# harrywaugh/UOB_Raytracer

Measured on AMD Instinct MI355X. Metric: Mrays/sec (nominal = W*H*AA*(1+S)/t), Cornell Box 4096^2, 8xAA, 64 shadow rays, higher is better.
Workload: dtype f32; 1 GPU; headline: Cornell Box 4096x4096, 4x2 AA, 64 shadow rays, 2 spheres, <=10 bounces, 26 triangles; parallelism=1 GPU

## Files before the change

include/uob_rt.h:

```cpp
#ifndef UOB_RT_H
#define UOB_RT_H

#include <stddef.h>
#include <stdint.h>

#ifdef __cplusplus
extern "C" {
#endif

#define RT_ABI_VERSION 2
#define RT_MAX_SPHERES 4
#define RT_MAX_DEVICES 8

enum {
  RT_OK = 0,
  RT_E_INVALID = -1,
  RT_E_DEVICE = -2,
  RT_E_NOMEM = -3,
  RT_E_IO = -4,
  RT_E_UNSUPPORTED = -5
};

typedef struct rt_sphere {
  float center[3];
// ... 39 lines not shown
            int32_t n_triangles, rt_ctx** out_ctx);

#define RT_UPDATE_REORDER 1u
int rt_update_scene(rt_ctx* ctx, const float* vertices4, const float* normals4, const float* colors4, int32_t n,
                    uint32_t flags);

int rt_update_scene_device(rt_ctx* ctx, const void* d_vertices4, const void* d_normals4, const void* d_colors4, int32_t n,
                           uint32_t flags, void* hip_stream);

#define RT_UPDATE_DEVICE_TILES 2u

int rt_replace_scene(rt_ctx* ctx, const float* vertices4, const float* normals4, const float* colors4, int32_t n_new,
                     uint32_t flags);

int rt_replace_scene_device(rt_ctx* ctx, const void* d_vertices4, const void* d_normals4, const void* d_colors4,
                            int32_t n_new, uint32_t flags, void* hip_stream);

int rt_update_spheres(rt_ctx* ctx, const rt_sphere* spheres, int32_t num_spheres);

int rt_debug_scene_capacity(rt_ctx* ctx, int64_t* out_triangles);

int rt_set_objects(rt_ctx* ctx, const int32_t* first, const int32_t* count, int32_t nobj);

int rt_pose_objects(rt_ctx* ctx, const float* xforms12, uint32_t flags);

int rt_pose_objects_device(rt_ctx* ctx, const void* d_xforms12, uint32_t flags, void* hip_stream);

int rt_debug_object_count(rt_ctx* ctx, int32_t* out);

int rt_set_skin(rt_ctx* ctx, int32_t first, int32_t count, const uint16_t* bone_index, const float* weights, int32_t nbones);

int rt_pose_skin(rt_ctx* ctx, const float* bones12, uint32_t flags);

int rt_pose_skin_device(rt_ctx* ctx, const void* d_bones12, uint32_t flags, void* hip_stream);

int rt_debug_skin_info(rt_ctx* ctx, int32_t* first, int32_t* count, int32_t* nbones);

int rt_render(rt_ctx* ctx, const float rot[12], const float cam[3], const float light[3], float focal,
              uint32_t* out_argb, float* out_rgb_f32);

int rt_render_device(rt_ctx* ctx, const float rot[12], const float cam[3], const float light[3],
                     float focal, void* d_out_argb, void* d_out_rgb_f32, void* hip_stream);

int rt_count_work(rt_ctx* ctx, const float rot[12], const float cam[3], const float light[3],
                  float focal, rt_work* out);

int rt_count_executed(rt_ctx* ctx, const float rot[12], const float cam[3], const float light[3],
                      float focal, uint64_t out[8]);

int rt_last_kernel_ms(rt_ctx* ctx, float* out_ms);

enum { RT_TRACE_IN_SHADOW = 0, RT_TRACE_CLOSEST_HIT = 1 };
int rt_debug_trace_rays(rt_ctx* ctx, int32_t what, const float* rays6, const float* radius_sq, int64_t nray,
                        int32_t* out_tri, float* out10);

int rt_trace_rays(rt_ctx* ctx, int32_t what, const float* rays6, const float* radius_sq, int64_t nray,
                  int32_t* out_tri, float* out10);
int rt_trace_rays_device(rt_ctx* ctx, int32_t what, const void* d_rays6, const void* d_radius_sq, int64_t nray,
                         void* d_out_tri, void* d_out10, void* hip_stream);
int rt_debug_trace_stats(rt_ctx* ctx, uint64_t out[8]);

int rt_shade_points(rt_ctx* ctx, const float* points6, const int32_t* seeds, int64_t npoints, const float light[3],
                    float* out_light, int32_t* out_unshadowed);
int rt_shade_points_device(rt_ctx* ctx, const void* d_points6, const void* d_seeds, int64_t npoints, const float light[3],
                           void* d_out_light, void* d_out_unshadowed, void* hip_stream);
int rt_debug_shade_stats(rt_ctx* ctx, uint64_t out[8]);

int rt_radiance_rays(rt_ctx* ctx, const float* rays6, const int32_t* seeds, int64_t nray, const float light[3],
                     float* out_rgba4, int32_t* out_prim);
int rt_radiance_rays_device(rt_ctx* ctx, const void* d_rays6, const void* d_seeds, int64_t nray, const float light[3],
                            void* d_out_rgba4, void* d_out_prim, void* hip_stream);
int rt_debug_radiance_stats(rt_ctx* ctx, uint64_t out[8]);

typedef struct rt_aov_buffers {
  int32_t* prim;
  float*   depth;
  float*   position4;
  float*   normal4;
  float*   albedo4;
  float*   direction4;
} rt_aov_buffers;

#define RT_AOV_ALL_SAMPLES (-1)
int rt_render_aov(rt_ctx* ctx, const float rot[12], const float cam[3], float focal, int32_t sample,
                  const rt_aov_buffers* host_out);
int rt_render_aov_device(rt_ctx* ctx, const float rot[12], const float cam[3], float focal, int32_t sample,
                         const rt_aov_buffers* device_out, void* hip_stream);
int rt_debug_aov_stats(rt_ctx* ctx, uint64_t out[8]);

typedef struct rt_filter_params {
  int32_t width, height;
  int32_t passes;
  float   normal_min_dot;
  float   plane_eps;
  float   value_max_diff;
} rt_filter_params;
void rt_filter_params_default(rt_filter_params* params, int32_t width, int32_t height);
int rt_filter_plane(rt_ctx* ctx, const rt_filter_params* params, const float* value, const float* position4,
                    const float* normal4, float* out);
int rt_filter_plane_device(rt_ctx* ctx, const rt_filter_params* params, const void* d_value, const void* d_position4,
                           const void* d_normal4, void* d_out, void* hip_stream);
int rt_debug_filter_stats(rt_ctx* ctx, uint64_t out[8]);
int rt_filter_plane_host(const rt_filter_params* params, const float* value, const float* position4, const float* normal4,
                         float* out);

typedef struct rt_history_texel {
  float position[3]; float mean;
  float normal[3];   float m2;
  float count;
  int32_t prim;
  float pad[2];
} rt_history_texel;

typedef struct rt_accumulate_params {
  int32_t width, height;
  float   prev_rot[12];
  float   prev_cam[3];
  float   prev_focal_px;
  float   normal_min_dot;
  float   plane_eps;
  int32_t max_history;
} rt_accumulate_params;
void rt_accumulate_params_default(rt_accumulate_params* params, int32_t width, int32_t height);
int rt_accumulate_plane(rt_ctx* ctx, const rt_accumulate_params* params, const float* value, const float* position4,
                        const float* normal4, const int32_t* prim, const rt_history_texel* prev, rt_history_texel* next,
                        float* out_mean, float* out_variance);
int rt_accumulate_plane_device(rt_ctx* ctx, const rt_accumulate_params* params, const void* d_value, const void* d_position4,
                               const void* d_normal4, const void* d_prim, const void* d_prev, void* d_next, void* d_out_mean,
                               void* d_out_variance, void* hip_stream);
int rt_debug_accumulate_stats(rt_ctx* ctx, uint64_t out[8]);
int rt_accumulate_plane_host(const rt_accumulate_params* params, const float* value, const float* position4,
                             const float* normal4, const int32_t* prim, const rt_history_texel* prev, rt_history_texel* next,
                             float* out_mean, float* out_variance);

int rt_debug_block_costs(rt_ctx* ctx, uint32_t* out, int32_t cap);

int rt_debug_world_masks(rt_ctx* ctx, uint64_t* out, int64_t cap, int32_t* grid, int32_t* words);

int rt_debug_tile_data(rt_ctx* ctx, int32_t* orig, float* tiles, int32_t cap_tiles);

int rt_debug_scene_data(rt_ctx* ctx, float* vertices4, float* normals4, float* colors4, float* vertices4_m,
                        float* normals4_m, float* colors4_m, int32_t* n_shadow, float vbox_lo[3], float vbox_hi[3],
                        int32_t cap_triangles);

int rt_register_output(rt_ctx* ctx, void* host, size_t bytes);
int rt_unregister_output(rt_ctx* ctx);

int rt_debug_wave_timeline(rt_ctx* ctx, uint64_t out[8]);

int rt_debug_wave_seeds(rt_ctx* ctx, void* records, int64_t cap, int32_t dims[3], uint64_t counters[4]);

int rt_debug_wave_seeds_wide(rt_ctx* ctx, void* records, int64_t cap, int32_t dims[3], uint64_t counters[10]);

enum { RT_COPY_2D = 0,
       RT_COPY_PEER = 1,
       RT_COPY_LINEAR = 2    };
typedef struct rt_band_copy {
  int32_t op, reserved;
  uint64_t dst_offset, dst_pitch, src_offset, src_pitch, width_bytes, rows;
} rt_band_copy;
int rt_debug_band_copy_plan(int32_t num_devices, int32_t k, int32_t device_band_rows, int32_t width, int32_t height,
                            int32_t elem_bytes, int32_t dev_to_dev, int32_t peer_ok, int32_t same_device,
                            rt_band_copy* out, int32_t cap);

int rt_selftest_rcp(uint64_t out[64]);

int rt_selftest_normalize(uint64_t out[8], uint32_t b_stride);

int rt_selftest_shade(int32_t nwaves, const int32_t* ns, const int32_t* lit, const int32_t* secondary, const int32_t* unshadowed,
                      const float* term, const float* col, int32_t straight_line, float* out);

int rt_selftest_all_within(int32_t nwaves, const int32_t* in, const float* v, const float* bound, int32_t* out);

void rt_destroy(rt_ctx* ctx);

int rt_debug_live_device_objects(int64_t out[4]);
const char* rt_last_error(void);
int rt_abi_version(void);

typedef struct rt_triangle {
  float v0[4], v1[4], v2[4], normal[4], color[4];
} rt_triangle;

int rt_scene_cornell_box(rt_triangle* out, int32_t cap);
int rt_scene_load_obj(const char* path, rt_triangle* out, int32_t cap);
int rt_scene_load_obj_ex(const char* path, const float color[4], float scale, const float translate[3],
                         rt_triangle* out, int32_t cap);
void rt_triangle_compute_normal(rt_triangle* t);
void rt_scene_transform(rt_triangle* tris, int32_t n, int32_t first, int32_t count, const float xform12[12]);
void rt_scene_skin(rt_triangle* tris, int32_t n, int32_t first, int32_t count, const uint16_t* bone_index,
                   const float* weights, const float* bones12, int32_t nbones);
void rt_scene_pack(const rt_triangle* tris, int32_t n, float* vertices4, float* normals4, float* colors4);
void rt_rotation_matrix(float yaw, float pitch, float rot[12]);

#ifdef __cplusplus
}
#endif
#endif
```

uob_raytracer_amd/csrc/rt_api.hip:

```cpp
#include <cmath>
#include <cstdarg>
#include <cstdio>
#include <cstdlib>
#include <cstring>
#include <memory>
#include <new>
#include <string>
#include <vector>

#include "rt_host.h"

namespace uobrt {

static thread_local std::string g_last_error;

void set_error(const char* fmt, ...) {
  char buf[1024];
  va_list ap;
  va_start(ap, fmt);
  vsnprintf(buf, sizeof buf, fmt, ap);
  va_end(ap);
  g_last_error = buf;
}

KeepError::KeepError() : text(g_last_error) {}
KeepError::~KeepError() { g_last_error = text; }

}

using namespace uobrt;

static int validate_config(const rt_config* c) {
  if (!c) { set_error("rt_config is NULL"); return RT_E_INVALID; }
  if (c->width < 1 || c->height < 1 || c->width > 32767 || c->height > 32767) {
    set_error("width/height must be in [1, 32767] (got %dx%d)", c->width, c->height); return RT_E_INVALID;
  }
  if (c->aa_x < 1 || c->aa_y < 1 || c->aa_x > 16 || c->aa_y > 16) { set_error("aa_x/aa_y must be in [1,16]"); return RT_E_INVALID; }
  if (c->shadow_samples < 1 || c->shadow_samples > 4096) { set_error("shadow_samples must be in [1,4096]"); return RT_E_INVALID; }
  if (c->max_bounces < 0 || c->max_bounces > 64) { set_error("max_bounces must be in [0,64]"); return RT_E_INVALID; }
  if (c->num_spheres < 0 || c->num_spheres > RT_MAX_SPHERES) { set_error("num_spheres must be in [0,%d]", RT_MAX_SPHERES); return RT_E_INVALID; }
  if (c->band_count < 1 || c->band_index < 0 || c->band_index >= c->band_count || c->band_rows < 1) {
    set_error("band partition invalid (rows=%d index=%d count=%d)", c->band_rows, c->band_index, c->band_count); return RT_E_INVALID;
  }
  if (!(c->light_spread >= 0.0f) || !(c->light_spread <= kMaxCoordinate)) { set_error("light_spread must be in [0, 2^16]"); return RT_E_INVALID; }
  if (validate_spheres(c->spheres, c->num_spheres) != RT_OK) return RT_E_INVALID;
  if ((double)c->width * c->height > 16777216.0) {
    set_error("width*height must not exceed 2^24 (the reference's FP32 pixel id)"); return RT_E_INVALID;
  }
  if (c->flags & 1) { set_error("flag bit 0 (the former RT_FLAG_FAST_MATH) is not defined in ABI %d", RT_ABI_VERSION); return RT_E_UNSUPPORTED; }
  if (c->num_devices < 0 || c->num_devices > RT_MAX_DEVICES || c->device_band_rows < 0) {
    set_error("num_devices must be in [0,%d] and device_band_rows >= 0", RT_MAX_DEVICES); return RT_E_INVALID;
  }
  if (c->num_devices > 1 && c->band_count != 1) {
    set_error("several devices in one context need the whole frame (band_count == 1)"); return RT_E_UNSUPPORTED;
  }
  return RT_OK;
}

static Tuning read_tuning(const rt_config& cfg) {
  Tuning t;
  if (const char* e = getenv("UOB_RT_JOB_TASKS")) t.job_tasks = atoi(e);
  if (const char* e = getenv("UOB_RT_HEAVY_FACTOR4")) { const int v = atoi(e); if (v >= 1 && v <= 4096) t.heavy_factor4 = v; }
  t.plain_order = (cfg.flags & RT_FLAG_PLAIN_ORDER) != 0 || getenv("UOB_RT_PLAIN_ORDER") != nullptr;
  t.full_grid = getenv("UOB_RT_FULL_GRID") != nullptr;
  t.no_specialise = getenv("UOB_RT_NO_SPECIALISE") != nullptr;
  if (const char* e = getenv("UOB_RT_HEAVY_DILATE")) t.heavy_dilate = atoi(e) != 0;
  if (const char* e = getenv("UOB_RT_L1_INFLATE")) { const float v = (float)atof(e); if (v >= 1.0f && v <= 64.0f) t.l1_inflate = v; }
  if (const char* e = getenv("UOB_RT_GRID_PER_CU")) { const int v = atoi(e); if (v >= 1 && v <= 8) t.grid_per_cu = v; }
  t.phase_profile = getenv("UOB_RT_PHASE_PROFILE") != nullptr;
  t.timeline = getenv("UOB_RT_TIMELINE") != nullptr;
  if (const char* e = getenv("UOB_RT_MASK_DEBUG")) t.mask_debug = atoi(e);
  if (const char* e = getenv("UOB_RT_TILE_ORDER")) t.tile_morton = !strcmp(e, "morton");
  if (const char* e = getenv("UOB_RT_NO_SEED")) t.no_seed = atoi(e) != 0;
  if (const char* e = getenv("UOB_RT_SEED_ROWS")) { const int v = atoi(e); if (v >= 1 && v <= 64) t.seed_rows = v; }
  if (const char* e = getenv("UOB_RT_SEED_KP")) { const int v = atoi(e); if (v >= 1 && v <= 64) t.seed_kp = v; }
  if (const char* e = getenv("UOB_RT_SEED_CASTERS")) { const int v = atoi(e); if (v >= 0 && v <= 64) t.seed_casters = v; }
  if (const char* e = getenv("UOB_RT_SEED_SPH")) t.seed_sph = atoi(e) != 0;
  if (const char* e = getenv("UOB_RT_FILTER_FORM")) t.filter_form = !strcmp(e, "direct") ? kFilterFormDirect : kFilterFormBuiltIn;
  return t;
}

extern "C" {

int rt_abi_version(void) { return RT_ABI_VERSION; }
const char* rt_last_error(void) { return g_last_error.c_str(); }

void rt_config_default(rt_config* cfg) {
  if (!cfg) return;
  memset(cfg, 0, sizeof *cfg);
  cfg->width = 1024; cfg->height = 1024;
  cfg->aa_x = 2; cfg->aa_y = 2;
  cfg->shadow_samples = 10; cfg->light_spread = 0.05f;
  cfg->max_bounces = 10;
  cfg->num_spheres = 2;
  const rt_sphere glass = {{0.3f, 0.1f, -0.5f}, 0.075f, {0.0f, 0.f, 0.f, -1.0f}};
  const rt_sphere mirror = {{-0.4f, 0.8f, -0.5f}, 0.05f, {0.0f, 0.f, 0.f, 0.0f}};
  cfg->spheres[0] = glass; cfg->spheres[1] = mirror;
  cfg->band_rows = cfg->height; cfg->band_index = 0; cfg->band_count = 1;
  cfg->device = -1; cfg->flags = 0;
  cfg->num_devices = 0; cfg->device_band_rows = 0;
}

int32_t rt_config_owned_rows(const rt_config* c) {
  if (!c || c->band_rows < 1 || c->band_count < 1) return 0;
  int rows = 0;
  for (int y = 0; y < c->height; ++y) rows += ((y / c->band_rows) % c->band_count) == c->band_index;
  return rows;
}

static int init_parent(const rt_config* cfg, const float* vertices4, const float* normals4, const float* colors4,
                       int32_t n, rt_ctx** out_ctx) {
  int ndev = 0;
  HIP_TRY(hipGetDeviceCount(&ndev));
  if (ndev < 1) { set_error("no HIP device present"); return RT_E_DEVICE; }
  for (int d = 0; d < cfg->num_devices; ++d)
    if (cfg->devices[d] < 0 || cfg->devices[d] >= ndev) {
      set_error("devices[%d] = %d, but %d HIP device(s) are present", d, cfg->devices[d], ndev); return RT_E_INVALID;
    }
  std::unique_ptr<rt_ctx> p(new (std::nothrow) rt_ctx());
  if (!p) { set_error("out of host memory"); return RT_E_NOMEM; }
  std::string downgrade;
  p->cfg = *cfg;
  p->device = cfg->devices[0];
  p->n = n; p->cap = n > 0 ? n : 1;
  p->owned_rows = rt_config_owned_rows(cfg);
  const int dbr = cfg->device_band_rows > 0 ? cfg->device_band_rows : 32;
  p->cfg.device_band_rows = dbr;
  for (int d = 0; d < cfg->num_devices; ++d) {
    rt_config kc = *cfg;
    kc.num_devices = 0; kc.device = cfg->devices[d];
    kc.band_rows = dbr; kc.band_index = d; kc.band_count = cfg->num_devices;
    rt_ctx* k = nullptr;
    const int rc = rt_init(&kc, vertices4, normals4, colors4, n, &k);
    if (rc != RT_OK) return rc;
    p->kids.push_back(k);
    if (hipSetDevice(k->device) != hipSuccess || k->ev_done.create(hipEventDisableTiming) != hipSuccess) {
      set_error("event creation failed on device %d", k->device); return RT_E_DEVICE;
    }
    if (k->device != p->device) {
      int can = 0;
      hipError_t e = hipDeviceCanAccessPeer(&can, k->device, p->device);
      if (e == hipSuccess && can) {
        e = hipDeviceEnablePeerAccess(p->device, 0);
        k->peer_ok = (e == hipSuccess || e == hipErrorPeerAccessAlreadyEnabled);
      } else {
        k->peer_ok = false;
      }
      (void)hipGetLastError();
      if (!k->peer_ok) {
        char line[160];
        snprintf(line, sizeof line, "%sdevice %d has no peer access to device %d (%s)", downgrade.empty() ? "warning: " : "; ",
                 k->device, p->device, e == hipSuccess ? "hipDeviceCanAccessPeer: no" : hipGetErrorString(e));
        downgrade += line;
      }
    }
  }
  if (hipSetDevice(p->device) != hipSuccess || p->ev_go.create(hipEventDisableTiming) != hipSuccess ||
      p->stream.create() != hipSuccess || p->ev0.create() != hipSuccess || p->ev1.create() != hipSuccess) {
    set_error("stream/event creation failed on device %d", p->device); return RT_E_DEVICE;
  }
  if (!downgrade.empty()) set_error("%s: their bands are copied band by band (hipMemcpyPeerAsync)", downgrade.c_str());
  *out_ctx = p.release();
  return RT_OK;
}

int rt_init(const rt_config* cfg, const float* vertices4, const float* normals4, const float* colors4,
            int32_t n, rt_ctx** out_ctx) {
  if (!out_ctx) { set_error("out_ctx is NULL"); return RT_E_INVALID; }
  *out_ctx = nullptr;
  int rc = validate_config(cfg);
  if (rc != RT_OK) return rc;
  if (n < 0 || (n > 0 && (!vertices4 || !normals4 || !colors4))) { set_error("scene arrays missing"); return RT_E_INVALID; }
  rc = validate_vertices(vertices4, n);
  if (rc != RT_OK) return rc;
  if (n > kMaxTriangles) { set_error("triangle list of %d exceeds the supported maximum of %d", n, kMaxTriangles); return RT_E_UNSUPPORTED; }
  DeviceGuard guard;
  if (cfg->num_devices > 1) return init_parent(cfg, vertices4, normals4, colors4, n, out_ctx);
  int ndev = 0;
  HIP_TRY(hipGetDeviceCount(&ndev));
  if (ndev < 1) { set_error("no HIP device present"); return RT_E_DEVICE; }
  std::unique_ptr<rt_ctx> c(new (std::nothrow) rt_ctx());
  if (!c) { set_error("out of host memory"); return RT_E_NOMEM; }
  c->cfg = *cfg;
  c->tune = read_tuning(*cfg);
  if (cfg->num_devices == 1) c->device = cfg->devices[0];
  else if (cfg->device >= 0) c->device = cfg->device;
  else hipGetDevice(&c->device);
  if (hipSetDevice(c->device) != hipSuccess) { set_error("hipSetDevice(%d) failed", c->device); return RT_E_DEVICE; }
  c->owned_rows = rt_config_owned_rows(cfg);
  if (hipDeviceGetAttribute(&c->cus, hipDeviceAttributeMultiprocessorCount, c->device) != hipSuccess || c->cus < 1) c->cus = 256;
  const size_t px = (size_t)(c->owned_rows > 0 ? c->owned_rows : 1) * cfg->width;
  if (c->d_argb.alloc(px) != hipSuccess || c->d_counters.alloc(sizeof(rt_work) / sizeof(unsigned long long)) != hipSuccess ||
      c->d_jobctr.alloc((2 * kJobHeads + 2) * kJobHeadStride) != hipSuccess || c->d_spheres.alloc(RT_MAX_SPHERES) != hipSuccess)
    return alloc_failed();
  {
    const int aa = cfg->aa_x * cfg->aa_y;
    const int pt = (aa >= 1 && aa <= 64) ? 64 / aa : 16;
    const size_t jobs_max = (size_t)((cfg->width + pt - 1) / pt) * (size_t)(c->owned_rows > 0 ? c->owned_rows : 1);
    c->heavy_cap = (int)(jobs_max / 3 > 64 ? jobs_max / 3 : 64);
    c->heavy_jobs_max = jobs_max;
  }
  if (c->stream.create() != hipSuccess || c->ev0.create() != hipSuccess || c->ev1.create() != hipSuccess) {
    set_error("stream/event creation failed"); return RT_E_DEVICE;
  }
  rc = upload_spheres(c.get());
  if (rc != RT_OK) return rc;
  rc = scene_first(c.get(), vertices4, normals4, colors4, n);
  if (rc != RT_OK) return rc;
  *out_ctx = c.release();
  return RT_OK;
}

}

void uobrt::fill_params(const rt_ctx* c, const float rot[12], const float cam[3], const float light[3], float focal,
                        FrameParams* P) {
  memset(P, 0, sizeof *P);
  memcpy(P->rot, rot, 12 * sizeof(float));
  memcpy(P->cam, cam, 3 * sizeof(float));
  memcpy(P->light, light, 3 * sizeof(float));
  P->focal = focal;
  const rt_config& g = c->cfg;
  P->spread = g.light_spread;
  P->W = g.width; P->H = g.height; P->aa_x = g.aa_x; P->aa_y = g.aa_y;
  P->S = g.shadow_samples; P->bounces = g.max_bounces; P->nsph = g.num_spheres; P->n = c->n;
  P->band_rows = g.band_rows; P->band_index = g.band_index; P->band_count = g.band_count;
  P->owned_rows = c->owned_rows;
  P->sy = (float)g.aa_x / (float)g.aa_y;
  {
    P->half_wx = ((float)g.width * (float)g.aa_x) / 2.0f;
    P->half_hy = ((float)g.height * (float)g.aa_y) / 2.0f;
    P->w_f = (float)g.width;
    P->focal0 = focal + 0.0f;
    P->rzf[0] = rot[2] * P->focal0; P->rzf[1] = rot[6] * P->focal0; P->rzf[2] = rot[10] * P->focal0;
    P->hbox = g.light_spread / 2.f;
    P->light_inf = fmaxf(fmaxf(fabsf(light[0]), fabsf(light[1])), fabsf(light[2]));
    P->band_rows_magic = div_magic_for(g.band_rows);
  }
  {
    const int aa = g.aa_x * g.aa_y;
    P->inv_S = (g.shadow_samples & (g.shadow_samples - 1)) == 0 ? 1.0f / (float)g.shadow_samples : 0.0f;
    P->inv_aa = (aa & (aa - 1)) == 0 ? 1.0f / (float)aa : 0.0f;
  }
  P->n_shadow = c->n_shadow;
  for (int i = 0; i < g.num_spheres; ++i) {
    P->sph[i].cx = g.spheres[i].center[0]; P->sph[i].cy = g.spheres[i].center[1]; P->sph[i].cz = g.spheres[i].center[2];
    P->sph[i].r2 = g.spheres[i].radius_sq;
    memcpy(P->sph[i].col, g.spheres[i].color, 16);
  }
  P->verts = c->d_verts; P->normals = c->d_normals; P->colors = c->d_colors;
  P->sph_dev = c->d_spheres;
  P->records = c->d_records;
  P->mask_debug = c->tune.mask_debug;
  P->job_counter = c->d_jobctr + kJobHeadStride;
  {
    const int aa = g.aa_x * g.aa_y;
    const bool wave_aa = aa >= 1 && aa <= 64;
    const int big_chunks = aa > 64 ? (aa + 63) / 64 : 0;
    const int pt = wave_aa ? 64 / aa : 64;
    P->aa_magic = wave_aa ? (65536 + aa - 1) / aa : 65536;
    P->aax_magic = (65536 + g.aa_x - 1) / g.aa_x;
    const int per_cu = c->tune.grid_per_cu ? c->tune.grid_per_cu : wave_blocks_per_cu(g.band_count > 1 && !c->tune.full_grid);
    P->wave_blocks = c->cus * per_cu;
    const long waves = (long)P->wave_blocks * 4;
    int jt = wave_aa ? 64 / pt : 1;
    while (jt > 1 && ((jt + 1) / 2) * pt >= 16 && (long)((g.width + jt * pt - 1) / (jt * pt)) * c->owned_rows < 16 * waves) jt = (jt + 1) / 2;
    if (wave_aa && c->tune.job_tasks >= 1 && c->tune.job_tasks * pt <= 64 && (c->tune.job_tasks * pt >= 16 || c->tune.job_tasks >= jt))
      jt = c->tune.job_tasks;
    if (big_chunks) jt = 16 * big_chunks;
    int job_pixels = 0;
    for (;;) {
      job_pixels = big_chunks ? jt / big_chunks : jt * pt;
      P->nseg = (g.width + job_pixels - 1) / job_pixels;
      P->njobs = P->nseg * c->owned_rows;
      P->nseg_magic = div_magic_for(P->nseg);
      if (big_chunks) break;
      const uint64_t err = P->nseg_magic ? (uint64_t)P->nseg_magic * (uint64_t)P->nseg - 0x100000000ull : 0ull;
      if ((uint64_t)(P->njobs > 0 ? P->njobs - 1 : 0) * err < 0x100000000ull || 2 * jt * pt > 64) break;
      jt *= 2;
    }
    P->job_tasks = jt;
    P->no_specialise = c->tune.no_specialise ? 1 : 0;
    P->l1_inflate = c->tune.l1_inflate;
    P->job_hx = 0.5f * (float)(job_pixels * g.aa_x - 1);
    P->job_hy = 0.5f * (float)(g.aa_y - 1) * P->sy;
    for (int k = 0; k < 3; ++k)
      P->job_eu[k] = 1.0001f * (fabsf(rot[4 * k]) * P->job_hx + fabsf(rot[4 * k + 1]) * P->job_hy);
  }
  if (c->d_screen_masks) {
    P->screen_masks = c->d_screen_masks; P->world_masks = c->d_world_masks; P->world_occ = c->d_world_occ;
    P->nwords = c->nwords; P->scx = c->scx; P->scy = c->scy; P->grid_g = kWorldGrid;
    float ext = 0.0f, dmax = 0.0f, amax = 0.0f, cmax = 0.0f;
    for (int k = 0; k < 3; ++k) {
      ext = fmaxf(ext, c->box_hi[k] - c->box_lo[k]);
      dmax = fmaxf(dmax, fmaxf(fabsf(light[k] - c->box_lo[k]), fabsf(light[k] - c->box_hi[k])));
      amax = fmaxf(amax, fmaxf(fabsf(c->box_lo[k]), fabsf(c->box_hi[k])));
      cmax = fmaxf(cmax, fabsf(cam[k]));
    }
    float grow = 2e-4f * dmax + 1e-4f * (amax + cmax) + 1e-3f * ext + 1e-30f;
    for (int i = 0; i < g.num_spheres; ++i) {
      float l2 = 0.0f;
      for (int k = 0; k < 3; ++k) l2 += (cam[k] - g.spheres[i].center[k]) * (cam[k] - g.spheres[i].center[k]);
      const float far = fmaxf(sqrtf(l2), 1.7321f * (ext + 2.0f * grow));
      grow = fmaxf(grow, 2.5e-3f * (far + sqrtf(fmaxf(g.spheres[i].radius_sq, 0.0f))));
    }
    for (int k = 0; k < 3; ++k) P->grid_lo[k] = c->box_lo[k] - grow;
    P->grid_cell = (ext + 2.0f * grow) / (float)kWorldGrid;
    P->grid_inv = 1.0f / P->grid_cell;
  }
}

void uobrt::use_tiled_scene(const rt_ctx* c, FrameParams* P) {
  P->verts = c->d_verts_m; P->normals = c->d_normals_m; P->colors = c->d_colors_m;
  P->orig = c->d_orig; P->tile_box = c->d_tile_box;
  P->mesh_blocks = c->cus * mesh_blocks_per_cu();
}

void uobrt::scene_params(const rt_ctx* c, const float light[3], bool tiled, FrameParams* P) {
  const float zero3[3] = {0.f, 0.f, 0.f}, ident[12] = {1, 0, 0, 0, 0, 1, 0, 0, 0, 0, 1, 0};
  fill_params(c, ident, zero3, light, 1.0f, P);
  if (tiled) use_tiled_scene(c, P);
}

static int launch_frame(rt_ctx* c, const float rot[12], const float cam[3], const float light[3], float focal,
                        uint32_t* d_argb, float4* d_rgb, hipStream_t stream, bool out_global = false) {
  if (!c || !rot || !cam || !light) { set_error("NULL argument"); return RT_E_INVALID; }
  for (int k = 0; k < 3; ++k)
    if (!(fabsf(cam[k]) <= kMaxCoordinate) || !(fabsf(light[k]) <= kMaxCoordinate)) {
      set_error("camera / light coordinates must be finite and <= 2^16"); return RT_E_INVALID;
    }
  if (!(fabsf(focal) <= 1.0e9f)) { set_error("focal length must be finite and <= 1e9"); return RT_E_INVALID; }
  for (int k = 0; k < 12; ++k)
    if (!(fabsf(rot[k]) <= 4.0f)) { set_error("rotation matrix entries must be finite and <= 4"); return RT_E_INVALID; }
  if (c->owned_rows == 0) return RT_OK;
  FrameParams P;
  fill_params(c, rot, cam, light, focal, &P);
  P.out_argb = d_argb; P.out_rgb = d_rgb; P.counters = nullptr;
  P.out_global = out_global ? 1 : 0;
  HIP_TRY(hipSetDevice(c->device));
  if (c->timed && stream != c->last_stream) HIP_TRY(hipStreamWaitEvent(stream, c->ev1, 0));
  HIP_TRY(wait_aov(c, stream));
  HIP_TRY(wait_scene(c, stream));
  HIP_TRY(hipEventRecord(c->ev0, stream));
  const bool wave_paths = !(c->cfg.flags & RT_FLAG_GENERIC_KERNEL);
  c->seed_tile_rows = 0;
  if (wave_paths && wave_kernel_supports(P) && (P.aa_x * P.aa_y <= 64 || !(c->cfg.flags & RT_FLAG_NO_CULL))) {
    if (c->d_heavy_flags && P.job_tasks >= 4) {
      const int prev = c->heavy_phase, cur = prev ^ 1;
      unsigned int* const st[2] = {c->d_jobctr, c->d_jobctr + (2 * kJobHeads + 1) * kJobHeadStride};
      P.heavy_prev = c->d_heavy[prev]; P.heavy_prev_state = st[prev];
      P.heavy_new = c->d_heavy[cur]; P.heavy_new_state = st[cur];
      P.heavy_flags = c->d_heavy_flags + (size_t)prev * c->heavy_jobs_max; P.heavy_flags_new = c->d_heavy_flags + (size_t)cur * c->heavy_jobs_max;
      P.heavy_gen = ++c->heavy_gen;
      P.heavy_factor4 = c->tune.heavy_factor4;
      P.heavy_cap = P.njobs / 3 < c->heavy_cap ? P.njobs / 3 : c->heavy_cap;
      P.heavy_dilate = c->tune.heavy_dilate ? 1 : 0;
      c->heavy_phase = cur;
    }
    c->timeline_valid = false;
    if (c->tune.timeline) {
      const size_t waves = (size_t)P.wave_blocks * 4;
      if (!c->d_timeline) {
        if (c->d_timeline.alloc(waves * 3) != hipSuccess) { set_error("hipMalloc failed (timeline)"); return RT_E_NOMEM; }
        c->timeline_waves = waves;
      }
      if (c->timeline_waves >= waves) {
        HIP_TRY(hipMemsetAsync(c->d_timeline, 0, c->timeline_waves * 3 * sizeof(uint64_t), stream));
        P.counters = reinterpret_cast<unsigned long long*>(c->d_timeline.p);
        c->timeline_valid = true;
      }
    }
    if (!c->tune.no_seed && wave_takes_seed(P, !(c->cfg.flags & RT_FLAG_NO_CULL))) {
      const int R = c->tune.seed_rows;
      const int tile_rows = (P.H + R - 1) / R;
      const size_t tiles = (size_t)tile_rows * (size_t)P.nseg;
      if (c->seed_cap < tiles) {
        if (c->d_seed.alloc(tiles) != hipSuccess) return alloc_failed();
        c->seed_cap = tiles;
      }
      P.seed = c->d_seed; P.seed_rows = R; P.seed_tile_rows = tile_rows; P.seed_rows_magic = div_magic_for(R);
      P.seed_hy = 0.5f * (float)(R * P.aa_y - 1) * P.sy;
      for (int k = 0; k < 3; ++k) P.seed_eu[k] = 1.0001f * (fabsf(rot[4 * k]) * P.job_hx + fabsf(rot[4 * k + 1]) * P.seed_hy);
      P.seed_kp_cap = c->tune.seed_kp; P.seed_caster_cap = c->tune.seed_casters; P.seed_keep_sph = c->tune.seed_sph ? 1 : 0;
      c->seed_tile_rows = tile_rows; c->seed_nseg = P.nseg; c->seed_rows = R;
    }
    launch_wave(P, !(c->cfg.flags & RT_FLAG_NO_CULL), false, stream);
  } else if (wave_paths && !(c->cfg.flags & RT_FLAG_NO_CULL) && mesh_kernel_supports(P)) {
    use_tiled_scene(c, &P);
    if (c->d_mesh_cost) {
      P.mesh_order = c->mesh_order_valid ? c->d_mesh_order : nullptr;
      P.mesh_cost = c->d_mesh_cost; P.mesh_order_out = c->d_mesh_order;
      P.mesh_queue_len = c->d_mesh_order + 4 * (size_t)((c->cfg.width + 15) / 16) * (size_t)((c->owned_rows + 15) / 16);
      c->mesh_order_valid = true;
    }
    launch_stage_records(P, stream);
    launch_mesh(P, false, false, stream, c->aux_stream, c->ev_fork, c->ev_join);
  } else {
    launch_generic(P, false, stream);
  }
  HIP_TRY(hipGetLastError());
  HIP_TRY(hipEventRecord(c->ev1, stream));
  c->timed = true;
  c->last_stream = stream;
  return RT_OK;
}

static int band_copy_plan(int N, int k, int dbr, int W, int owned_rows, size_t elem, bool dev_to_dev, bool peer_ok,
                          bool same_device, rt_band_copy* out, int cap) {
  const size_t band_bytes = (size_t)dbr * W * elem;
  const int full = owned_rows / dbr, rem = owned_rows % dbr;
  const size_t d0 = (size_t)k * band_bytes;
  int cnt = 0;
  auto emit = [&](int op, size_t doff, size_t dpitch, size_t soff, size_t spitch, size_t width, size_t rows) {
    if (cnt < cap && out) {
      rt_band_copy& c = out[cnt];
      c.op = op; c.reserved = 0; c.dst_offset = doff; c.dst_pitch = dpitch; c.src_offset = soff; c.src_pitch = spitch;
      c.width_bytes = width; c.rows = rows;
    }
    ++cnt;
  };
  if (full > 0) {
    if (!dev_to_dev || peer_ok) {
      emit(RT_COPY_2D, d0, (size_t)N * band_bytes, 0, band_bytes, band_bytes, (size_t)full);
    } else {
      for (int b = 0; b < full; ++b)
        emit(RT_COPY_PEER, d0 + (size_t)b * N * band_bytes, 0, (size_t)b * band_bytes, 0, band_bytes, 1);
    }
  }
  if (rem > 0) {
    const size_t bytes = (size_t)rem * W * elem;
    emit(dev_to_dev && !same_device ? RT_COPY_PEER : RT_COPY_LINEAR, d0 + (size_t)full * N * band_bytes, 0,
         (size_t)full * band_bytes, 0, bytes, 1);
  }
  return cnt;
}

static int deliver_bands(rt_ctx* p, int k, const void* stripe, void* dst, size_t elem, hipMemcpyKind kind, hipStream_t stream) {
  rt_ctx* c = p->kids[k];
  const int N = (int)p->kids.size(), dbr = p->cfg.device_band_rows, W = p->cfg.width;
  const bool d2d = kind == hipMemcpyDeviceToDevice;
  const int full = c->owned_rows / dbr;
  std::vector<rt_band_copy> plan((size_t)full + 2);
  int cnt = band_copy_plan(N, k, dbr, W, c->owned_rows, elem, d2d, c->peer_ok, c->device == p->device, plan.data(), (int)plan.size());
  for (int i = 0; i < cnt; ++i) {
    const rt_band_copy& q = plan[(size_t)i];
    char* const d = (char*)dst + q.dst_offset;
    const char* const sp = (const char*)stripe + q.src_offset;
    if (q.op == RT_COPY_2D) {
      const hipError_t e = hipMemcpy2DAsync(d, q.dst_pitch, sp, q.src_pitch, q.width_bytes, q.rows, kind, stream);
      if (e != hipSuccess && d2d && c->device != p->device) {
        (void)hipGetLastError();
        c->peer_ok = false;
        set_error("warning: device %d cannot copy 2-D into device %d (%s): its bands go band by band through hipMemcpyPeerAsync",
                  c->device, p->device, hipGetErrorString(e));
        cnt = band_copy_plan(N, k, dbr, W, c->owned_rows, elem, d2d, false, false, plan.data(), (int)plan.size());
        i = -1;
        continue;
      }
      if (e != hipSuccess) { set_error("hipMemcpy2DAsync failed: %s", hipGetErrorString(e)); return RT_E_DEVICE; }
    } else if (q.op == RT_COPY_PEER) {
      HIP_TRY(hipMemcpyPeerAsync(d, p->device, sp, c->device, q.width_bytes, stream));
    } else {
      HIP_TRY(hipMemcpyAsync(d, sp, q.width_bytes, kind, stream));
    }
  }
  return RT_OK;
}

static int parent_render(rt_ctx* p, const float rot[12], const float cam[3], const float light[3], float focal,
                         uint32_t* host_argb, float* host_rgb, uint32_t* d_argb, float4* d_rgb, hipStream_t caller) {
  const bool to_host = host_argb != nullptr;
  const size_t W = (size_t)p->cfg.width;
  const size_t nk = p->kids.size();
  if (!to_host) {
    HIP_TRY(hipSetDevice(p->device));
    HIP_TRY(hipEventRecord(p->ev0, caller));
    HIP_TRY(hipEventRecord(p->ev_go, caller));
  }
  const bool want_rgb = to_host ? host_rgb != nullptr : d_rgb != nullptr;
  std::vector<char> launched(nk, 0), direct(nk, 0);
  auto fail = [&](int rc) {
    KeepError keep;
    for (size_t k = 0; k < nk; ++k)
      if (launched[k]) { hipSetDevice(p->kids[k]->device); hipStreamSynchronize(p->kids[k]->stream); }
    (void)hipGetLastError();
    return rc;
  };
  for (size_t k = 0; k < nk; ++k) {
    rt_ctx* c = p->kids[k];
    if (c->owned_rows == 0) continue;
    if (hipSetDevice(c->device) != hipSuccess) { set_error("hipSetDevice(%d) failed", c->device); return fail(RT_E_DEVICE); }
    if (want_rgb && !c->d_rgb && c->d_rgb.alloc((size_t)c->owned_rows * W) != hipSuccess) {
      set_error("hipMalloc failed (float tap, device %d)", c->device); return fail(RT_E_NOMEM);
    }
    if (!to_host && hipStreamWaitEvent(c->stream, p->ev_go, 0) != hipSuccess) { set_error("hipStreamWaitEvent failed"); return fail(RT_E_DEVICE); }
    const bool mapped = to_host && !host_rgb && c->reg_host && (char*)host_argb >= c->reg_host &&
                        (char*)host_argb + (size_t)p->cfg.height * W * 4 <= c->reg_host + c->reg_bytes &&
                        !(p->cfg.flags & RT_FLAG_STAGED_GATHER);
    direct[k] = mapped || (!to_host && c->device == p->device && !(p->cfg.flags & RT_FLAG_STAGED_GATHER));
    uint32_t* const dst = mapped ? reinterpret_cast<uint32_t*>(c->reg_dev + ((char*)host_argb - c->reg_host)) : d_argb;
    const int rc = direct[k] ? launch_frame(c, rot, cam, light, focal, dst, mapped ? nullptr : d_rgb, c->stream, true)
                             : launch_frame(c, rot, cam, light, focal, c->d_argb, want_rgb ? c->d_rgb : nullptr, c->stream);
    if (rc != RT_OK) return fail(rc);
    launched[k] = 1;
  }
  for (size_t k = 0; k < nk; ++k) {
    rt_ctx* c = p->kids[k];
    if (!launched[k]) continue;
    if (hipSetDevice(c->device) != hipSuccess) { set_error("hipSetDevice(%d) failed", c->device); return fail(RT_E_DEVICE); }
    if (!direct[k]) {
      const hipMemcpyKind kind = to_host ? hipMemcpyDeviceToHost : hipMemcpyDeviceToDevice;
      int rc = deliver_bands(p, (int)k, c->d_argb, to_host ? (void*)host_argb : (void*)d_argb, 4, kind, c->stream);
      if (rc == RT_OK && want_rgb)
        rc = deliver_bands(p, (int)k, c->d_rgb, to_host ? (void*)host_rgb : (void*)d_rgb, sizeof(float4), kind, c->stream);
      if (rc != RT_OK) return fail(rc);
    }
    if (!to_host && hipEventRecord(c->ev_done, c->stream) != hipSuccess) { set_error("hipEventRecord failed"); return fail(RT_E_DEVICE); }
  }
  if (to_host) {
    for (rt_ctx* c : p->kids) if (c->owned_rows) { HIP_TRY(hipSetDevice(c->device)); HIP_TRY(hipStreamSynchronize(c->stream)); }
    p->timed = false;
  } else {
    HIP_TRY(hipSetDevice(p->device));
    for (rt_ctx* c : p->kids) if (c->owned_rows) HIP_TRY(hipStreamWaitEvent(caller, c->ev_done, 0));
    HIP_TRY(hipEventRecord(p->ev1, caller));
    p->timed = true;
  }
  return RT_OK;
}

extern "C" {

int rt_render_device(rt_ctx* c, const float rot[12], const float cam[3], const float light[3], float focal,
                     void* d_out_argb, void* d_out_rgb_f32, void* hip_stream) {
  if (!c || !d_out_argb) { set_error("NULL argument"); return RT_E_INVALID; }
  DeviceGuard guard;
  if (!c->kids.empty()) {
// ... 49 lines not shown
  return RT_OK;
}

int rt_register_output(rt_ctx* c, void* host, size_t bytes) {
  if (!c || !host || bytes == 0) { set_error("NULL argument"); return RT_E_INVALID; }
  const int rc = rt_unregister_output(c);
  if (rc != RT_OK) return rc;
  DeviceGuard guard;
  HIP_TRY(hipSetDevice(c->device));
  HIP_TRY(hipHostRegister(host, bytes, hipHostRegisterMapped | hipHostRegisterPortable));
  auto alias = [&](rt_ctx* x) -> bool {
    void* dev = nullptr;
    if (hipSetDevice(x->device) != hipSuccess || hipHostGetDevicePointer(&dev, host, 0) != hipSuccess || !dev) return false;
    x->reg_host = static_cast<char*>(host); x->reg_dev = static_cast<char*>(dev); x->reg_bytes = bytes;
    return true;
  };
  bool ok = alias(c);
  for (rt_ctx* k : c->kids) ok = ok && alias(k);
  if (!ok) {
    for (rt_ctx* k : c->kids) { k->reg_host = k->reg_dev = nullptr; k->reg_bytes = 0; }
    c->reg_host = c->reg_dev = nullptr; c->reg_bytes = 0;
    hipHostUnregister(host);
    set_error("hipHostGetDevicePointer failed: %s", hipGetErrorString(hipGetLastError()));
    return RT_E_DEVICE;
  }
  c->reg_owner = true;
  return RT_OK;
}

int rt_count_work(rt_ctx* c, const float rot[12], const float cam[3], const float light[3], float focal, rt_work* out) {
  if (!c || !out || !rot || !cam || !light) { set_error("NULL argument"); return RT_E_INVALID; }
  memset(out, 0, sizeof *out);
  DeviceGuard guard;
  if (!c->kids.empty()) {
    for (rt_ctx* k : c->kids) {
      rt_work w;
      const int rc = rt_count_work(k, rot, cam, light, focal, &w);
      if (rc != RT_OK) return rc;
      for (size_t q = 0; q < sizeof(rt_work) / 8; ++q) ((uint64_t*)out)[q] += ((const uint64_t*)&w)[q];
    }
    return RT_OK;
  }
  if (c->owned_rows == 0) return RT_OK;
  FrameParams P;
  fill_params(c, rot, cam, light, focal, &P);
  P.counters = c->d_counters;
  HIP_TRY(hipSetDevice(c->device));
  HIP_TRY(wait_aov(c, c->stream));
  HIP_TRY(wait_scene(c, c->stream));
  HIP_TRY(hipMemsetAsync(c->d_counters, 0, sizeof(rt_work), c->stream));
  launch_generic(P, true, c->stream);
  HIP_TRY(hipGetLastError());
  HIP_TRY(hipMemcpyAsync(out, c->d_counters, sizeof(rt_work), hipMemcpyDeviceToHost, c->stream));
  HIP_TRY(hipStreamSynchronize(c->stream));
  return RT_OK;
}

int rt_count_executed(rt_ctx* c, const float rot[12], const float cam[3], const float light[3], float focal, uint64_t out[8]) {
  if (!c || !out || !rot || !cam || !light) { set_error("NULL argument"); return RT_E_INVALID; }
  memset(out, 0, 8 * sizeof(uint64_t));
  DeviceGuard guard;
  if (!c->kids.empty()) {
    for (rt_ctx* k : c->kids) {
      uint64_t w[8];
      const int rc = rt_count_executed(k, rot, cam, light, focal, w);
      if (rc != RT_OK) return rc;
      for (int q = 0; q < 8; ++q) out[q] += w[q];
    }
    return RT_OK;
  }
  if (c->owned_rows == 0) return RT_OK;
  FrameParams P;
  fill_params(c, rot, cam, light, focal, &P);
  const bool generic = (c->cfg.flags & RT_FLAG_GENERIC_KERNEL) != 0;
  const bool mesh = !generic && !wave_kernel_supports(P) && !(c->cfg.flags & RT_FLAG_NO_CULL) && mesh_kernel_supports(P);
  if (generic || (!wave_kernel_supports(P) && !mesh) || (!mesh && P.S > 64)) {
    set_error("rt_count_executed: this configuration runs on the generic kernel, whose executed work is rt_count_work");
    return RT_E_UNSUPPORTED;
  }
  if (!mesh && P.aa_x * P.aa_y > 64) {
    set_error("rt_count_executed: more than 64 AA samples per pixel run on the wave kernel's chunked build, which has no counting build");
    return RT_E_UNSUPPORTED;
  }
  P.counters = c->d_counters;
  HIP_TRY(hipSetDevice(c->device));
  if (c->timed) HIP_TRY(hipStreamWaitEvent(c->stream, c->ev1, 0));
  HIP_TRY(wait_aov(c, c->stream));
  HIP_TRY(wait_scene(c, c->stream));
  HIP_TRY(hipMemsetAsync(c->d_counters, 0, sizeof(rt_work), c->stream));
  if (mesh) { use_tiled_scene(c, &P); launch_stage_records(P, c->stream); launch_mesh(P, true, c->tune.phase_profile, c->stream, nullptr, nullptr, nullptr); }
  else if (c->tune.phase_profile) launch_wave_prof(P, c->stream);
  else launch_wave(P, !(c->cfg.flags & RT_FLAG_NO_CULL), true, c->stream);
  HIP_TRY(hipGetLastError());
  HIP_TRY(hipMemcpyAsync(out, c->d_counters, sizeof(rt_work), hipMemcpyDeviceToHost, c->stream));
  HIP_TRY(hipStreamSynchronize(c->stream));
  return RT_OK;
}

int rt_debug_wave_timeline(rt_ctx* c, uint64_t out[8]) {
  if (!c || !out) { set_error("NULL argument"); return RT_E_INVALID; }
  c = lead_ctx(c);
  if (!c->tune.timeline || !c->timeline_valid) {
    set_error("rt_debug_wave_timeline: needs UOB_RT_TIMELINE=1 at rt_init and a frame rendered by the wave kernel");
    return RT_E_UNSUPPORTED;
  }
  DeviceGuard guard;
  HIP_TRY(hipSetDevice(c->device));
  if (c->timed) HIP_TRY(hipEventSynchronize(c->ev1));
  std::vector<uint64_t> rec(c->timeline_waves * 3);
  HIP_TRY(hipMemcpy(rec.data(), c->d_timeline, rec.size() * sizeof(uint64_t), hipMemcpyDeviceToHost));
  for (int q = 0; q < 8; ++q) out[q] = 0;
  out[1] = ~0ull;
  for (size_t w = 0; w < c->timeline_waves; ++w) {
    const uint64_t t0 = rec[3 * w], t1 = rec[3 * w + 1], jobs = rec[3 * w + 2] & 0xffffffffull;
    if (t1 == 0) continue;
    out[7] = rec[3 * w + 2] >> 32;
    out[0] += 1; out[3] += t0; out[4] += t1; out[5] += jobs;
    if (t0 < out[1]) out[1] = t0;
    if (t1 > out[2]) out[2] = t1;
    if (jobs > out[6]) out[6] = jobs;
  }
  return RT_OK;
}

static int read_seed_table(rt_ctx* c, std::vector<SeedRec>* rec, std::vector<uint64_t>* rows) {
  rec->clear(); rows->clear();
  if (c->seed_tile_rows == 0) return RT_OK;
  DeviceGuard guard;
  HIP_TRY(hipSetDevice(c->device));
  if (c->timed) HIP_TRY(hipEventSynchronize(c->ev1));
  rec->resize((size_t)c->seed_tile_rows * (size_t)c->seed_nseg);
  HIP_TRY(hipMemcpy(rec->data(), c->d_seed, rec->size() * sizeof(SeedRec), hipMemcpyDeviceToHost));
  const rt_config& g = c->cfg;
  rows->assign((size_t)c->seed_tile_rows, 0);
  for (int tr = 0; tr < c->seed_tile_rows; ++tr)
    for (int y = tr * c->seed_rows; y < (tr + 1) * c->seed_rows && y < g.height; ++y)
      (*rows)[tr] += ((y / g.band_rows) % g.band_count) == g.band_index;
  return RT_OK;
}

int rt_debug_wave_seeds(rt_ctx* c, void* records, int64_t cap, int32_t dims[3], uint64_t counters[4]) {
  if (!c || !dims || !counters || cap < 0 || (cap > 0 && !records)) { set_error("NULL argument"); return RT_E_INVALID; }
  c = lead_ctx(c);
  dims[0] = c->seed_tile_rows; dims[1] = c->seed_nseg; dims[2] = c->seed_rows;
  for (int q = 0; q < 4; ++q) counters[q] = 0;
  if (c->seed_tile_rows == 0) { dims[1] = 0; return RT_OK; }
  std::vector<SeedRec> rec;
  std::vector<uint64_t> rows;
  const int rc = read_seed_table(c, &rec, &rows);
  if (rc != RT_OK) return rc;
  for (size_t t = 0; t < rec.size(); ++t) {
    SeedRec& r = rec[t];
    r.flags &= kSeedPrimary | kSeedShadow;
    if (!(r.flags & kSeedPrimary)) r.Kp = 0ull;
    if (!(r.flags & kSeedShadow)) { r.D0[0] = r.D0[1] = r.D0[2] = 0.0f; r.ed = 0.0f; r.K = 0ull; r.Kh = 0ull; r.h = -1; }
    const uint64_t n = rows[t / (size_t)c->seed_nseg];
    if (r.flags & kSeedPrimary) { counters[0] += 1; counters[2] += n; }
    if (r.flags & kSeedShadow) { counters[1] += 1; counters[3] += n; }
  }
  if (records) memcpy(records, rec.data(), (size_t)((int64_t)rec.size() < cap ? (int64_t)rec.size() : cap) * sizeof(SeedRec));
  return RT_OK;
}

int rt_debug_wave_seeds_wide(rt_ctx* c, void* records, int64_t cap, int32_t dims[3], uint64_t counters[10]) {
  if (!c || !dims || !counters || cap < 0 || (cap > 0 && !records)) { set_error("NULL argument"); return RT_E_INVALID; }
  c = lead_ctx(c);
  dims[0] = c->seed_tile_rows; dims[1] = c->seed_nseg; dims[2] = c->seed_rows;
  for (int q = 0; q < 10; ++q) counters[q] = 0;
  if (c->seed_tile_rows == 0) { dims[1] = 0; return RT_OK; }
  std::vector<SeedRec> rec;
  std::vector<uint64_t> rows;
  const int rc = read_seed_table(c, &rec, &rows);
  if (rc != RT_OK) return rc;
  for (size_t t = 0; t < rec.size(); ++t) {
    const SeedRec& r = rec[t];
    const uint64_t n = rows[t / (size_t)c->seed_nseg];
    const bool shadow = (r.flags & kSeedShadowWide) != 0u;
    const bool is[5] = {(r.flags & kSeedPrimaryWide) != 0u, shadow, shadow && r.Kh != 0ull, shadow && (r.flags & kSeedShadowSph) != 0u,
                        shadow && (r.flags & kSeedShadowBlocked) != 0u};
    for (int q = 0; q < 5; ++q)
      if (is[q]) { counters[2 * q] += 1; counters[2 * q + 1] += n; }
  }
  if (records) memcpy(records, rec.data(), (size_t)((int64_t)rec.size() < cap ? (int64_t)rec.size() : cap) * sizeof(SeedRec));
  return RT_OK;
}

int rt_debug_trace_rays(rt_ctx* c, int32_t what, const float* rays6, const float* radius_sq, int64_t nray,
                        int32_t* out_tri, float* out10) {
  if (!c || !rays6 || !out_tri || nray < 0) { set_error("NULL argument"); return RT_E_INVALID; }
  if (what != RT_TRACE_IN_SHADOW && what != RT_TRACE_CLOSEST_HIT) { set_error("rt_debug_trace_rays: unknown mode %d", what); return RT_E_INVALID; }
  if (what == RT_TRACE_IN_SHADOW && !radius_sq) { set_error("rt_debug_trace_rays: radius_sq missing"); return RT_E_INVALID; }
  if (what == RT_TRACE_CLOSEST_HIT && !out10) { set_error("rt_debug_trace_rays: out10 missing"); return RT_E_INVALID; }
  c = lead_ctx(c);
  if (nray == 0) return RT_OK;
  DeviceGuard guard;
  HIP_TRY(hipSetDevice(c->device));
  const float zero3[3] = {0.f, 0.f, 0.f};
  FrameParams P;
  scene_params(c, zero3, false, &P);
  DevMem<float> d_rays, d_r2, d_out;
  DevMem<int> d_tri;
  const size_t n = (size_t)nray;
  if (d_rays.alloc(n * 6) != hipSuccess || d_tri.alloc(n) != hipSuccess || (radius_sq && d_r2.alloc(n) != hipSuccess) ||
      (out10 && d_out.alloc(n * 10) != hipSuccess))
    return alloc_failed();
  if (c->timed) HIP_TRY(hipStreamWaitEvent(c->stream, c->ev1, 0));
  HIP_TRY(wait_aov(c, c->stream));
  HIP_TRY(wait_scene(c, c->stream));
  HIP_TRY(hipMemcpyAsync(d_rays, rays6, n * 24, hipMemcpyHostToDevice, c->stream));
  if (radius_sq) HIP_TRY(hipMemcpyAsync(d_r2, radius_sq, n * 4, hipMemcpyHostToDevice, c->stream));
  if (d_out) HIP_TRY(hipMemsetAsync(d_out, 0, n * 40, c->stream));
  if (generic_needs_records(c->n)) launch_stage_records(P, c->stream);
  launch_trace_rays(P, what, d_rays, d_r2, (long)nray, d_tri, d_out, c->stream);
  HIP_TRY(hipGetLastError());
  HIP_TRY(hipMemcpyAsync(out_tri, d_tri, n * 4, hipMemcpyDeviceToHost, c->stream));
  if (out10 && what == RT_TRACE_CLOSEST_HIT) HIP_TRY(hipMemcpyAsync(out10, d_out, n * 40, hipMemcpyDeviceToHost, c->stream));
  HIP_TRY(hipStreamSynchronize(c->stream));
  return RT_OK;
}

int rt_debug_band_copy_plan(int32_t num_devices, int32_t k, int32_t device_band_rows, int32_t width, int32_t height,
                            int32_t elem_bytes, int32_t dev_to_dev, int32_t peer_ok, int32_t same_device,
                            rt_band_copy* out, int32_t cap) {
  if (num_devices < 1 || num_devices > RT_MAX_DEVICES || k < 0 || k >= num_devices || device_band_rows < 0 || width < 1 ||
      height < 1 || elem_bytes < 1 || cap < 0 || (!out && cap > 0)) {
    set_error("rt_debug_band_copy_plan: invalid argument"); return RT_E_INVALID;
  }
  const int dbr = device_band_rows > 0 ? device_band_rows : 32;
  rt_config kc;
  memset(&kc, 0, sizeof kc);
  kc.height = height; kc.band_rows = dbr; kc.band_index = k; kc.band_count = num_devices;
  return band_copy_plan(num_devices, k, dbr, width, rt_config_owned_rows(&kc), (size_t)elem_bytes, dev_to_dev != 0, peer_ok != 0,
                        same_device != 0, out, cap);
}

int rt_debug_block_costs(rt_ctx* c, uint32_t* out, int32_t cap) {
  if (!c || (!out && cap > 0) || cap < 0) { set_error("NULL argument"); return RT_E_INVALID; }
  c = lead_ctx(c);
  if (!c->d_mesh_cost || !c->mesh_order_valid) { set_error("rt_debug_block_costs: this context records no block costs"); return RT_E_UNSUPPORTED; }
  DeviceGuard guard;
  HIP_TRY(hipSetDevice(c->device));
  const int jobs = ((c->cfg.width + 15) / 16) * ((c->owned_rows + 15) / 16);
  if (c->timed) HIP_TRY(hipEventSynchronize(c->ev1));
  std::vector<uint32_t> raw((size_t)jobs);
  HIP_TRY(hipMemcpy(raw.data(), c->d_mesh_cost, (size_t)jobs * 4, hipMemcpyDeviceToHost));
  const int wx = (c->cfg.width + 15) / 16, wy = (c->owned_rows + 15) / 16, mid = (wy + 1) >> 1;
  for (int j = 0; j < jobs; ++j) {
    const int jy = j / wx, jx = j - jy * wx;
    const int row = (jy & 1) ? mid + (jy >> 1) : mid - 1 - (jy >> 1);
    const int at = row * wx + jx;
    if (at >= 0 && at < cap) out[at] = raw[(size_t)j];
  }
  return jobs;
}

int rt_debug_world_masks(rt_ctx* c, uint64_t* out, int64_t cap, int32_t* grid, int32_t* words) {
  if (!c || (!out && cap > 0) || cap < 0 || !grid || !words) { set_error("NULL argument"); return RT_E_INVALID; }
  c = lead_ctx(c);
  if (!c->d_world_masks || c->nwords <= 0) { set_error("rt_debug_world_masks: this context builds no tile masks"); return RT_E_UNSUPPORTED; }
  DeviceGuard guard;
  HIP_TRY(hipSetDevice(c->device));
  if (c->timed) HIP_TRY(hipEventSynchronize(c->ev1));
  const size_t total = (size_t)kWorldGrid * kWorldGrid * kWorldGrid * (size_t)c->nwords;
  *grid = kWorldGrid; *words = c->nwords;
  const size_t take = total < (size_t)cap ? total : (size_t)cap;
  if (take > 0) HIP_TRY(hipMemcpy(out, c->d_world_masks, take * 8, hipMemcpyDeviceToHost));
  return (int)total;
}

int rt_last_kernel_ms(rt_ctx* c, float* out_ms) {
  if (!c || !out_ms) { set_error("NULL argument"); return RT_E_INVALID; }
  DeviceGuard guard;
  if (!c->kids.empty() && !c->timed) {
    float mx = -1.0f;
    for (rt_ctx* k : c->kids) {
      float ms = 0.0f;
      if (k->timed && rt_last_kernel_ms(k, &ms) == RT_OK && ms > mx) mx = ms;
    }
    if (mx < 0.0f) { set_error("no frame has been rendered on this context"); return RT_E_INVALID; }
    *out_ms = mx;
    return RT_OK;
  }
  if (!c->timed) { set_error("no frame has been rendered on this context"); return RT_E_INVALID; }
  HIP_TRY(hipSetDevice(c->device));
  HIP_TRY(hipEventSynchronize(c->ev1));
  HIP_TRY(hipEventElapsedTime(out_ms, c->ev0, c->ev1));
  return RT_OK;
}

int rt_debug_live_device_objects(int64_t out[4]) {
  if (!out) { set_error("rt_debug_live_device_objects: NULL argument"); return RT_E_INVALID; }
  for (int k = 0; k < 4; ++k) out[k] = g_live[k].load(std::memory_order_relaxed);
  return RT_OK;
}

void rt_destroy(rt_ctx* c) {
  if (!c) return;
  DeviceGuard guard;
  delete c;
}

}

rt_ctx::~rt_ctx() {
  for (rt_ctx* k : kids) delete k;
  hipSetDevice(device);
  if (stream) hipStreamSynchronize(stream);
  if (aux_stream) hipStreamSynchronize(aux_stream);
  for (SideCall* k : {&query, &shade, &rad, &aov, &filter, &accum})
    if (k->ev) hipEventSynchronize(k->ev);
  if (reg_host && reg_owner) hipHostUnregister(reg_host);
}
```

uob_raytracer_amd/csrc/rt_device.h:

```cpp
#pragma once
#include <hip/hip_runtime.h>
#include <stdint.h>

#include "../../include/uob_rt.h"

namespace uobrt {

constexpr int kJobHeads = 31;
constexpr int kJobHeadStride = 32;
constexpr int kHeavyStateWords = 8;
constexpr float kMaxCoordinate = 65536.0f;
constexpr int kRecordsPerTriangle = 8;

struct DevSphere {
  float cx, cy, cz, r2;
  float col[4];
};

struct alignas(16) SeedRec {
  float D0[3], ed;
  unsigned long long K, Kh, Kp;
  int32_t h;
  uint32_t flags;
  uint32_t pad[4];
};
constexpr uint32_t kSeedPrimary = 1u, kSeedShadow = 2u;
constexpr uint32_t kSeedPrimaryWide = 4u, kSeedPrimarySph = 8u;
constexpr int kSeedShadowShift = 4;
constexpr uint32_t kSeedShadowWide = 1u << kSeedShadowShift, kSeedShadowSph = 2u << kSeedShadowShift, kSeedShadowBlocked = 4u << kSeedShadowShift;
static_assert(sizeof(SeedRec) == 64, "one record per 64-byte line");

struct FrameParams {
  float rot[12];
  float cam[3];
  float focal;
  float light[3];
  float spread;
  int32_t W, H, aa_x, aa_y;
  int32_t S;
  int32_t bounces;
  int32_t nsph;
  int32_t n;
  int32_t band_rows, band_index, band_count, owned_rows;
  float sy;
  float half_wx, half_hy;
  float w_f;
  float focal0;
  float rzf[3];
  float hbox;
  float light_inf;
  float job_hx, job_hy;
  float job_eu[3];
  uint32_t nseg_magic, band_rows_magic;
  float inv_S, inv_aa;
  int32_t n_shadow;
  DevSphere sph[RT_MAX_SPHERES];
  const DevSphere* sph_dev;
  const float4* verts;
  const float4* normals;
  const float4* colors;
  uint32_t* out_argb;
  float4* out_rgb;
  int32_t out_global;
  int32_t wave_blocks;
  unsigned long long* counters;
  unsigned int* job_counter;
  int32_t njobs, nseg;
  int32_t aa_magic;
  int32_t aax_magic;
  int32_t job_tasks;
  int32_t no_specialise;
  const unsigned int* heavy_prev;
  const unsigned int* heavy_prev_state;
  unsigned int* heavy_new;
  unsigned int* heavy_new_state;
  const unsigned int* heavy_flags;
  unsigned int* heavy_flags_new;
  uint32_t heavy_gen;
  int32_t heavy_factor4;
  int32_t heavy_cap;
  float l1_inflate;
  int32_t heavy_dilate;
  float4* records;
  const unsigned int* mesh_order;
  unsigned int* mesh_cost;
  unsigned int* mesh_order_out;
  unsigned int* mesh_queue_len;
  int32_t mesh_blocks;
  const int* orig;
  const float4* tile_box;
  unsigned long long* screen_masks;
  unsigned long long* world_masks;
  unsigned int* world_occ;
  int32_t mask_debug;
  int32_t nwords, scx, scy, grid_g;
  float grid_lo[3], grid_cell, grid_inv;
  SeedRec* seed;
  int32_t seed_rows;
  int32_t seed_tile_rows;
  uint32_t seed_rows_magic;
  float seed_hy;
  float seed_eu[3];
  int32_t seed_kp_cap, seed_caster_cap, seed_keep_sph;
};


struct AovPlanes {
  int* prim;
  float* depth;
  float4 *position, *normal, *albedo, *direction;
};

__device__ inline uint32_t div_magic(uint32_t n, uint32_t magic) { return magic ? __umulhi(n, magic) : n; }

__host__ __device__ inline int band_global_row(int lr, int band_rows, int band_index, int band_count) {
  return ((lr / band_rows) * band_count + band_index) * band_rows + (lr % band_rows);
}
__device__ inline int band_global_row(const struct FrameParams& P, int lr);

__device__ inline int band_global_row(const FrameParams& P, int lr) {
  const int q = (int)div_magic((uint32_t)lr, P.band_rows_magic);
  return (q * P.band_count + P.band_index) * P.band_rows + (lr - q * P.band_rows);
}

}
```

uob_raytracer_amd/csrc/rt_host.h:

```cpp
#pragma once
#include <hip/hip_runtime.h>

#include <atomic>
#include <string>
#include <utility>
#include <vector>

#include "rt_device.h"

#define HIP_TRY(expr)                                                                   \
  do {                                                                                  \
    hipError_t e_ = (expr);                                                             \
    if (e_ != hipSuccess) {                                                             \
      uobrt::set_error("%s failed: %s (%s:%d)", #expr, hipGetErrorString(e_), __FILE__, __LINE__); \
      return RT_E_DEVICE;                                                               \
    }                                                                                   \
  } while (0)

namespace uobrt {

void set_error(const char* fmt, ...);

struct KeepError {
  std::string text;
  KeepError();
  ~KeepError();
};

constexpr int kMaxTriangles = 4000000;
constexpr int kWorldGrid = 32;

void launch_generic(const FrameParams& P, bool count, hipStream_t stream);
bool generic_needs_records(int n);
void launch_stage_records(const FrameParams& P, hipStream_t stream);
void launch_trace_rays(const FrameParams& P, int what, const float* d_rays, const float* d_r2, long nray, int* d_tri,
                       float* d_out10, hipStream_t stream);
void launch_wave(const FrameParams& P, bool cull, bool count, hipStream_t stream);
void launch_wave_prof(const FrameParams& P, hipStream_t stream);
bool wave_kernel_supports(const FrameParams& P);
bool wave_takes_seed(const FrameParams& P, bool cull);
int wave_blocks_per_cu(bool leave_room);
void launch_mesh(const FrameParams& P, bool count, bool prof, hipStream_t stream, hipStream_t aux, hipEvent_t ev_fork, hipEvent_t ev_join);
void launch_bin_primary(const FrameParams& P, hipStream_t stream);
bool mesh_kernel_supports(const FrameParams& P);
int mesh_tiles(int n);
int mesh_occ_words(int grid);
int mesh_screen_cells(int pixels);
int mesh_blocks_per_cu();
int launch_scene_check(const float4* v, const float4* col, int n, unsigned int* out, hipStream_t stream);
void launch_scene_refit(const float4* v, const float4* nrm, const float4* col, const int* orig, int n, float4* vm, float4* nm,
                        float4* cm, float4* tile_box, hipStream_t stream);
constexpr unsigned int kPoseStatic = 0xffffu;
void launch_pose(const float4* rest_v, const float4* rest_n, const unsigned short* object_of, const float* d_xforms12, int n,
                 float4* out_v, float4* out_n, hipStream_t stream);
void launch_skin(const float4* rest_v, const float4* rest_n, const ushort4* index, const float4* weights, const float* d_bones12,
                 int n, int first, int count, float4* out_v, float4* out_n, hipStream_t stream);
size_t tile_build_scratch_bytes(int n);
int launch_tile_build(const float4* v, int n, const float lo[3], const float hi[3], int* orig, void* scratch, hipStream_t stream);
int query_stats_words();
void launch_query(const FrameParams& P, bool tiled, int what, const float* d_rays, const float* d_r2, long nray, int* d_tri,
                  float* d_out10, unsigned long long* stats, int cus, hipStream_t stream);
int shade_stats_words();
void launch_shade(const FrameParams& P, bool tiled, const float* d_points6, const int* d_seeds, long npoints, float* d_light,
                  int* d_cnt, unsigned long long* stats, int cus, hipStream_t stream);
int radiance_stats_words();
size_t radiance_record_bytes(long nray);
void launch_radiance(const FrameParams& P, bool tiled, const float* d_rays6, const int* d_seeds, long nray, float4* d_rgba,
                     int* d_prim, float4* d_records, unsigned long long* stats, int cus, hipStream_t stream);
int aov_stats_words();
void launch_aov(const FrameParams& P, bool tiled, const AovPlanes& A, int sample, unsigned long long* stats, int cus, hipStream_t stream);
constexpr int kFilterTX = 64, kFilterTY = 4, kFilterMaxTiledSpacing = 32;
constexpr int kFilterFormBuiltIn = 0, kFilterFormDirect = 1;
int filter_stats_words();
void launch_filter_pack(const float4* d_pos, const float4* d_nrm, long count, int passes, float4* d_rec, unsigned long long* stats,
                        hipStream_t stream);
void launch_filter_pass(const rt_filter_params& p, int pass, int form, const float4* d_rec, const float* d_src, float* d_dst,
                        unsigned long long* stats, hipStream_t stream);
void launch_filter_counters(unsigned long long* stats, hipStream_t stream);
int filter_check(const rt_filter_params* p, const void* value, const void* position4, const void* normal4, const void* out,
                 const char* fn);
int accumulate_stats_words();
void launch_accumulate(const rt_accumulate_params& p, const float* d_value, const float4* d_pos, const float4* d_nrm, const int* d_prim,
                       const float4* d_prev, float4* d_next, float* d_out_mean, float* d_out_variance, unsigned long long* stats,
                       hipStream_t stream);
int accumulate_check(const rt_accumulate_params* p, const void* value, const void* position4, const void* normal4, const void* prev,
                     const void* next, const char* fn);
void vertex_box(const float* vertices4, int n, float lo[3], float hi[3]);
std::vector<int> tiled_order(const float* v4, int n, bool morton);
std::vector<float> tile_data_host(const float* v4, const int* orig, int n);

inline uint32_t div_magic_for(int d) { return d > 1 ? (uint32_t)((0x100000000ull + (uint64_t)d - 1) / (uint64_t)d) : 0u; }

inline int blocks_per_cu(const void* kernel, int threads) {
  int per_cu = 0;
  if (hipOccupancyMaxActiveBlocksPerMultiprocessor(&per_cu, kernel, threads, 0) != hipSuccess || per_cu < 1) per_cu = 2;
  return per_cu;
}
inline unsigned grid_blocks(long want, long cap) { return (unsigned)(want < cap ? (want > 0 ? want : 1) : cap); }

struct Tuning {
  int job_tasks = 0;
  int heavy_factor4 = 8;
  bool plain_order = false;
  bool full_grid = false;
  float l1_inflate = 3.5f;
  bool heavy_dilate = true;
  bool no_specialise = false;
  int grid_per_cu = 0;
  bool phase_profile = false;
  bool timeline = false;
  int mask_debug = 0;
  bool tile_morton = false;
  int filter_form = 0;
  bool no_seed = false;
  int seed_rows = 16;
  int seed_kp = 64;
  int seed_casters = 32;
  bool seed_sph = true;
};

inline std::atomic<int64_t> g_live[4];
inline void live_add(int slot, int64_t d) { g_live[slot].fetch_add(d, std::memory_order_relaxed); }

template <class T>
struct DevMem {
  T* p = nullptr;
  size_t bytes = 0;
  DevMem() = default;
  DevMem(DevMem&& o) noexcept : p(std::exchange(o.p, nullptr)), bytes(std::exchange(o.bytes, 0)) {}
  DevMem& operator=(DevMem&& o) noexcept {
    if (this != &o) { reset(); p = std::exchange(o.p, nullptr); bytes = std::exchange(o.bytes, 0); }
    return *this;
  }
  ~DevMem() { reset(); }
  hipError_t alloc(size_t count) {
    reset();
    const size_t want = count ? count * sizeof(T) : 1;
    const hipError_t e = hipMalloc(&p, want);
    if (e != hipSuccess) { p = nullptr; return e; }
    bytes = want; live_add(0, 1); live_add(1, (int64_t)want);
    return hipSuccess;
  }
  void reset() {
    if (p) { hipFree(p); live_add(0, -1); live_add(1, -(int64_t)bytes); }
    p = nullptr; bytes = 0;
  }
  operator T*() const { return p; }
};
inline int alloc_failed() { set_error("hipMalloc failed: %s", hipGetErrorString(hipGetLastError())); return RT_E_NOMEM; }
using DevBuffer = DevMem<char>;
int ensure_bytes(DevBuffer* b, size_t bytes);

template <class H, hipError_t (*Create)(H*, unsigned), hipError_t (*Destroy)(H), int Slot>
struct Handle {
  H h = nullptr;
  Handle() = default;
  Handle(Handle&& o) noexcept : h(std::exchange(o.h, nullptr)) {}
  Handle& operator=(Handle&& o) noexcept { if (this != &o) { reset(); h = std::exchange(o.h, nullptr); } return *this; }
  ~Handle() { reset(); }
  hipError_t create(unsigned flags = 0) {
    reset();
    const hipError_t e = Create(&h, flags);
    if (e != hipSuccess) h = nullptr; else live_add(Slot, 1);
    return e;
  }
  void reset() { if (h) { Destroy(h); live_add(Slot, -1); h = nullptr; } }
  operator H() const { return h; }
};
using Event = Handle<hipEvent_t, hipEventCreateWithFlags, hipEventDestroy, 2>;
using Stream = Handle<hipStream_t, hipStreamCreateWithFlags, hipStreamDestroy, 3>;

struct SceneStore {
  DevMem<float4> verts_m, normals_m, colors_m, tile_box, records;
  DevMem<int> orig;
  DevMem<unsigned long long> screen_masks, world_masks;
  DevMem<unsigned int> world_occ;
  DevMem<unsigned int> heavy[2], heavy_flags, mesh_cost, mesh_order;
};

struct SideCall {
  Event ev;
  bool pending = false;
  DevMem<unsigned long long> d_stats;
  int tiles = 0;
  DevBuffer io;
};

}

struct rt_ctx {
  ~rt_ctx();
  rt_config cfg;
  uobrt::Tuning tune;
  int device = 0;
  int n = 0, n_shadow = 0;
  int cap = 0;
  uobrt::SceneStore own;
  uobrt::DevBuffer tile_scratch;
  int owned_rows = 0;
  uobrt::DevMem<float4> d_verts, d_normals, d_colors;
  uobrt::DevMem<uint32_t> d_argb;
  uobrt::DevMem<float4> d_rgb;
  uobrt::DevMem<unsigned long long> d_counters;
  uobrt::DevMem<unsigned int> d_jobctr;
  uobrt::DevMem<uobrt::SeedRec> d_seed;
  size_t seed_cap = 0;
  int seed_tile_rows = 0, seed_nseg = 0, seed_rows = 0;
  int cus = 256;
  unsigned int *d_heavy[2] = {nullptr, nullptr}, *d_heavy_flags = nullptr;
  int heavy_cap = 0, heavy_phase = 0;
  size_t heavy_jobs_max = 0;
  char* reg_host = nullptr; char* reg_dev = nullptr; size_t reg_bytes = 0;
  bool reg_owner = false;
  bool timeline_valid = false;
  uobrt::DevMem<uint64_t> d_timeline;
  size_t timeline_waves = 0;
  uint32_t heavy_gen = 0;
  float4* d_records = nullptr;
  float4 *d_verts_m = nullptr, *d_normals_m = nullptr, *d_colors_m = nullptr, *d_tile_box = nullptr;
  int* d_orig = nullptr;
  uobrt::DevMem<uobrt::DevSphere> d_spheres;
  unsigned int *d_mesh_cost = nullptr, *d_mesh_order = nullptr;
  bool mesh_order_valid = false;
  unsigned long long *d_screen_masks = nullptr, *d_world_masks = nullptr;
  unsigned int* d_world_occ = nullptr;
  int nwords = 0, scx = 0, scy = 0;
  float box_lo[3] = {0, 0, 0}, box_hi[3] = {0, 0, 0};
  float vbox_lo[3] = {0, 0, 0}, vbox_hi[3] = {0, 0, 0};
  uobrt::Stream stream;
  uobrt::Stream aux_stream;
  uobrt::Event ev_fork, ev_join;
  uobrt::Event ev0, ev1;
  bool timed = false;
  hipStream_t last_stream = nullptr;
  std::vector<rt_ctx*> kids;
  uobrt::Event ev_go;
  uobrt::Event ev_done;
  bool peer_ok = true;
  uobrt::Event ev_upd;
  bool upd_pending = false;
  uobrt::DevMem<unsigned int> d_check;
  int nobj = 0;
  uobrt::DevMem<float4> d_rest_verts, d_rest_normals;
  uobrt::DevMem<unsigned short> d_object_of;
  uobrt::DevBuffer pose_verts, pose_normals, pose_xforms;
  int skin_first = 0, skin_count = 0, skin_nbones = 0;
  uobrt::DevMem<ushort4> d_skin_index;
  uobrt::DevMem<float4> d_skin_weights;
  uobrt::SideCall query, shade, rad;
  uobrt::DevMem<float4> d_qrecords;
  uobrt::DevBuffer rrec;
  uobrt::SideCall aov;
  hipStream_t aov_stream = nullptr;
  uobrt::SideCall filter;
  uobrt::DevBuffer filter_guides, filter_planes;
  uobrt::SideCall accum;
};

namespace uobrt {

struct DeviceGuard {
  int prev = -1;
  DeviceGuard() { if (hipGetDevice(&prev) != hipSuccess) prev = -1; }
  ~DeviceGuard() { if (prev >= 0) hipSetDevice(prev); }
};

inline rt_ctx* lead_ctx(rt_ctx* c) { return c->kids.empty() ? c : c->kids[0]; }

inline hipError_t wait_scene(const rt_ctx* c, hipStream_t s) {
  return c->upd_pending ? hipStreamWaitEvent(s, c->ev_upd, 0) : hipSuccess;
}
// ... 21 lines not shown
```

uob_raytracer_amd/csrc/rt_kernel_wave.hip:

```cpp
#define RT_SPHERES_IN_LDS
#define RT_RNG_JUMP_IN_LDS
#include "rt_host.h"
#include "rt_wave_common.h"

#include <type_traits>

namespace uobrt {

namespace {

constexpr int kChunk = 4;

struct WaveLds {
  float4* r0;
  float4* r1;
  float2* r2;
  float4* h0;
  float4* h1;
  uint32_t* rng;
};
__host__ __device__ constexpr int wave_lds_bytes(bool cull) {
  return (cull ? 0 : 64 * (16 + 16 + 8)) + 64 * 32 + kRngPixels * kRngStride * 4;
}

// ... 132 lines not shown

template <int SP>
__device__ __forceinline__ void wave_unshadowed_packed(const FrameParams& P, const ShadowCasters& SC, const WaveLds& L, int lane,
                                                       unsigned long long pmA, int baseA, const uint32_t* rngA,
                                                       unsigned long long pmB, int baseB, const uint32_t* rngB,
                                                       unsigned long long K, unsigned long long need_l, unsigned long long sphmask,
                                                       int NS, int& unshadowed) {
  constexpr int PK = 64 / SP;
  const int q = lane / SP, sidx = lane - q * SP;
  int ja[PK], jb[PK];
  {
    unsigned long long m = pmA;
#pragma unroll
    for (int i = 0; i < PK; ++i) { ja[i] = m != 0ull ? baseA + __builtin_ctzll(m) : -1; m &= m - 1ull; }
    m = pmB;
#pragma unroll
    for (int i = 0; i < PK; ++i) { jb[i] = m != 0ull ? baseB + __builtin_ctzll(m) : -1; m &= m - 1ull; }
  }
  int myA = ja[0], myB = jb[0];
#pragma unroll
  for (int i = 1; i < PK; ++i) { myA = q == i ? ja[i] : myA; myB = q == i ? jb[i] : myB; }
  const bool actA = myA >= 0 && sidx < NS, actB = myB >= 0 && sidx < NS;
  unsigned long long need = 0ull;
#pragma unroll
  for (int i = 0; i < PK; ++i) {
    if (ja[i] >= 0) need |= ((unsigned long long)(unsigned)__builtin_amdgcn_readlane((int)(need_l >> 32), ja[i]) << 32) | (unsigned)__builtin_amdgcn_readlane((int)need_l, ja[i]);
    if (jb[i] >= 0) need |= ((unsigned long long)(unsigned)__builtin_amdgcn_readlane((int)(need_l >> 32), jb[i]) << 32) | (unsigned)__builtin_amdgcn_readlane((int)need_l, jb[i]);
  }
  const float4 ha0 = L.h0[actA ? myA : 0], ha1 = L.h1[actA ? myA : 0], hb0 = L.h0[actB ? myB : 0], hb1 = L.h1[actB ? myB : 0];
  const f3 sa = mk(ha0.x, ha0.y, ha0.z), sb = mk(hb0.x, hb0.y, hb0.z);
  const float ra = ha0.w, rb = hb0.w;
  const int sw = (sidx < NS ? sidx : 0) * 4;
  const f3 jitA = mk(crush1(rngA[sw], P.spread), crush1(rngA[sw + 1], P.spread), crush1(rngA[sw + 2], P.spread));
  const f3 jitB = mk(crush1(rngB[sw], P.spread), crush1(rngB[sw + 1], P.spread), crush1(rngB[sw + 2], P.spread));
  const f3 da = mk(ha1.x, ha1.y, ha1.z) + jitA, db = mk(hb1.x, hb1.y, hb1.z) + jitB;
  const f3 nda = -da, ndb = -db;
  bool blkA = false, blkB = false;
  int pos = 0;
  for (unsigned long long kk = K; kk != 0ull; kk &= kk - 1ull, ++pos) {
    if (((need >> pos) & 1ull) == 0ull) continue;
    const int k = __builtin_ctzll(kk);
    const f3 v0 = xyz(SC.v0[k]), e1 = xyz(SC.e1[k]), e2 = xyz(SC.e2[k]), c = xyz(SC.c[k]);
    const f3 ba = sa - v0, bb = sb - v0;
    const float nA0a = detc(ba, c), nA0b = detc(bb, c);
    const float detAa = detc(nda, c), detAb = detc(ndb, c);
    float rra = rcp_newton(detAa, 1), rrb = rcp_newton(detAb, 1);
    float ta = nA0a * rra, tb = nA0b * rrb;
    f3 dva = ta * da, dvb = tb * db;
    float dista = dva.x * dva.x + dva.y * dva.y + dva.z * dva.z;
    float distb = dvb.x * dvb.x + dvb.y * dvb.y + dvb.z * dvb.z;
    bool passa = !(ta < 0.0f) && !(dista >= ra), passb = !(tb < 0.0f) && !(distb >= rb);
    if (ballot((actA && !blkA && passa) || (actB && !blkB && passb)) == 0ull) continue;
    if (ballot((actA && rra != rra) || (actB && rrb != rrb)) != 0ull) {
      rra = 1.0f / detAa; rrb = 1.0f / detAb;
      ta = nA0a * rra; tb = nA0b * rrb;
      dva = ta * da; dvb = tb * db;
      dista = dva.x * dva.x + dva.y * dva.y + dva.z * dva.z;
      distb = dvb.x * dvb.x + dvb.y * dvb.y + dvb.z * dvb.z;
      passa = ta >= 0 && dista < ra; passb = tb >= 0 && distb < rb;
    }
    const float ua = detc(nda, cof(ba, e2)) * rra, va = detc(nda, cof(e1, ba)) * rra;
    const float ub = detc(ndb, cof(bb, e2)) * rrb, vb = detc(ndb, cof(e1, bb)) * rrb;
    blkA = blkA || (passa && ua >= 0 && va >= 0 && (ua + va) <= 1);
    blkB = blkB || (passb && ub >= 0 && vb >= 0 && (ub + vb) <= 1);
    if (ballot((actA && !blkA) || (actB && !blkB)) == 0ull) break;
  }
  const bool sphA = actA && ((sphmask >> (myA >= 0 ? myA : 0)) & 1ull) != 0ull, sphB = actB && ((sphmask >> (myB >= 0 ? myB : 0)) & 1ull) != 0ull;
  if (ballot((sphA && !blkA) || (sphB && !blkB)) != 0ull) {
    Work unused;
    if (sphA && !blkA) blkA = shadow_spheres<false>(P, sa, da, ra, unused);
    if (sphB && !blkB) blkB = shadow_spheres<false>(P, sb, db, rb, unused);
  }
  const unsigned long long mA = ballot(actA && !blkA), mB = ballot(actB && !blkB);
#pragma unroll
  for (int i = 0; i < PK; ++i) {
    if (jb[i] >= 0 && lane == jb[i]) unshadowed = __popcll((mB >> (i * SP)) & ((1ull << SP) - 1ull));
    if (ja[i] >= 0 && lane == ja[i]) unshadowed = __popcll((mA >> (i * SP)) & ((1ull << SP) - 1ull));
  }
}


}

constexpr int kWavesPerBlock = 4;
constexpr int kMinWaves = 5;
template <int STRIDE, bool CULL>
__host__ __device__ constexpr int wave_fixed_lds_float4() {
  return kLdsRecords * STRIDE + STRIDE / 4 + 4 * STRIDE + kWavesPerBlock * wave_lds_bytes(CULL) / 16;
}

template <bool CULL, bool COUNT, bool PROF = false, int STRIDE = 0, bool MULTI = false, int AA_X = 0, int AA_Y = 0, int SS = 0, bool BIGAA = false>
__global__ __launch_bounds__(64 * kWavesPerBlock, kMinWaves) void rt_draw_wave(const FrameParams P) {
  unsigned long long prof[8] = {0, 0, 0, 0, 0, 0, 0, 0};
  unsigned long long tlast = PROF ? __builtin_amdgcn_s_memtime() : 0ull;
  extern __shared__ float4 lds_dyn[];
  __shared__ float4 lds_fix[STRIDE ? wave_fixed_lds_float4<STRIDE ? STRIDE : 4, CULL>() : 1];
  float4* const lds = STRIDE ? lds_fix : lds_dyn;
  const int tid = threadIdx.x;
  const int wave = tid >> 6, lane = tid & 63;
  const int n = P.n, ns = P.n_shadow;
  const int st = STRIDE ? STRIDE : n, sst = STRIDE ? STRIDE : ns;

  stage_triangles(P, lds, tid, 64 * kWavesPerBlock, st);
  stage_spheres(P, tid);
  stage_rng_jump(tid);
  int* sidx = reinterpret_cast<int*>(lds + kLdsRecords * st);
  if (wave == 0) {
    const bool casts = (lane < n) && (P.colors[lane < n ? lane : 0].w != -1.0f);
    const unsigned long long m = ballot(casts);
    if (casts) sidx[__popcll(m & ((1ull << lane) - 1ull))] = lane;
  }
  RT_STAMP(prof, 7)
  __syncthreads();
  float4* scbase = reinterpret_cast<float4*>(sidx + ((st + 3) & ~3));
  for (int kq = tid; kq < ns; kq += 64 * kWavesPerBlock) {
    const int ti = sidx[kq];
    scbase[kq] = lds[ti]; scbase[sst + kq] = lds[st + ti]; scbase[2 * sst + kq] = lds[2 * st + ti];
    const float4 c4 = lds[3 * st + ti];
    scbase[3 * sst + kq] = make_float4(c4.x, c4.y, c4.z, norm1(xyz(c4)));
  }
  __syncthreads();
  const ShadowCasters SC{scbase, scbase + sst, scbase + 2 * sst, scbase + 3 * sst};
  const WaveLds L = wave_lds(reinterpret_cast<char*>(scbase + 4 * sst) + wave * wave_lds_bytes(CULL), CULL);

  const LdsScene S = lds_scene(lds, n, st);
  const int aa_x = AA_X ? AA_X : P.aa_x, aa_y = AA_Y ? AA_Y : P.aa_y;
  const float sy = (AA_X && AA_Y) ? (float)AA_X / (float)AA_Y : P.sy;
  const int aa_full = aa_x * aa_y;
  const int chunks = BIGAA ? (aa_full + 63) >> 6 : 1;
  const int aa = BIGAA ? 64 : aa_full;
  const int PT = BIGAA ? 1 : 64 / aa;
  f3 aa_run = mk(0.f, 0.f, 0.f);
  const int GP = PT < kRngPixels ? PT : kRngPixels;
  const int gp_magic = (65536 + GP - 1) / GP;
  const f3 light = mk(P.light[0], P.light[1], P.light[2]);
  const float hbox = P.hbox;
  const unsigned long long tri_lanes = ns == 64 ? ~0ull : ((1ull << ns) - 1ull);
  const int NS = SS ? SS : P.S;
  const float inv_S = SS ? ((SS & (SS - 1)) == 0 ? 1.0f / (float)(SS ? SS : 1) : 0.0f) : P.inv_S;
  const float inv_aa = (AA_X && AA_Y) ? (((AA_X * AA_Y) & (AA_X * AA_Y - 1)) == 0 ? 1.0f / (float)(AA_X * AA_Y ? AA_X * AA_Y : 1) : 0.0f) : P.inv_aa;
  const int n_pass = MULTI ? (NS + 63) >> 6 : 1;
  const unsigned long long active = NS >= 64 ? ~0ull : ((1ull << NS) - 1ull);

  const int tl = lane < ns ? lane : 0;
  TriLane T;
  if (!CULL) {
    T = tri_lane(SC.v0, SC.e1, SC.e2, SC.c, tl);
    L.r0[lane] = make_float4(T.c.x, T.c.y, T.c.z, 0.f);
  }

  RT_STAMP(prof, 0)
  Work wk, xw;
  if (COUNT) for (int q = 0; q < 8; ++q) xw.v[q] = 0;
  int head = (int)((blockIdx.x * kWavesPerBlock + wave) % kJobHeads);
  const bool lpt = !COUNT && !PROF && PC(heavy_new) != nullptr;
  unsigned int n_heavy = 0u;
  unsigned long long heavy_thr = ~0ull;
  unsigned long long* const cost_acc = reinterpret_cast<unsigned long long*>(L.rng + 256);
  if (lpt && lane == 0) { cost_acc[0] = 0ull; cost_acc[1] = 0ull; }
  if (lpt) {
    n_heavy = PC(heavy_prev_state)[0] < (unsigned int)PC(heavy_cap) ? PC(heavy_prev_state)[0] : (unsigned int)PC(heavy_cap);
    const unsigned long long psum = ((unsigned long long)PC(heavy_prev_state)[3] << 32) | PC(heavy_prev_state)[2];
    const unsigned int pjobs = PC(heavy_prev_state)[4];
    if (pjobs != 0u) heavy_thr = (unsigned long long)PC(heavy_factor4) * (psum / pjobs) / 4ull;
  }
  const bool timeline = !COUNT && !PROF && PC(counters) != nullptr;
  unsigned long long* const tls = reinterpret_cast<unsigned long long*>(L.rng + kRngStride + 256);
  if (timeline && lane == 0) { tls[0] = __builtin_amdgcn_s_memrealtime(); tls[1] = 0ull; }
  bool phase_a = n_heavy != 0u;
  const int grid_waves = (int)gridDim.x * kWavesPerBlock;
  const int per_wave = PC(job_tasks) * PT > 32 ? 8 * grid_waves : grid_waves;
  int next_job = -1, chunk_left = 0;
  unsigned int listed = 0u;
  int chunk = PC(njobs) > 2 * per_wave ? kChunk : (PC(njobs) > per_wave ? 2 : 1);
  for (;;) {
  int job = 0;
  const int jt = PC(job_tasks);
  if (phase_a) {
    if (lane == 0) job = (int)atomicAdd(PC(job_counter) + (kJobHeads + head) * kJobHeadStride, 1u);
    const unsigned int unit = (unsigned int)__builtin_amdgcn_readfirstlane(job) * kJobHeads + (unsigned int)head;
    if (unit >= n_heavy) { phase_a = false; continue; }
    job = (int)PC(heavy_prev)[unit];
    if (job < 0 || job >= PC(njobs)) continue;
  } else {
    if (chunk_left > 0) {
      job = next_job; next_job += kJobHeads; --chunk_left; listed >>= 1;
    } else {
      if (lane == 0) job = (int)atomicAdd(PC(job_counter) + head * kJobHeadStride, (unsigned int)chunk);
      job = __builtin_amdgcn_readfirstlane(job) * kJobHeads + head;
      next_job = job + kJobHeads; chunk_left = chunk - 1;
      listed = 0u;
      if (n_heavy != 0u) {
        const int jl = job + lane * kJobHeads;
        listed = (unsigned int)ballot(lane <= chunk_left && jl < PC(njobs) && PC(heavy_flags)[jl] == PC(heavy_gen));
      }
      const int left = PC(njobs) - next_job;
      chunk = left > 2 * per_wave ? kChunk : (left > per_wave ? 2 : 1);
    }
    if (job >= PC(njobs)) {
      chunk_left = 0;
      const unsigned int at = lane < kJobHeads ? __hip_atomic_load(PC(job_counter) + lane * kJobHeadStride, __ATOMIC_RELAXED, __HIP_MEMORY_SCOPE_AGENT) : 0u;
      const unsigned long long avail = ballot(lane < kJobHeads && (long long)at * kJobHeads + lane < (long long)PC(njobs));
      if (avail == 0ull) break;
      const unsigned long long above = avail & ~((2ull << head) - 1ull);
      head = __builtin_ctzll(above != 0ull ? above : avail);
      continue;
    }
    if ((listed & 1u) != 0u) continue;
  }
  RT_STAMP(prof, 7)
  if (timeline && lane == 0) tls[1] += 1ull;
  const unsigned long long job_t0 = lpt ? __builtin_amdgcn_s_memtime() : 0ull;
  const int jrow = (int)div_magic((uint32_t)job, PC(nseg_magic));
  const int mid = (PC(owned_rows) + 1) >> 1;
  const int lr = (jrow & 1) ? mid + (jrow >> 1) : mid - 1 - (jrow >> 1);
  const int JP = BIGAA ? jt / chunks : jt * PT;
  const int x0 = (job - jrow * PC(nseg)) * JP;
  const int y = band_global_row_cold(P, lr);
  f3 outc = mk(0.f, 0.f, 0.f);
  constexpr bool MASKS = !(SS > 0 && SS < 32) && (STRIDE != 0 || BIGAA || COUNT);
  constexpr int kJkValid = 1, kJkSph = 2, kJkBlocked = 4;
  int jk_flags = 0;
  bool jk_valid = false, jk_sph = false, jk_blocked = false;
  f3 jk_D0 = mk(0.f, 0.f, 0.f);
  float jk_ed = 0.0f;
  unsigned long long jk_K = 0ull;
  using kh_t = typename std::conditional<STRIDE == 32, uint32_t, unsigned long long>::type;
  kh_t jk_Kh = (kh_t)0;
  int jk_h = -1;
  unsigned long long Kp_job = n == 64 ? ~0ull : ((1ull << n) - 1ull);
  bool sph_job = P.nsph > 0;
  constexpr bool SEED = CULL && !COUNT && !PROF && MASKS && STRIDE == 32 && AA_X == 4 && AA_Y == 2 && SS == 64 && !MULTI && !BIGAA;
  bool seeded = false;
  if (SEED && PC(seed) != nullptr) {
    const int trow = (int)div_magic((uint32_t)y, PC(seed_rows_magic));
    const int ti = __builtin_amdgcn_readfirstlane(trow * PC(nseg) + (job - jrow * PC(nseg)));
    typedef const __attribute__((address_space(4))) SeedRec* SeedPtr;
    const SeedPtr rec = (SeedPtr)(unsigned long long)(PC(seed) + ti);
    const uint32_t sf = rec->flags;
    if ((sf & kSeedPrimaryWide) != 0u) { Kp_job = rec->Kp; sph_job = (sf & kSeedPrimarySph) != 0u; seeded = true; }
    if ((sf & kSeedShadowWide) != 0u) {
      jk_D0 = mk(rec->D0[0], rec->D0[1], rec->D0[2]); jk_ed = rec->ed;
      jk_K = rec->K; jk_Kh = (kh_t)rec->Kh; jk_h = rec->h;
    }
    static_assert((kSeedShadowWide >> kSeedShadowShift) == kJkValid && (kSeedShadowSph >> kSeedShadowShift) == kJkSph &&
                  (kSeedShadowBlocked >> kSeedShadowShift) == kJkBlocked, "jk_flags is a shift and a mask of the record's flags");
    jk_flags = (int)((sf >> kSeedShadowShift) & 7u);
  }
  if (CULL && !(SEED && seeded)) {
    const int lnJ = opaque(lane);
    const float Xlo = (float)(x0 * aa_x) - P.half_wx;
    const float Ylo = ((float)(y * aa_y) - P.half_hy) * sy;
    const f3 wc = mk(Xlo + PC(job_hx), Ylo + PC(job_hy), P.focal);
    const f3 duc = mk(P.rot[0] * wc.x + P.rot[1] * wc.y + P.rzf[0], P.rot[4] * wc.x + P.rot[5] * wc.y + P.rzf[1],
                      P.rot[8] * wc.x + P.rot[9] * wc.y + P.rzf[2]);
    const f3 eu = mk(PC(job_eu[0]), PC(job_eu[1]), PC(job_eu[2]));
    const float dumax = fmaxf(fmaxf(fabsf(duc.x) + eu.x, fabsf(duc.y) + eu.y), fabsf(duc.z) + eu.z);
    const int ti = lnJ < n ? lnJ : 0;
    const float4 c4 = S.c[ti];
    const bool clear = primary_clear(duc, eu, dumax, xyz(c4), c4.w, xyz(S.pc[ti]), xyz(S.qc[ti]));
    if (dumax < 1e30f) Kp_job &= ~ballot(clear);
    if (P.nsph > 0 && dumax < 1e30f)
      sph_job = ballot(sphere_bundle_maybe(P, lane, mk(P.cam[0], P.cam[1], P.cam[2]), 0.0f, duc, bsqrt(dot3(duc, duc)),
                                           1.0001f * bsqrt(dot3(eu, eu)), false)) != 0ull;
  }
  RT_STAMP(prof, 0)
  for (int k = 0; k < jt; ++k) {
    const int lnA = opaque(lane);
    const int kp = BIGAA ? k / chunks : k;
    const int chunk = BIGAA ? k - kp * chunks : 0;
    const int pA = BIGAA ? 0 : ((AA_X && AA_Y) ? lnA / (AA_X * AA_Y ? AA_X * AA_Y : 1) : (lnA * P.aa_magic) >> 16);
    const int pj = kp * PT + pA;
    const int a = (lnA - pA * aa) + 64 * chunk;
    const int x = x0 + pj;
    const bool valid = x < P.W && pA < PT && (!BIGAA || a < aa_full);
    const int ay = AA_X ? a / (AA_X ? AA_X : 1) : (a * P.aax_magic) >> 16;
    Ray ray = primary_ray(P, x, y, a - ay * aa_x, ay, aa_x, aa_y, sy);
    bool lit = false, secondary = false;
    const unsigned long long Kp = uniform64(Kp_job);
    if (valid) {
      if (CULL) closest_hit_primary_masked(S, P, ray, Kp, sph_job);
      else closest_hit_primary<false>(S, P, ray, wk);
      if (ray.tri != -1) {
        if (ray.col.w <= 0.0f) { secondary = true; if (!CULL) lit = bounce_to_diffuse<false>(S, P, ray, wk); }
        else lit = true;
      }
    }
    if (CULL) {
      bool bouncing = secondary;
      for (int b = 0; b < P.bounces; ++b) {
        const bool act = bouncing && ray.col.w <= 0.0f;
        const unsigned long long actm = ballot(act);
        if (actm == 0ull) break;
        if (act) ray = (ray.col.w == 0.0f) ? reflect_ray(ray) : refract_ray(ray);
        unsigned long long Kb = n == 64 ? ~0ull : ((1ull << n) - 1ull);
        {
          const int lnK = opaque(lane);
          const BounceBundle bnd = bounce_bundle(act, ray.start, ray.dir);
          if (bnd.mode == 1) {
            const TriLane Tb = tri_lane(S.v0, S.e1, S.e2, S.c, lnK < n ? lnK : 0);
            Kb &= ~ballot(task_bound(Tb, bnd.s0, bnd.D0, bnd.es, bnd.ed, 2e-6f * bnd.dl, 0.0f, bnd.dl).clear);
          } else if (!bnd.finite) {
            Kb = 0ull;
          }
        }
        if (act) {
          closest_hit_masked(S, P, ray, Kb);
          if (ray.tri != -1 && ray.col.w > 0.0f) { lit = true; bouncing = false; }
        }
      }
    }
    RT_STAMP(prof, 1)
    const int lnB = opaque(lane);
    const LightSetup ls = light_setup(light, ray);
    const f3 dir = ls.dir, start = ls.start;
    const float radius_sq = ls.radius_sq, term = ls.term;

    const bool slit = lit && !(term == 0.0f);
    int unshadowed = NS;
    unsigned long long work = ballot(slit);
    const bool sum_needed = work != 0ull;
    using need_t = typename std::conditional<STRIDE == 32, uint32_t, unsigned long long>::type;
    unsigned long long K = tri_lanes, sphmask = P.nsph > 0 ? ~0ull : 0ull;
    need_t need = (need_t)~(need_t)0;
    if (CULL && work != 0ull) {
      const CullConsts cc = cull_consts(radius_sq, hbox, slit);
      const float dlen = cc.dlen, hh = cc.hh;
      const bool sane = cc.sane;
      bool task_blocked = false;
      SphereBound sb;
      sb.maybe = false; sb.all_blocked = false;
      bool task_sph = P.nsph > 0;
      {
        const bool all_sane = ballot(slit && !sane) == 0ull;
        bool reuse = false;
        if ((MASKS ? (jk_flags & kJkValid) != 0 : jk_valid) && all_sane) {
          const f3 dj = dir - jk_D0;
          reuse = MASKS ? all_within(work, norm_inf(dj), jk_ed) : wave_max_pos(slit ? norm_inf(dj) : 0.0f) <= jk_ed;
        }
        int h = -1;
        unsigned long long Kh = 0ull;
        if (reuse) {
          K = jk_K; Kh = (unsigned long long)jk_Kh; h = jk_h;
          task_sph = MASKS ? (jk_flags & kJkSph) != 0 : jk_sph; task_blocked = MASKS ? (jk_flags & kJkBlocked) != 0 : jk_blocked;
        } else {
        const int jr = 63 - __builtin_clzll(work);
        const f3 s0 = mk(rl(start.x, jr), rl(start.y, jr), rl(start.z, jr));
        const f3 D0 = mk(rl(dir.x, jr), rl(dir.y, jr), rl(dir.z, jr));
        const f3 dd = dir - D0;
        const float ed_task = wave_max_pos(slit ? norm_inf(dd) : 0.0f);
        const float left = (float)(jt - 1 - k);
        const float ed = ed_task * (left > 0.0f ? fminf(PC(l1_inflate), left + 0.5f) : 1.0f);
        const float dlen0 = rl(dlen, jr);
        const float dlen_max = (dlen0 + 1.7321f * ed) * 1.000001f;
        const float dlen_min = fmaxf(dlen0 - 1.7321f * ed, 0.0f) * 0.999999f;
        const float es = 1.0002f * ed + 2e-6f * (P.light_inf + dlen_max);
        jk_flags = 0; jk_valid = false;
        if (all_sane && es < 1e30f && ed < 1e30f) {
          const float hh_task = 1.002f * hbox + 2e-6f * (dlen_max + hbox);
          if (P.nsph > 0)
            task_sph = ballot(sphere_bundle_maybe(P, lane, s0, es, D0, dlen0, 1.7321f * (1.001f * ed + hh_task), true)) != 0ull;
          const TriLane T1 = tri_lane(SC.v0, SC.e1, SC.e2, SC.c, lnB < ns ? lnB : 0);
          const Bound tb = light_bundle_bound(T1, light, s0, es, D0, ed, hh_task, dlen_min, dlen_max, P.light_inf + dlen_max + norm1(T1.v0));
          K = tri_lanes & ~ballot(tb.clear);
          task_blocked = (tri_lanes & ballot(tb.all_blocked)) != 0ull;
          h = __builtin_amdgcn_readlane(ray.tri, jr);
          Kh = K;
          if (left < 2.0f || aa < 8) h = -1;
          if (h >= 0) {
            __builtin_amdgcn_sched_barrier(0);
            const int lnH = opaque(lane);
            const float4 kc = SC.c[lnH < ns ? lnH : 0];
            TriLane Tk;
            Tk.v0 = xyz(SC.v0[lnH < ns ? lnH : 0]); Tk.c = xyz(kc); Tk.c1 = kc.w;
            const f3 hv0 = xyz(S.v0[h]), he1 = xyz(S.e1[h]), he2 = xyz(S.e2[h]);
            const float Mh = norm_inf(hv0) + norm_inf(he1) + norm_inf(he2);
            Kh = K & ~ballot(plane_slab_tneg(Tk, hv0, he1, he2, D0, ed, hh_task, Mh + P.light_inf + dlen_max + norm1(Tk.v0)));
          }
          jk_Kh = (kh_t)Kh; jk_h = h;
          jk_D0 = D0; jk_ed = uniform(ed * 0.9999f); jk_K = K;
          if (MASKS) jk_flags = kJkValid | (task_sph ? kJkSph : 0) | (task_blocked ? kJkBlocked : 0);
          else { jk_valid = true; jk_sph = task_sph; jk_blocked = task_blocked; }
        }
        }
        if (h >= 0 && ballot(slit && ray.tri != h) == 0ull) K = Kh;
      }
      if (task_sph && !task_blocked && sane) sb = spheres_point(P, start, dir, dlen, hh);
      sphmask = ballot(slit && P.nsph > 0 && (sb.maybe || !sane));
      const bool sph_blocked = sane && sb.all_blocked;
      RT_STAMP(prof, 2)
      if (task_blocked) {
        unshadowed = 0; work = 0ull;
        if (COUNT) xw.v[5] += 1;
      } else {

        bool blocked = sph_blocked;
        need = (need_t)0;
        int pos = 0;
        for (unsigned long long kk = K; kk != 0ull; kk &= kk - 1ull, ++pos) {
          const int kq = __builtin_ctzll(kk);
          const float4 c4_ = SC.c[kq];
          const f3 c_ = xyz(c4_);
          const float nA0_ = detc(start - xyz(SC.v0[kq]), c_), D0_ = detc(-dir, c_), Dl_ = hh * c4_.w;
          const bool tneg = sane && ((D0_ - Dl_ > 0.0f && nA0_ < -1e-18f) || (D0_ + Dl_ < 0.0f && nA0_ > 1e-18f));
          if (ballot(slit && !tneg) == 0ull) continue;
          const Bound pb = point_bound_c1<true>(start, dir, hh, dlen, cc.dminlen, cc.dk, xyz(SC.v0[kq]), xyz(SC.e1[kq]), xyz(SC.e2[kq]),
                                       c_, c4_.w, slit && !tneg && !blocked);
          if (!pb.clear || !sane) need |= (need_t)((need_t)1 << pos);
          blocked = blocked || (sane && pb.all_blocked);
        }
        if (blocked) unshadowed = 0;
        work = ballot(slit && !blocked && (need != (need_t)0 || ((sphmask >> lnB) & 1ull) != 0ull));
        if (COUNT) { xw.v[4] += (unsigned)__popcll(ballot(slit && !blocked && need == (need_t)0)); if (work == 0ull) xw.v[5] += 1; }
      }
    }

    RT_STAMP(prof, 3)
    const int lnC = opaque(lane);
    if (work != 0ull) {
      __builtin_amdgcn_wave_barrier();
      L.h0[lnC] = make_float4(start.x, start.y, start.z, radius_sq);
      L.h1[lnC] = make_float4(dir.x, dir.y, dir.z, 0.f);
      __builtin_amdgcn_wave_barrier();
    }
    const int GL = GP * aa;
    for (int g = 0; g * GP < PT && work != 0ull; ++g) {
      const unsigned long long gm = (work >> (g * GL)) & (GL == 64 ? ~0ull : ((1ull << GL) - 1ull));
      if (gm == 0ull) continue;
      for (int pass = 0; pass < n_pass; ++pass) {
      const int first_s = pass << 6;
      const int cnt_s = NS - first_s < 64 ? NS - first_s : 64;
      const unsigned long long act = (!MULTI || cnt_s == 64) ? active : ((1ull << cnt_s) - 1ull);
      const int q3 = lnC / 3, comp = lnC - 3 * q3;
      const int seg = (q3 * gp_magic) >> 16, pp = q3 - seg * GP;
      if (seg < kRngSegs) {
        uint32_t* dst = L.rng + pp * kRngStride + comp;
        const uint32_t s = (!MULTI || pass == 0) ? rng_seed(pixel_global_id(P, x0 + kp * PT + g * GP + pp, y), comp)
                                                 : dst[63 * 4];
        rng_fill_segment(dst, s, seg, cnt_s);
      }
      wave_lds_sync();
      RT_STAMP(prof, 4)
      if (CULL && !COUNT && !MULTI && ((SS > 0 && SS <= 32) || (SS == 0 && STRIDE == 32 && !BIGAA && NS <= 16))) {
        constexpr int SP = (SS > 16) ? 32 : 16, PK = 64 / SP;
        const unsigned long long aam = aa == 64 ? ~0ull : ((1ull << aa) - 1ull);
        unsigned long long rest = gm;
        while (rest != 0ull) {
          unsigned long long pmv[2] = {0ull, 0ull};
          int basev[2] = {0, 0}, ppv[2] = {0, 0};
#pragma unroll
          for (int inst = 0; inst < 2; ++inst) {
            if (rest == 0ull) break;
            const int b0 = __builtin_ctzll(rest);
            const int pp = (b0 * (aa == 1 ? 65536 : P.aa_magic)) >> 16;
            unsigned long long pm = (rest >> (pp * aa)) & aam, take = 0ull;
            for (int i = 0; i < PK && pm != 0ull; ++i) { take |= pm & (0ull - pm); pm &= pm - 1ull; }
            pmv[inst] = take; basev[inst] = g * GL + pp * aa; ppv[inst] = pp;
            rest &= ~(take << (pp * aa));
          }
          wave_unshadowed_packed<SP>(P, SC, L, lnC, pmv[0], basev[0], L.rng + ppv[0] * kRngStride, pmv[1], basev[1],
                                     L.rng + ppv[1] * kRngStride, K, (unsigned long long)need, sphmask, NS, unshadowed);
        }
      } else
      for (int pp = 0; pp < GP; ++pp) {
        unsigned long long pm = (gm >> (pp * aa)) & (aa == 64 ? ~0ull : ((1ull << aa) - 1ull));
        if (pm == 0ull) continue;
        const uint32_t* src = L.rng + pp * kRngStride + lnC * 4;
        const f3 jit = mk(crush1(src[0], P.spread), crush1(src[1], P.spread), crush1(src[2], P.spread));
        const int base = g * GL + pp * aa;
        while (pm != 0ull) {
          const int j = base + __builtin_ctzll(pm);
          pm &= pm - 1ull;
          if (CULL) {
            const int j2 = pm != 0ull ? base + __builtin_ctzll(pm) : j;
            pm &= pm - 1ull;
            unsigned long long n1, n2;
            if (STRIDE == 32) {
              n1 = (unsigned)__builtin_amdgcn_readlane((int)(uint32_t)need, j);
              n2 = (unsigned)__builtin_amdgcn_readlane((int)(uint32_t)need, j2);
            } else {
              const unsigned long long nd64 = (unsigned long long)need;
              n1 = ((unsigned long long)(unsigned)__builtin_amdgcn_readlane((int)(nd64 >> 32), j) << 32) | (unsigned)__builtin_amdgcn_readlane((int)nd64, j);
              n2 = ((unsigned long long)(unsigned)__builtin_amdgcn_readlane((int)(nd64 >> 32), j2) << 32) | (unsigned)__builtin_amdgcn_readlane((int)nd64, j2);
            }
            const Count2 c2 = wave_unshadowed_pair<COUNT>(P, SC, L, lnC, j, j2, K, n1 | n2, (sphmask >> j) & 1ull,
                                                          (sphmask >> j2) & 1ull, jit, act, xw);
            const int before = (MULTI && pass > 0) ? unshadowed : 0;
            if (lnC == j2) unshadowed = before + c2.b;
            if (lnC == j) unshadowed = before + c2.a;
          } else {
            const int cnt = wave_unshadowed_all<COUNT>(P, T, L, lnC, ns, j, jit, act, xw);
            if (lnC == j) unshadowed = (MULTI && pass > 0 ? unshadowed : 0) + cnt;
          }
        }
      }
      if (MULTI) __builtin_amdgcn_wave_barrier();
      }
      __builtin_amdgcn_wave_barrier();
      RT_STAMP(prof, 5)
    }
    RT_STAMP(prof, 5)

    const int lnD = opaque(lane);
    if (COUNT) {
      xw.v[6] += (unsigned)__popcll(work & ballot(lit && unshadowed == NS));
      xw.v[7] += (unsigned)__popcll(work & ballot(lit && unshadowed == 0));
    }
    const f3 contrib = shade<(SS <= 64 ? SS : 0)>(lit, secondary, unshadowed, NS, term, inv_S, ray.col, sum_needed);
    if (BIGAA) {
      if (chunk == 0) aa_run = mk(0.f, 0.f, 0.f);
#pragma unroll 8
      for (int r = 0; r < 64; ++r) aa_run = aa_run + mk(rl(contrib.x, r), rl(contrib.y, r), rl(contrib.z, r));
      if (chunk == chunks - 1 && lnD == kp) outc = aa_run;
    } else {
    const f3 acc = aa_sum(contrib, aa, ((AA_X && AA_Y) ? lnD / (AA_X * AA_Y ? AA_X * AA_Y : 1) : (lnD * P.aa_magic) >> 16) * aa);
      {
        const int rel = lnD - k * PT;
        const int srcl = (rel >= 0 && rel < PT) ? rel * aa : 0;
        const f3 v = mk(shfl(acc.x, srcl), shfl(acc.y, srcl), shfl(acc.z, srcl));
        if (rel >= 0 && rel < PT) outc = v;
      }
    }
    RT_STAMP(prof, 6)
  }
  const int x = x0 + lane;
  if (!COUNT && !PROF && (BIGAA ? lane < JP : lane < jt * PT) && x < P.W) {
    const f3 c = pixel_colour(outc, aa_full, inv_aa);
    const size_t o = (size_t)(PC(out_global) ? y : lr) * P.W + x;
    PC(out_argb)[o] = pack_argb(c);
    if (PC(out_rgb)) PC(out_rgb)[o] = make_float4(c.x, c.y, c.z, 1.0f);
  }
  if (lpt) {
    const unsigned long long cost = __builtin_amdgcn_s_memtime() - job_t0;
    if (lane == 0) { cost_acc[0] += cost; cost_acc[1] += (unsigned long long)jt; }
    if (cost > heavy_thr * (unsigned long long)jt && lane < (PC(heavy_dilate) ? 3 : 1)) {
      const int jn = job + (lane == 1 ? -1 : (lane == 2 ? 1 : 0));
      const int col = jn - jrow * PC(nseg);
      if (col >= 0 && col < PC(nseg)) {
        const unsigned int was = atomicMax(PC(heavy_flags_new) + jn, PC(heavy_gen) + 1u);
        if (was < PC(heavy_gen) + 1u) {
          const unsigned int at = atomicAdd(PC(heavy_new_state), 1u);
          if (at < (unsigned int)PC(heavy_cap)) PC(heavy_new)[at] = (unsigned int)jn;
          else atomicExch(PC(heavy_flags_new) + jn, was);
        }
      }
    }
  }
  }
  if (lpt && lane == 0) {
    atomicAdd(reinterpret_cast<unsigned long long*>(PC(heavy_new_state) + 2), cost_acc[0]);
    atomicAdd(PC(heavy_new_state) + 4, (unsigned int)cost_acc[1]);
  }
  if (timeline && lane == 0) {
    const unsigned long long t1 = __builtin_amdgcn_s_memrealtime(), t0 = tls[0];
    unsigned long long* const rec = PC(counters) + 3 * (size_t)(blockIdx.x * kWavesPerBlock + wave);
    rec[0] = t0; rec[1] = t1; rec[2] = tls[1] | ((unsigned long long)n_heavy << 32);
  }
  if (PROF) {
    if (lane == 0) for (int q = 0; q < 8; ++q) atomicAdd(&PC(counters)[q], prof[q]);
    return;
  }
  if (COUNT) {
    if (lane == 0) for (int q = 0; q < 8; ++q) if (xw.v[q]) atomicAdd(&PC(counters)[q], xw.v[q]);
  }
}

template __global__ void rt_draw_wave<false, false>(const FrameParams);
template __global__ void rt_draw_wave<true, false>(const FrameParams);
template __global__ void rt_draw_wave<false, true>(const FrameParams);
template __global__ void rt_draw_wave<true, true>(const FrameParams);
template __global__ void rt_draw_wave<true, false, true>(const FrameParams);
template __global__ void rt_draw_wave<true, false, false, 32>(const FrameParams);
template __global__ void rt_draw_wave<true, false, false, 0, true>(const FrameParams);
template __global__ void rt_draw_wave<true, false, false, 32, false, 4, 2, 64>(const FrameParams);
template __global__ void rt_draw_wave<true, false, false, 32, false, 2, 2, 64>(const FrameParams);
template __global__ void rt_draw_wave<true, false, false, 32, false, 2, 2, 16>(const FrameParams);
template __global__ void rt_draw_wave<true, false, false, 32, false, 2, 2, 10>(const FrameParams);
template __global__ void rt_draw_wave<false, false, false, 0, true>(const FrameParams);
template __global__ void rt_draw_wave<true, false, false, 0, false, 0, 0, 0, true>(const FrameParams);

__global__ __launch_bounds__(64 * kWavesPerBlock) void rt_wave_seed(const FrameParams P) {
  extern __shared__ float4 lds_dyn[];
  float4* const lds = lds_dyn;
  const int tid = threadIdx.x;
  const int wave = __builtin_amdgcn_readfirstlane(tid >> 6), lane = tid & 63;
  const int n = P.n, ns = P.n_shadow;
  stage_triangles(P, lds, tid, 64 * kWavesPerBlock, n);
  stage_spheres(P, tid);
  int* sidx = reinterpret_cast<int*>(lds + kLdsRecords * n);
  if (wave == 0) {
    const bool casts = (lane < n) && (P.colors[lane < n ? lane : 0].w != -1.0f);
    const unsigned long long m = ballot(casts);
    if (casts) sidx[__popcll(m & ((1ull << lane) - 1ull))] = lane;
  }
  __syncthreads();
  float4* scbase = reinterpret_cast<float4*>(sidx + ((n + 3) & ~3));
  for (int kq = tid; kq < ns; kq += 64 * kWavesPerBlock) {
    const int ti = sidx[kq];
    scbase[kq] = lds[ti]; scbase[ns + kq] = lds[n + ti]; scbase[2 * ns + kq] = lds[2 * n + ti];
    const float4 c4 = lds[3 * n + ti];
    scbase[3 * ns + kq] = make_float4(c4.x, c4.y, c4.z, norm1(xyz(c4)));
  }
  __syncthreads();
  const ShadowCasters SC{scbase, scbase + ns, scbase + 2 * ns, scbase + 3 * ns};
  const LdsScene S = lds_scene(lds, n, n);
  const f3 light = mk(P.light[0], P.light[1], P.light[2]);
  const unsigned long long tri_lanes = ns == 64 ? ~0ull : ((1ull << ns) - 1ull);
  const int aa = P.aa_x * P.aa_y;
  const int JP = P.job_tasks * (64 / aa);
  const int R = P.seed_rows, nseg = P.nseg;
  const int tiles = P.seed_tile_rows * nseg;
  for (int t = (int)blockIdx.x * kWavesPerBlock + wave; t < tiles; t += (int)gridDim.x * kWavesPerBlock) {
    const int trow = t / nseg, col = t - trow * nseg;
    const int x0 = col * JP, y0 = trow * R;
    SeedRec rec;
    rec.D0[0] = rec.D0[1] = rec.D0[2] = 0.0f; rec.ed = 0.0f;
    rec.K = 0ull; rec.Kh = 0ull; rec.Kp = 0ull; rec.h = -1; rec.flags = 0u;
    rec.pad[0] = rec.pad[1] = rec.pad[2] = rec.pad[3] = 0u;
    bool mine = false;
    {
      const int yr = y0 + lane;
      const int q = yr / P.band_rows;
      const int lr = (q / P.band_count) * P.band_rows + (yr - q * P.band_rows);
      mine = lane < R && yr < P.H && q % P.band_count == P.band_index && lr < P.owned_rows;
    }
    if (ballot(mine) != 0ull) {
      const float Xlo = (float)(x0 * P.aa_x) - P.half_wx;
      const float Ylo = ((float)(y0 * P.aa_y) - P.half_hy) * P.sy;
      const f3 wc = mk(Xlo + P.job_hx, Ylo + P.seed_hy, P.focal);
      const f3 duc = mk(P.rot[0] * wc.x + P.rot[1] * wc.y + P.rzf[0], P.rot[4] * wc.x + P.rot[5] * wc.y + P.rzf[1],
                        P.rot[8] * wc.x + P.rot[9] * wc.y + P.rzf[2]);
      const f3 eu = mk(P.seed_eu[0], P.seed_eu[1], P.seed_eu[2]);
      const float dumax = fmaxf(fmaxf(fabsf(duc.x) + eu.x, fabsf(duc.y) + eu.y), fabsf(duc.z) + eu.z);
      const int ti = lane < n ? lane : 0;
      const float4 c4 = S.c[ti];
      const bool clear = primary_clear(duc, eu, dumax, xyz(c4), c4.w, xyz(S.pc[ti]), xyz(S.qc[ti]));
      const unsigned long long Kp = (n == 64 ? ~0ull : ((1ull << n) - 1ull)) & ~ballot(clear);
      bool sph = P.nsph > 0;
      if (P.nsph > 0 && dumax < 1e30f)
        sph = ballot(sphere_bundle_maybe(P, lane, mk(P.cam[0], P.cam[1], P.cam[2]), 0.0f, duc, bsqrt(dot3(duc, duc)),
                                         1.0001f * bsqrt(dot3(eu, eu)), false)) != 0ull;
      const int nkp = __popcll(Kp);
      if (dumax < 1e30f) {
        const bool strict = nkp == 1 && !sph;
        if (nkp <= P.seed_kp_cap) {
          rec.Kp = Kp;
          rec.flags = kSeedPrimaryWide | (sph ? kSeedPrimarySph : 0u) | (strict ? kSeedPrimary : 0u);
        }
        const int cx = lane < 4 ? ((lane & 1) ? x0 + JP - 1 : x0) : x0 + (JP >> 1);
        const int cy = lane < 4 ? ((lane & 2) ? y0 + R - 1 : y0) : y0 + (R >> 1);
        const int cdx = (lane < 4 && (lane & 1)) ? P.aa_x - 1 : 0, cdy = (lane < 4 && (lane & 2)) ? P.aa_y - 1 : 0;
        Ray ray = primary_ray(P, cx, cy, cdx, cdy, P.aa_x, P.aa_y, P.sy);
        const f3 rd = ray.dir;
        closest_hit_primary_masked(S, P, ray, Kp, sph);
        const int jr = 4;
        const int hc_tri = __builtin_amdgcn_readlane(ray.tri, jr);
        const int h = nkp == 1 ? __builtin_ctzll(Kp) : hc_tri;
        if (h >= 0 && h < n) {
        const LightSetup ls = light_setup(light, ray);
        const bool slit = ray.tri == h && ray.col.w > 0.0f && !(ls.term == 0.0f);
        const CullConsts cc = cull_consts(ls.radius_sq, P.hbox, slit);
        const f3 s0 = mk(rl(ls.start.x, jr), rl(ls.start.y, jr), rl(ls.start.z, jr));
        const f3 D0 = mk(rl(ls.dir.x, jr), rl(ls.dir.y, jr), rl(ls.dir.z, jr));
        const float dlen0 = rl(cc.dlen, jr);
        const bool sane0 = ((ballot(cc.sane) >> jr) & 1ull) != 0ull;
        const float4 hc = S.c[h];
        const float tc = hc.w / detc(-rd, xyz(hc));
        const f3 Xc = mk(P.cam[0], P.cam[1], P.cam[2]) + tc * rd;
        const float dev = norm_inf((light - Xc) - D0);
        const bool corner_ok = tc > 0.0f && dev < 1e30f;
        const bool corners = (ballot(!corner_ok) & 0xfull) == 0ull;
        const float ed = 1.05f * wave_max_pos(lane < 4 && corner_ok ? dev : 0.0f) + 1e-5f * (P.light_inf + dlen0);
        if (sane0 && corners && ed < 1e30f) {
          const Level1 l1 = level1_bundle(P, S, SC, lane, ns, tri_lanes, light, P.hbox, s0, D0, ed, dlen0, h);
          const bool nothing = l1.Kh == 0ull && !l1.sph && !l1.blocked;
          const bool keep = l1.blocked || (__popcll(l1.Kh) <= P.seed_caster_cap && (!l1.sph || P.seed_keep_sph != 0));
          if (l1.ok && keep) {
            rec.D0[0] = D0.x; rec.D0[1] = D0.y; rec.D0[2] = D0.z;
            rec.ed = uniform(ed * 0.9999f);
            rec.K = l1.K; rec.Kh = l1.Kh; rec.h = h;
            rec.flags |= kSeedShadowWide | (l1.sph ? kSeedShadowSph : 0u) | (l1.blocked ? kSeedShadowBlocked : 0u) |
                         (strict && nothing ? kSeedShadow : 0u);
          }
        }
        }
      }
    }
    if (lane == 0) P.seed[t] = rec;
  }
}

bool wave_takes_seed(const FrameParams& P, bool cull) {
  return cull && P.n <= 32 && !P.no_specialise && P.aa_x == 4 && P.aa_y == 2 && P.S == 64 && P.job_tasks == 8;
}

bool wave_kernel_supports(const FrameParams& P) {
  const int aa = P.aa_x * P.aa_y;
  return P.S >= 1 && P.S <= 4096 && aa >= 1 && (aa <= 64 || (aa <= 256 && P.S <= 64)) && P.n >= 1 && P.n <= 64 && P.n_shadow >= 1 &&
         P.spread >= 0.0f;
}

static size_t wave_kernel_lds(const FrameParams& P, bool cull) {
  return (size_t)P.n * kLdsRecords * sizeof(float4) + (size_t)((P.n + 3) & ~3) * sizeof(int) +
         (size_t)P.n_shadow * 4 * sizeof(float4) + kWavesPerBlock * (size_t)wave_lds_bytes(cull);
}

int wave_blocks_per_cu(bool leave_room) { return leave_room ? kMinWaves - 1 : kMinWaves; }

static dim3 wave_grid(const FrameParams& P) {
  const int resident = P.wave_blocks > 0 ? P.wave_blocks : 256 * kMinWaves;
  const int needed = (P.njobs + kWavesPerBlock - 1) / kWavesPerBlock;
  return dim3(needed < resident ? (needed > 0 ? needed : 1) : resident);
}

void launch_wave_prof(const FrameParams& P, hipStream_t stream) {
  hipMemsetAsync(P.job_counter, 0, 2 * kJobHeads * kJobHeadStride * sizeof(unsigned int), stream);
  hipLaunchKernelGGL((rt_draw_wave<true, false, true>), wave_grid(P), dim3(64 * kWavesPerBlock), wave_kernel_lds(P, true), stream, P);
}

void launch_wave(const FrameParams& P, bool cull, bool count, hipStream_t stream) {
  const dim3 block(64 * kWavesPerBlock);
  const dim3 grid = wave_grid(P);
  const size_t lds_bytes = wave_kernel_lds(P, cull);
  if (P.seed != nullptr && !count) {
    const int tiles = P.seed_tile_rows * P.nseg;
    const int want = (tiles + kWavesPerBlock - 1) / kWavesPerBlock;
    const int room = P.wave_blocks > 0 ? P.wave_blocks : 256 * kMinWaves;
    hipLaunchKernelGGL(rt_wave_seed, dim3(want < room ? (want > 0 ? want : 1) : room), block, wave_kernel_lds(P, true) , stream, P);
  }
  const size_t heads_bytes = 2 * kJobHeads * kJobHeadStride * sizeof(unsigned int), state_bytes = kJobHeadStride * sizeof(unsigned int);
  if (P.heavy_new != nullptr && !count) {
    const bool before = P.heavy_new_state < P.job_counter;
    hipMemsetAsync(before ? (void*)P.heavy_new_state : (void*)P.job_counter, 0, heads_bytes + state_bytes, stream);
  } else {
    hipMemsetAsync(P.job_counter, 0, heads_bytes, stream);
  }
  if (P.aa_x * P.aa_y > 64) {
    hipLaunchKernelGGL((rt_draw_wave<true, false, false, 0, false, 0, 0, 0, true>), grid, block, lds_bytes, stream, P);
  } else if (count) {
    if (cull) hipLaunchKernelGGL((rt_draw_wave<true, true>), grid, block, lds_bytes, stream, P);
    else hipLaunchKernelGGL((rt_draw_wave<false, true>), grid, block, lds_bytes, stream, P);
  } else if (P.S > 64) {
    if (cull) hipLaunchKernelGGL((rt_draw_wave<true, false, false, 0, true>), grid, block, lds_bytes, stream, P);
    else hipLaunchKernelGGL((rt_draw_wave<false, false, false, 0, true>), grid, block, lds_bytes, stream, P);
  } else {
    const bool spec = cull && P.n <= 32 && !P.no_specialise;
    if (spec && P.aa_x == 4 && P.aa_y == 2 && P.S == 64) hipLaunchKernelGGL((rt_draw_wave<true, false, false, 32, false, 4, 2, 64>), grid, block, 0, stream, P);
    else if (spec && P.aa_x == 2 && P.aa_y == 2 && P.S == 64) hipLaunchKernelGGL((rt_draw_wave<true, false, false, 32, false, 2, 2, 64>), grid, block, 0, stream, P);
    else if (spec && P.aa_x == 2 && P.aa_y == 2 && P.S == 16) hipLaunchKernelGGL((rt_draw_wave<true, false, false, 32, false, 2, 2, 16>), grid, block, 0, stream, P);
    else if (spec && P.aa_x == 2 && P.aa_y == 2 && P.S == 10) hipLaunchKernelGGL((rt_draw_wave<true, false, false, 32, false, 2, 2, 10>), grid, block, 0, stream, P);
    else if (cull && P.n <= 32) hipLaunchKernelGGL((rt_draw_wave<true, false, false, 32>), grid, block, 0, stream, P);
    else if (cull) hipLaunchKernelGGL((rt_draw_wave<true, false>), grid, block, lds_bytes, stream, P);
    else hipLaunchKernelGGL((rt_draw_wave<false, false>), grid, block, lds_bytes, stream, P);
  }
}

}
```

uob_raytracer_amd/csrc/rt_wave_common.h:

```cpp
#pragma once
#include "rt_trace.h"

namespace uobrt {
namespace {

constexpr int kRngPixels = 4;
constexpr int kRngStride = 64 * 4 + 4;

__device__ __forceinline__ float rl(float v, int lane) {
  return __int_as_float(__builtin_amdgcn_readlane(__float_as_int(v), lane));
}
__device__ __forceinline__ float shfl(float v, int lane) { return __shfl(v, lane, 64); }
__device__ __forceinline__ int opaque(int v) {
  asm volatile("" : "+v"(v));
  return v;
}
__device__ __forceinline__ unsigned long long ballot(bool p) { return __builtin_amdgcn_ballot_w64(p); }
__device__ __forceinline__ float norm1(f3 a) { return fabsf(a.x) + fabsf(a.y) + fabsf(a.z); }
__device__ __forceinline__ float bsqrt(float x) { return __builtin_amdgcn_sqrtf(x); }
__device__ __forceinline__ float norm_inf(f3 a) { return fmaxf(fmaxf(fabsf(a.x), fabsf(a.y)), fabsf(a.z)); }
__device__ __forceinline__ float max_abs3(float a, float b, float c) { return fmaxf(fmaxf(fabsf(a), fabsf(b)), fabsf(c)); }

typedef const __attribute__((address_space(4))) FrameParams* KernargParams;
__device__ __forceinline__ KernargParams cold(const FrameParams&) {
// ... 285 lines not shown
  return r;
}

__device__ __forceinline__ Bound light_bundle_bound(const TriLane& T, f3 light, f3 s0, float es, f3 D0, float ed, float hh,
                                                    float dlen_min, float dlen_max, float M) {
  const f3 Lv = light - T.v0;
  const float Linf = norm_inf(Lv);
  const f3 pL = bcof(Lv, T.e2), qL = bcof(T.e1, Lv);
  const f3 b0 = s0 - T.v0;
  const float binf = norm_inf(b0);
  const float eb = 1.001f * es + 2e-6f * (binf + es);
  const float pj = norm1(bcof(b0, T.e2)) + 2.002f * eb * T.e2_1;
  const float qj = norm1(bcof(T.e1, b0)) + 2.002f * eb * T.e1_1;
  const f3 md = -D0;
  const float A0 = bdetc(md, T.c), N1 = bdetc(md, pL), N2 = bdetc(md, qL);
  const float nA0 = bdetc(Lv, T.c) + 0.9999f * A0;
  const float ed1 = 1.001f * ed;
  const float Bmax = Linf + dlen_max;
  const float rnd = 8e-6f * dlen_max * (Bmax + M);
  const float E0 = (ed1 + 4e-6f * (M + Bmax)) * T.c1 * 1.0001f;
  const float EA = (ed1 + hh) * T.c1 * 1.0001f;
  const float E1 = (ed1 * norm1(pL) + hh * pj + rnd * T.e2_1) * 1.0001f;
  const float E2 = (ed1 * norm1(qL) + hh * qj + rnd * T.e1_1) * 1.0001f;
  const float aD = fabsf(A0), hiD = aD + EA, loD = aD - EA;
  const bool robust = aD > EA + 1e-30f;
  const float sg = copysignf(1.0f, A0);
  const float tn = sg * nA0, un = sg * N1, vn = sg * N2;
  const float dmin = fmaxf(dlen_min - 1.7321f * hh, 0.0f), dmax = dlen_max + 1.7321f * hh;
  const f3 g = T.e2 - T.e1;
  const float g1 = norm1(g);
  const f3 wL = bcof(Lv - T.e1, g);
  const float wj = norm1(bcof(b0 - T.e1, g)) + 2.002f * eb * g1;
  const float W0 = sg * bdetc(md, wL);
  const float EW = (ed1 * norm1(wL) + hh * wj + rnd * g1) * 1.0001f;
  const float slackW = 4e-6f * (dlen_max + hh) * ((pj + qj + T.c1) +
                                                  (norm1(Lv) + norm1(b0) + 3.0f * eb + T.e1_1) * (T.e1_1 + T.e2_1));
  const bool can_pos = (A0 + EA > 0.0f) && (nA0 + E0 > -1e-18f) && (N1 + E1 > -1e-18f) && (N2 + E2 > -1e-18f);
  const bool can_neg = (A0 - EA < 0.0f) && (nA0 - E0 < 1e-18f) && (N1 - E1 < 1e-18f) && (N2 - E2 < 1e-18f);
  const bool cR = (fabsf(nA0) - E0) * dmin > hiD * (dlen_max * 1.000004f);
  const bool cW = fabsf(N1 + N2) - (E1 + E2) > hiD * 1.000004f;
  const bool cU = (fabsf(N1) - E1 > hiD * 1.000004f) || (fabsf(N2) - E2 > hiD * 1.000004f);
  const bool cE = robust && (W0 - EW > slackW);
  Bound r;
  r.clear = (!can_pos && !can_neg) || cR || cW || cU || cE;
  r.all_blocked = robust && (tn - E0 > 1e-18f) && (un - E1 > 1e-18f) && (vn - E2 > 1e-18f) &&
                  (W0 + EW < -slackW) &&
                  ((fabsf(nA0) + E0) * dmax < loD * (dlen_min * 0.999996f));
  return r;
}

__device__ __forceinline__ bool plane_slab_tneg(const TriLane& T, f3 hv0, f3 he1, f3 he2, f3 D0, float ed, float hh, float M) {
  const float f0 = fabsf(bdetc(hv0 - T.v0, T.c));
  const float f1 = fabsf(bdetc((hv0 + he1) - T.v0, T.c));
  const float f2 = fabsf(bdetc((hv0 + he2) - T.v0, T.c));
  const float aD = fabsf(bdetc(D0, T.c));
  const float EA = (1.001f * ed + hh) * T.c1 * 1.0001f;
  const bool robust = aD > EA + 1e-30f;
  const float m = 1e-4f * (aD - EA) * 0.9999f - 4e-6f * M * T.c1;
  return robust && (m - 1.00001f * f0 > 1e-18f) && (m - 1.00001f * f1 > 1e-18f) && (m - 1.00001f * f2 > 1e-18f);
}

template <bool STAGED_C1>
__device__ __forceinline__ Bound point_bound_c1(f3 start, f3 dir, float hh, float dlen, float dminlen, float dk,
                                                f3 v0, f3 e1, f3 e2, f3 c, float c1_staged, bool live) {
  const f3 b = start - v0;
  const f3 p = cof(b, e2), q = cof(e1, b);
  const float nA0 = detc(b, c);
  const f3 md = -dir;
  const float D0 = bdetc(md, c), N1 = bdetc(md, p), N2 = bdetc(md, q);
  const float aD = fabsf(D0);
  const float c1 = STAGED_C1 ? c1_staged : norm1(c), p1 = norm1(p), q1 = norm1(q);
  const float Delta = hh * c1;
  const bool robust = aD > Delta + 1e-30f;
  const float sg = copysignf(1.0f, D0);
  const float tn = sg * nA0, un = sg * N1, vn = sg * N2;
  const float hp = hh * p1, hq = hh * q1;
  const float hiD = aD + Delta, loD = aD - Delta;
  const bool can_pos = (D0 + Delta > 0.0f) && (nA0 > -1e-18f) && (N1 + hp > -1e-18f) && (N2 + hq > -1e-18f);
  const bool can_neg = (D0 - Delta < 0.0f) && (nA0 < 1e-18f) && (N1 - hp < 1e-18f) && (N2 - hq < 1e-18f);
  const bool cR = fabsf(nA0) * dminlen > hiD * dk;
  const bool cW = fabsf(N1 + N2) - (hp + hq) > hiD * 1.000004f;
  const bool cU = (fabsf(N1) - hp > hiD * 1.000004f) || (fabsf(N2) - hq > hiD * 1.000004f);
  const bool cheap0 = (!can_pos && !can_neg) || cR || cW || cU;
  Bound r;
  r.clear = cheap0; r.all_blocked = false;
  if (__builtin_amdgcn_ballot_w64(live && !cheap0) == 0ull) return r;
  const f3 w = bcof(b - e1, e2 - e1);
  const float W0 = sg * bdetc(md, w), hw = hh * norm1(w);
  const float e1n = norm1(e1);
  const float slackW = 4e-6f * (dlen + hh) * ((p1 + q1 + c1) + (norm1(b) + e1n) * (e1n + norm1(e2)));
  const bool cE = robust && (W0 - hw > slackW);
  bool cC = false;
  const bool cheap = (!can_pos && !can_neg) || cR || cW || cE;
  if (__builtin_amdgcn_ballot_w64(live && robust && !cheap) != 0ull) {
    const f3 mu = sg * p, mv = sg * q, mw = -sg * w;
    const float fu0 = -un, fv0 = -vn, fw0 = W0;
    const float su = p1, sv = q1, sw = norm1(w) + p1 + q1 + c1;
    auto corner = [&](f3 mi, f3 mj, float fi0, float fj0, float si, float sj, float extra) {
      bool ok = false;
      const float mik[3] = {mi.x, mi.y, mi.z}, mjk[3] = {mj.x, mj.y, mj.z};
#pragma unroll
      for (int k = 0; k < 3; ++k) {
        const float al = fabsf(mjk[k]), be = fabsf(mik[k]);
        const bool opp = (mik[k] > 0.0f) != (mjk[k] > 0.0f) && al > 0.0f && be > 0.0f;
        const f3 m = al * mi + be * mj;
        const float mk[3] = {m.x, m.y, m.z};
        float rad = 0.0f;
#pragma unroll
        for (int j = 0; j < 3; ++j) if (j != k) rad += fabsf(mk[j]);
        const float F0 = al * fi0 + be * fj0;
        const float slack = 8e-6f * (dlen + hh) * (al * si + be * sj) + (al + be) * extra;
        ok = ok || (opp && F0 - hh * rad * 1.0001f > slack);
      }
      return ok;
    };
    const float exw = 4e-6f * (dlen + hh) * (norm1(b) + e1n) * (e1n + norm1(e2));
    const bool in_u = !(fu0 > 0.0f), in_w = !(fw0 > 0.0f);
    const f3 mi = in_u ? mv : mu, mj = in_w ? mv : mw;
    const float fi0 = in_u ? fv0 : fu0, fj0 = in_w ? fv0 : fw0, si = in_u ? sv : su, sj = in_w ? sv : sw;
    const bool wedge = fi0 > 0.0f && fj0 > 0.0f && !(in_u && in_w);
    cC = robust && wedge && corner(mi, mj, fi0, fj0, si, sj, in_w ? 0.0f : exw);
  }
  r.clear = cheap0 || cE || cC;
  r.all_blocked = robust && (tn > 1e-18f) && (un - hp > 1e-18f) && (vn - hq > 1e-18f) &&
                  (W0 + hw < -slackW) &&
                  (fabsf(nA0) * (dlen + 1.7321f * hh) < loD * (dlen * 0.999996f));
  return r;
}

__device__ __forceinline__ Bound point_bound(f3 start, f3 dir, float hh, float dlen, float dminlen, float dk,
                                             f3 v0, f3 e1, f3 e2, f3 c, bool live = true) {
  return point_bound_c1<false>(start, dir, hh, dlen, dminlen, dk, v0, e1, e2, c, 0.0f, live);
}

__device__ __forceinline__ bool primary_clear(f3 duc, f3 eu, float dumax, f3 c, float nA0cam, f3 pc, f3 qc) {
  const f3 md = -duc;
  const float Ac = bdetc(md, c), N1 = bdetc(md, pc), N2 = bdetc(md, qc);
  const float sl = 4e-6f * dumax;
  const float EA = eu.x * fabsf(c.x) + eu.y * fabsf(c.y) + eu.z * fabsf(c.z) + sl * norm1(c);
  const float E1 = eu.x * fabsf(pc.x) + eu.y * fabsf(pc.y) + eu.z * fabsf(pc.z) + sl * norm1(pc);
  const float E2 = eu.x * fabsf(qc.x) + eu.y * fabsf(qc.y) + eu.z * fabsf(qc.z) + sl * norm1(qc);
  const bool can_pos = (Ac + EA > 0.0f) && (nA0cam > -1e-18f) && (N1 + E1 > -1e-30f) && (N2 + E2 > -1e-30f);
  const bool can_neg = (Ac - EA < 0.0f) && (nA0cam < 1e-18f) && (N1 - E1 < 1e-30f) && (N2 - E2 < 1e-30f);
  const bool cW = fabsf(N1 + N2) - (E1 + E2) > (fabsf(Ac) + EA) * 1.000004f;
  const bool cU = (fabsf(N1) - E1 > (fabsf(Ac) + EA) * 1.000004f) || (fabsf(N2) - E2 > (fabsf(Ac) + EA) * 1.000004f);
  const f3 w = (pc + qc) - c;
  const float cn = norm1(c) + norm1(pc) + norm1(qc);
  const float W = copysignf(1.0f, Ac) * bdetc(md, w);
  const float EW = eu.x * fabsf(w.x) + eu.y * fabsf(w.y) + eu.z * fabsf(w.z) + 2.0f * sl * cn;
  const bool cE = (fabsf(Ac) > EA) && (W - EW > 0.0f);
  return (!can_pos && !can_neg) || cW || cU || cE;
}

static_assert(RT_MAX_SPHERES <= 64, "sphere_bundle_maybe: one lane per sphere");
__device__ __forceinline__ bool sphere_bundle_maybe(const FrameParams& P, int lane, f3 o, float eo, f3 dir, float dlen, float jm,
                                                    bool casters_only) {
  const float eo2 = 1.7321f * 1.001f * eo;
  const DevSphere& sp = RT_SPH(P, lane < P.nsph ? lane : 0);
  const f3 Lv = o - mk(sp.cx, sp.cy, sp.cz);
  const f3 cr = mk(Lv.y * dir.z - Lv.z * dir.y, Lv.z * dir.x - Lv.x * dir.z, Lv.x * dir.y - Lv.y * dir.x);
  const float crn = bsqrt(bdot3(cr, cr)), Ln = bsqrt(bdot3(Lv, Lv)), R = bsqrt(fmaxf(sp.r2, 0.0f));
  const bool near = (Ln + eo2 < 40.0f * R) && (sp.r2 > 0.0f);
  const bool miss = near && (crn - Ln * jm - eo2 * (dlen + jm) > R * (dlen + jm) * 1.002f);
  const float gap = Ln - eo2 - R;
  const bool beyond = casters_only && near && (dlen > 5.0f * jm) && (gap > 0.01f * (Ln + eo2)) && (gap * 0.995f > dlen + jm);
  return lane < P.nsph && !(casters_only && sp.col[3] == -1.0f) && !miss && !beyond;
}
struct SphereBound { bool maybe, all_blocked; };
__device__ __forceinline__ SphereBound spheres_point(const FrameParams& P, f3 start, f3 dir, float dlen, float hh) {
  SphereBound r;
  r.maybe = false; r.all_blocked = false;
  const float jm = 1.7321f * hh;
  for (int i = 0; i < P.nsph; ++i) {
    const DevSphere& sp = RT_SPH(P, i);
    if (sp.col[3] == -1.0f) continue;
    const f3 Lv = start - mk(sp.cx, sp.cy, sp.cz);
    const f3 cr = mk(Lv.y * dir.z - Lv.z * dir.y, Lv.z * dir.x - Lv.x * dir.z, Lv.x * dir.y - Lv.y * dir.x);
    const f3 cl = mk(cr.y * Lv.z - cr.z * Lv.y, cr.z * Lv.x - cr.x * Lv.z, cr.x * Lv.y - cr.y * Lv.x);
    const float crn = bsqrt(bdot3(cr, cr)), Ln2 = bdot3(Lv, Lv), Ln = bsqrt(Ln2), R = bsqrt(fmaxf(sp.r2, 0.0f));
    const bool near = (Ln < 40.0f * R) && (sp.r2 > 0.0f);
    const bool miss = near && (crn * crn - hh * norm1(cl) > R * (dlen + jm) * 1.002f * crn);
    const float gap = Ln - R;
    const bool beyond = near && (dlen > 5.0f * jm) && (gap > 0.01f * Ln) && (gap * 0.995f > dlen);
    const bool behind = near && (Ln2 > 1.001f * sp.r2) && (bdot3(dir, Lv) - hh * norm1(Lv) > 1e-5f * (dlen + jm) * Ln);
    r.maybe = r.maybe || !(miss || beyond || behind);
    const bool hit = near && (Ln2 > 1.001f * sp.r2) && (bdot3(dir, Lv) + hh * norm1(Lv) < 0.0f) && (Ln < 0.999f * dlen) &&
                     (crn + Ln * jm < 0.99f * R * (dlen - jm)) && (dlen > jm);
    r.all_blocked = r.all_blocked || hit;
  }
  return r;
}

#pragma clang fp contract(off)

struct ShadowCasters { const float4 *v0, *e1, *e2, *c; };

struct Level1 {
  unsigned long long K, Kh;
  bool sph, blocked, ok;
};
__device__ __forceinline__ Level1 level1_bundle(const FrameParams& P, const LdsScene& S, const ShadowCasters& SC, int lane, int ns,
                                                unsigned long long tri_lanes, f3 light, float hbox, f3 s0, f3 D0, float ed,
                                                float dlen0, int h) {
  Level1 r;
  r.K = tri_lanes; r.Kh = tri_lanes; r.sph = P.nsph > 0; r.blocked = false; r.ok = false;
  const float dlen_max = (dlen0 + 1.7321f * ed) * 1.000001f;
  const float dlen_min = fmaxf(dlen0 - 1.7321f * ed, 0.0f) * 0.999999f;
  const float es = 1.0002f * ed + 2e-6f * (P.light_inf + dlen_max);
  if (es < 1e30f && ed < 1e30f) {
    const float hh_task = 1.002f * hbox + 2e-6f * (dlen_max + hbox);
    if (P.nsph > 0)
      r.sph = ballot(sphere_bundle_maybe(P, lane, s0, es, D0, dlen0, 1.7321f * (1.001f * ed + hh_task), true)) != 0ull;
    const TriLane T1 = tri_lane(SC.v0, SC.e1, SC.e2, SC.c, lane < ns ? lane : 0);
    const Bound tb = light_bundle_bound(T1, light, s0, es, D0, ed, hh_task, dlen_min, dlen_max, P.light_inf + dlen_max + norm1(T1.v0));
    r.K = tri_lanes & ~ballot(tb.clear);
    r.blocked = (tri_lanes & ballot(tb.all_blocked)) != 0ull;
    r.Kh = r.K;
    if (h >= 0) {
      TriLane Tk;
      Tk.v0 = T1.v0; Tk.c = T1.c; Tk.c1 = T1.c1;
      const f3 hv0 = xyz(S.v0[h]), he1 = xyz(S.e1[h]), he2 = xyz(S.e2[h]);
      const float Mh = norm_inf(hv0) + norm_inf(he1) + norm_inf(he2);
      r.Kh = r.K & ~ballot(plane_slab_tneg(Tk, hv0, he1, he2, D0, ed, hh_task, Mh + P.light_inf + dlen_max + norm1(Tk.v0)));
    }
    r.ok = true;
  }
  return r;
}

}
}
```

uob_raytracer_amd/runtime.py:

```python
import ctypes as C
import os

import numpy as np

try:
    import torch as _torch
except ImportError:
    _torch = None

from . import abi

_HERE = os.path.dirname(os.path.abspath(__file__))
LIB_PATH = os.environ.get("UOB_RT_LIB", os.path.join(_HERE, "libuob_rt.so"))

EXPORTS = (
    "rt_abi_version", "rt_last_error", "rt_config_default", "rt_config_owned_rows", "rt_init", "rt_render",
    "rt_render_device", "rt_count_work", "rt_count_executed", "rt_last_kernel_ms", "rt_destroy", "rt_scene_cornell_box",
    "rt_scene_load_obj", "rt_scene_load_obj_ex", "rt_triangle_compute_normal", "rt_scene_pack", "rt_rotation_matrix",
    "rt_selftest_rcp", "rt_selftest_normalize", "rt_selftest_shade", "rt_selftest_all_within", "rt_debug_trace_rays", "rt_debug_block_costs", "rt_debug_world_masks", "rt_debug_wave_timeline", "rt_debug_wave_seeds", "rt_debug_wave_seeds_wide", "rt_register_output", "rt_unregister_output",
    "rt_debug_band_copy_plan", "rt_update_scene", "rt_update_scene_device", "rt_debug_tile_data",
    "rt_trace_rays", "rt_trace_rays_device", "rt_debug_trace_stats",
    "rt_render_aov", "rt_render_aov_device", "rt_debug_aov_stats",
    "rt_shade_points", "rt_shade_points_device", "rt_debug_shade_stats",
    "rt_radiance_rays", "rt_radiance_rays_device", "rt_debug_radiance_stats",
    "rt_replace_scene", "rt_replace_scene_device", "rt_update_spheres", "rt_debug_scene_capacity",
    "rt_scene_transform", "rt_set_objects", "rt_pose_objects", "rt_pose_objects_device", "rt_debug_object_count",
    "rt_debug_scene_data",
    "rt_scene_skin", "rt_set_skin", "rt_pose_skin", "rt_pose_skin_device", "rt_debug_skin_info",
    "rt_debug_live_device_objects",
    "rt_filter_params_default", "rt_filter_plane", "rt_filter_plane_device", "rt_debug_filter_stats", "rt_filter_plane_host",
    "rt_accumulate_params_default", "rt_accumulate_plane", "rt_accumulate_plane_device", "rt_debug_accumulate_stats",
    "rt_accumulate_plane_host",
)

LIVE_OBJECT_KEYS = ("allocations", "bytes", "events", "streams")

TRACE_STATS_KEYS = ("rays", "waves", "tiles", "bundle_tiles", "tested_tiles", "triangle_tests", "unculled_rays", "reserved")
AOV_STATS_KEYS = ("samples", "waves", "tiles", "mask_tiles", "tested_tiles", "triangle_tests", "reserved6", "reserved7")

SHADE_STATS_KEYS = ("points", "sample_rays", "waves", "tiles", "bundle_tiles", "tested_tiles", "triangle_tests", "skipped_points")

RADIANCE_STATS_KEYS = ("rays", "bounce_rays", "shaded_points", "sample_rays", "closest_tested_tiles", "closest_triangle_tests",
                       "shadow_triangle_tests", "unculled_rays")

FILTER_STATS_KEYS = ("pixels", "passes", "accepted_taps", "valid_pixels", "kept", "reserved5", "reserved6", "reserved7")

ACCUMULATE_STATS_KEYS = ("pixels", "valid_pixels", "found_history", "accepted_taps", "no_candidate", "reserved5", "reserved6",
                         "reserved7")

_lib = None


class RtError(RuntimeError):
    def __init__(self, code, msg):
        super().__init__("libuob_rt: error %d: %s" % (code, msg))
        self.code = code


SEED_DTYPE = np.dtype([("D0", "<f4", 3), ("ed", "<f4"), ("K", "<u8"), ("Kh", "<u8"), ("Kp", "<u8"), ("h", "<i4"), ("flags", "<u4"),
                       ("pad", "<u4", 4)])
SEED_PRIMARY, SEED_SHADOW = 1, 2
SEED_PRIMARY_WIDE, SEED_PRIMARY_SPH, SEED_SHADOW_WIDE, SEED_SHADOW_SPH, SEED_SHADOW_BLOCKED = 4, 8, 16, 32, 64
SEED_WIDE_KEYS = ("primary", "shadow", "casters", "sphere", "blocked")


def lib():
    global _lib
    if _lib is None:
        if not os.path.exists(LIB_PATH):
            raise ImportError("%s is missing: build it with `python -c 'import __graft_entry__ as g; g.build()'` "
                              "(there is no CPU fallback)" % LIB_PATH)
        L = C.CDLL(LIB_PATH)
        fp, vp = C.POINTER(C.c_float), C.c_void_p
        L.rt_last_error.restype = C.c_char_p
        L.rt_config_default.argtypes = [C.POINTER(abi.RtConfig)]
        L.rt_config_default.restype = None
        L.rt_config_owned_rows.argtypes = [C.POINTER(abi.RtConfig)]
        L.rt_init.argtypes = [C.POINTER(abi.RtConfig), fp, fp, fp, C.c_int32, C.POINTER(vp)]
        L.rt_update_scene.argtypes = [vp, fp, fp, fp, C.c_int32, C.c_uint32]
        L.rt_update_scene_device.argtypes = [vp, vp, vp, vp, C.c_int32, C.c_uint32, vp]
        L.rt_debug_tile_data.argtypes = [vp, C.POINTER(C.c_int32), fp, C.c_int32]
        L.rt_debug_scene_data.argtypes = [vp, fp, fp, fp, fp, fp, fp, C.POINTER(C.c_int32), fp, fp, C.c_int32]
        L.rt_replace_scene.argtypes = [vp, fp, fp, fp, C.c_int32, C.c_uint32]
        L.rt_replace_scene_device.argtypes = [vp, vp, vp, vp, C.c_int32, C.c_uint32, vp]
        L.rt_update_spheres.argtypes = [vp, C.POINTER(abi.RtSphere), C.c_int32]
        L.rt_debug_scene_capacity.argtypes = [vp, C.POINTER(C.c_int64)]
        L.rt_scene_transform.argtypes = [C.POINTER(abi.RtTriangle), C.c_int32, C.c_int32, C.c_int32, fp]
        L.rt_scene_transform.restype = None
        L.rt_set_objects.argtypes = [vp, C.POINTER(C.c_int32), C.POINTER(C.c_int32), C.c_int32]
        L.rt_pose_objects.argtypes = [vp, fp, C.c_uint32]
        L.rt_pose_objects_device.argtypes = [vp, vp, C.c_uint32, vp]
        L.rt_debug_object_count.argtypes = [vp, C.POINTER(C.c_int32)]
        L.rt_scene_skin.argtypes = [C.POINTER(abi.RtTriangle), C.c_int32, C.c_int32, C.c_int32, C.POINTER(C.c_uint16), fp, fp,
                                    C.c_int32]
        L.rt_scene_skin.restype = None
        L.rt_set_skin.argtypes = [vp, C.c_int32, C.c_int32, C.POINTER(C.c_uint16), fp, C.c_int32]
        L.rt_pose_skin.argtypes = [vp, fp, C.c_uint32]
        L.rt_pose_skin_device.argtypes = [vp, vp, C.c_uint32, vp]
        L.rt_debug_skin_info.argtypes = [vp, C.POINTER(C.c_int32), C.POINTER(C.c_int32), C.POINTER(C.c_int32)]
        L.rt_debug_live_device_objects.argtypes = [C.POINTER(C.c_int64)]
        L.rt_render.argtypes = [vp, fp, fp, fp, C.c_float, C.POINTER(C.c_uint32), fp]
        L.rt_render_device.argtypes = [vp, fp, fp, fp, C.c_float, vp, vp, vp]
        L.rt_count_work.argtypes = [vp, fp, fp, fp, C.c_float, C.POINTER(abi.RtWork)]
        L.rt_count_executed.argtypes = [vp, fp, fp, fp, C.c_float, C.POINTER(C.c_uint64)]
        L.rt_last_kernel_ms.argtypes = [vp, fp]
        L.rt_destroy.argtypes = [vp]
        L.rt_destroy.restype = None
        L.rt_scene_cornell_box.argtypes = [C.POINTER(abi.RtTriangle), C.c_int32]
        L.rt_scene_load_obj.argtypes = [C.c_char_p, C.POINTER(abi.RtTriangle), C.c_int32]
        L.rt_scene_load_obj_ex.argtypes = [C.c_char_p, fp, C.c_float, fp, C.POINTER(abi.RtTriangle), C.c_int32]
        L.rt_debug_trace_rays.argtypes = [vp, C.c_int32, fp, fp, C.c_int64, C.POINTER(C.c_int32), fp]
        L.rt_trace_rays.argtypes = [vp, C.c_int32, fp, fp, C.c_int64, C.POINTER(C.c_int32), fp]
        L.rt_trace_rays_device.argtypes = [vp, C.c_int32, vp, vp, C.c_int64, vp, vp, vp]
        L.rt_debug_trace_stats.argtypes = [vp, C.POINTER(C.c_uint64)]
        L.rt_render_aov.argtypes = [vp, fp, fp, C.c_float, C.c_int32, C.POINTER(abi.RtAovBuffers)]
        L.rt_render_aov_device.argtypes = [vp, fp, fp, C.c_float, C.c_int32, C.POINTER(abi.RtAovBuffers), vp]
        L.rt_debug_aov_stats.argtypes = [vp, C.POINTER(C.c_uint64)]
        L.rt_shade_points.argtypes = [vp, fp, C.POINTER(C.c_int32), C.c_int64, fp, fp, C.POINTER(C.c_int32)]
        L.rt_shade_points_device.argtypes = [vp, vp, vp, C.c_int64, fp, vp, vp, vp]
        L.rt_debug_shade_stats.argtypes = [vp, C.POINTER(C.c_uint64)]
        L.rt_radiance_rays.argtypes = [vp, fp, C.POINTER(C.c_int32), C.c_int64, fp, fp, C.POINTER(C.c_int32)]
        L.rt_radiance_rays_device.argtypes = [vp, vp, vp, C.c_int64, fp, vp, vp, vp]
        L.rt_debug_radiance_stats.argtypes = [vp, C.POINTER(C.c_uint64)]
        L.rt_filter_params_default.argtypes = [C.POINTER(abi.RtFilterParams), C.c_int32, C.c_int32]
        L.rt_filter_params_default.restype = None
        L.rt_filter_plane.argtypes = [vp, C.POINTER(abi.RtFilterParams), fp, fp, fp, fp]
        L.rt_filter_plane_device.argtypes = [vp, C.POINTER(abi.RtFilterParams), vp, vp, vp, vp, vp]
        L.rt_debug_filter_stats.argtypes = [vp, C.POINTER(C.c_uint64)]
        L.rt_filter_plane_host.argtypes = [C.POINTER(abi.RtFilterParams), fp, fp, fp, fp]
        ap, ip = C.POINTER(abi.RtAccumulateParams), C.POINTER(C.c_int32)
        L.rt_accumulate_params_default.argtypes = [ap, C.c_int32, C.c_int32]
        L.rt_accumulate_params_default.restype = None
        L.rt_accumulate_plane.argtypes = [vp, ap, fp, fp, fp, ip, fp, fp, fp, fp]
        L.rt_accumulate_plane_device.argtypes = [vp, ap] + [vp] * 9
        L.rt_debug_accumulate_stats.argtypes = [vp, C.POINTER(C.c_uint64)]
        L.rt_accumulate_plane_host.argtypes = [ap, fp, fp, fp, ip, fp, fp, fp, fp]
        L.rt_debug_block_costs.argtypes = [vp, C.POINTER(C.c_uint32), C.c_int32]
        L.rt_debug_world_masks.argtypes = [vp, C.POINTER(C.c_uint64), C.c_int64, C.POINTER(C.c_int32), C.POINTER(C.c_int32)]
        L.rt_debug_wave_timeline.argtypes = [vp, C.POINTER(C.c_uint64)]
        L.rt_debug_band_copy_plan.argtypes = [C.c_int32] * 9 + [C.POINTER(abi.RtBandCopy), C.c_int32]
        L.rt_register_output.argtypes = [vp, vp, C.c_size_t]
        L.rt_unregister_output.argtypes = [vp]
        L.rt_triangle_compute_normal.argtypes = [C.POINTER(abi.RtTriangle)]
        L.rt_triangle_compute_normal.restype = None
        L.rt_scene_pack.argtypes = [C.POINTER(abi.RtTriangle), C.c_int32, fp, fp, fp]
        L.rt_scene_pack.restype = None
        L.rt_rotation_matrix.argtypes = [C.c_float, C.c_float, fp]
        L.rt_rotation_matrix.restype = None
        if L.rt_abi_version() != abi.RT_ABI_VERSION:
            raise ImportError("libuob_rt.so ABI %d != binding %d" % (L.rt_abi_version(), abi.RT_ABI_VERSION))
        _lib = L
    return _lib


def _check(rc):
    if rc < 0:
        raise RtError(rc, lib().rt_last_error().decode(errors="replace"))
    return rc


def _fp(a):
    return a.ctypes.data_as(C.POINTER(C.c_float))


def _need(name, t, dtype, shape, dev):
    if not isinstance(t, _torch.Tensor):
        raise TypeError("%s must be a torch tensor" % name)
    if t.dtype != dtype or t.device != dev or tuple(t.shape) != shape or not t.is_contiguous():
        raise ValueError("%s must be a contiguous %s tensor of shape %s on %s (got %s %s on %s)"
                         % (name, dtype, shape, dev, t.dtype, tuple(t.shape), t.device))


def _seeds_ptr(seeds, k, what):
    if seeds is None:
        return None
    seeds = np.ascontiguousarray(seeds, np.int32).reshape(-1)
    if seeds.shape[0] != k:
        raise ValueError("seeds must have one entry per %s" % what)
    return seeds.ctypes.data_as(C.POINTER(C.c_int32))


def band_copy_plan(num_devices, k, device_band_rows, width, height, elem_bytes, dev_to_dev, peer_ok, same_device):
    n = _check(lib().rt_debug_band_copy_plan(num_devices, k, device_band_rows, width, height, elem_bytes, int(dev_to_dev),
                                             int(peer_ok), int(same_device), None, 0))
    buf = (abi.RtBandCopy * max(n, 1))()
    _check(lib().rt_debug_band_copy_plan(num_devices, k, device_band_rows, width, height, elem_bytes, int(dev_to_dev),
                                         int(peer_ok), int(same_device), buf, n))
    return [{f: int(getattr(buf[i], f)) for f, _ in abi.RtBandCopy._fields_ if f != "reserved"} for i in range(n)]


def live_device_objects():
    out = (C.c_int64 * 4)()
    _check(lib().rt_debug_live_device_objects(out))
    return {key: int(out[i]) for i, key in enumerate(LIVE_OBJECT_KEYS)}


def selftest_rcp():
    out = (C.c_uint64 * 64)()
    _check(lib().rt_selftest_rcp(out))
    v = list(out)
    return {"safe_mismatch_1step": v[0], "safe_mismatch_2step": v[1], "edge_mismatch_1step": v[2],
            "edge_mismatch_2step": v[3], "examples": [int(b) & 0xFFFFFFFF for b in v[8:8 + min(v[4], 56)]]}


def selftest_normalize(b_stride=64):
    out = (C.c_uint64 * 8)()
    _check(lib().rt_selftest_normalize(out, C.c_uint32(b_stride)))
    v = list(out)
    return {"sqrt_mismatches": v[0], "div_mismatches": v[1], "div_pairs": v[2], "sqrt_example": v[3], "div_example": v[4]}


def selftest_shade(ns, lit, secondary, unshadowed, term, col, straight_line=False):
    ns = np.ascontiguousarray(ns, np.int32).reshape(-1)
    w = ns.shape[0]
    ints = [np.ascontiguousarray(a, np.int32).reshape(w, 64) for a in (lit, secondary, unshadowed)]
    term = np.ascontiguousarray(term, np.float32).reshape(w, 64)
# ... 712 lines not shown
        raw = self._raw_stream(stream, dev)
        ptr = lambda t: C.c_void_p(t.data_ptr() if t is not None else 0)
        _check(lib().rt_accumulate_plane_device(self._h, C.byref(p), ptr(value), ptr(position4), ptr(normal4), ptr(prim), ptr(prev),
                                                ptr(next), ptr(out_mean), ptr(out_variance), C.c_void_p(raw)))
        return next, out_mean, out_variance

    def accumulate_stats(self):
        return self._stats("rt_debug_accumulate_stats", ACCUMULATE_STATS_KEYS)

    def reset_history(self):
        self._history = None

    def render_accumulated_light(self, rot, cam, light, focal, sample=0, filter=False, want_parts=False, **params):
        import math
        import torch
        aa = self.cfg.aa_x * self.cfg.aa_y
        if sample is None or isinstance(sample, bool) or int(sample) != sample or not 0 <= int(sample) < aa:
            raise ValueError("sample must be one AA sample index in [0, %d)" % aa)
        if max(self.cfg.band_count, 1) != 1:
            raise ValueError("render_accumulated_light: a context of row bands does not hold neighbouring rows")
        if self.cfg.width * self.cfg.height > abi.RT_SHADE_SEED_MAX:
            raise ValueError("render_accumulated_light: %d x %d pixels exceed the seed domain of 2^24 ids" % (self.cfg.width, self.cfg.height))
        dev = self._torch_device()
        shape = (self.rows, self.width)
        count = shape[0] * shape[1]
        if self._history is None:
            hist = [torch.empty(shape + (abi.HISTORY_WORDS,), dtype=torch.float32, device=dev) for _ in range(2)]
            self._history = [hist, 0, None, 0]
        hist, cur, view, frame = self._history
        planes = {"prim": torch.empty(shape, dtype=torch.int32, device=dev),
                  "position": torch.empty(shape + (4,), dtype=torch.float32, device=dev),
                  "normal": torch.empty(shape + (4,), dtype=torch.float32, device=dev)}
        self.render_aov_device(rot, cam, focal, sample=sample, out=planes)
        pos, nrm = planes["position"], planes["normal"]
        seeds = ((torch.arange(count, dtype=torch.int64, device=dev) + frame * count) % abi.RT_SHADE_SEED_MAX).to(torch.int32)
        p6 = torch.cat([pos[..., :3], nrm[..., :3]], -1).reshape(-1, 6).contiguous()
        _, counts = self.shade_points_device(p6, light, seeds=seeds, want_counts=True)
        hit = planes["prim"] != -1
        zero = torch.zeros(shape, dtype=torch.float32, device=dev)
        vis = torch.where(hit, counts.reshape(shape).to(torch.float32) / float(self.cfg.shadow_samples), zero)
        d = torch.tensor(np.ascontiguousarray(light, np.float32)[:3], device=dev) - pos[..., :3]
        r2 = (d * d).sum(-1)
        term = 16.0 * (d * nrm[..., :3]).sum(-1).clamp_min(0.0) / (4.0 * math.pi * r2)
        term = torch.where(hit, term, zero)
        if view is None:
            p, prev = accumulate_params(shape[1], shape[0], **params), None
        else:
            p, prev = accumulate_params(shape[1], shape[0], view[0], view[1], view[2], aa_x=self.cfg.aa_x, **params), hist[cur]
        nxt, vis_m, var = self.accumulate_plane_device(vis, pos, nrm, prim=planes["prim"], prev=prev, next=hist[1 - cur], params=p)
        r, c, _ = self._args(rot, cam, cam)
        self._history = [hist, 1 - cur, (r, c, float(focal)), frame + 1]
        vis_o = self.filter_plane_device(vis_m, pos, nrm) if filter else vis_m
        out = term * torch.where(hit, vis_o, zero)
        return (out, term, vis, vis_m, var, nxt[..., abi.HISTORY_COUNT].clone()) if want_parts else out

    def shade_stats(self):
        return self._stats("rt_debug_shade_stats", SHADE_STATS_KEYS)

    def radiance_rays(self, rays, light, seeds=None, want_prim=False):
        rays = np.ascontiguousarray(rays, np.float32).reshape(-1, 6)
        k = rays.shape[0]
        li = np.ascontiguousarray(light, np.float32)[:3].copy()
        sp = _seeds_ptr(seeds, k, "ray")
        out = np.zeros((k, 4), np.float32)
        prim = np.zeros(k, np.int32) if want_prim else None
        _check(lib().rt_radiance_rays(self._h, _fp(rays), sp, k, _fp(li), _fp(out),
                                      prim.ctypes.data_as(C.POINTER(C.c_int32)) if want_prim else None))
        return (out, prim) if want_prim else out

    def radiance_rays_device(self, rays6, light, seeds=None, out=None, out_prim=None, stream=None):
        import torch
        dev = self._torch_device()

        if not isinstance(rays6, torch.Tensor) or rays6.dim() != 2:
            raise ValueError("rays6 must be a torch tensor of shape [k, 6]")
        k = rays6.shape[0]
        _need("rays6", rays6, torch.float32, (k, 6), dev)
        if seeds is not None:
            _need("seeds", seeds, torch.int32, (k,), dev)
        if out is None:
            out = torch.empty((k, 4), dtype=torch.float32, device=dev)
        _need("out", out, torch.float32, (k, 4), dev)
        if out_prim is not None:
            _need("out_prim", out_prim, torch.int32, (k,), dev)
        li = np.ascontiguousarray(light, np.float32)[:3].copy()
        raw = self._raw_stream(stream, dev)
        if k:
            _check(lib().rt_radiance_rays_device(self._h, C.c_void_p(rays6.data_ptr()),
                                                 C.c_void_p(seeds.data_ptr() if seeds is not None else 0), k, _fp(li),
                                                 C.c_void_p(out.data_ptr()),
                                                 C.c_void_p(out_prim.data_ptr() if out_prim is not None else 0),
                                                 C.c_void_p(raw)))
        return out if out_prim is None else (out, out_prim)

    def radiance_stats(self):
        return self._stats("rt_debug_radiance_stats", RADIANCE_STATS_KEYS)

    def render_panorama(self, width, height, cam, light, yaw=0.0):
        import math
        import torch
        width, height = int(width), int(height)
        if width < 1 or height < 1:
            raise ValueError("width and height must be positive")
        dev = self._torch_device()
        f32 = dict(dtype=torch.float32, device=dev)
        xs = (torch.arange(width, **f32) + 0.5) * torch.tensor(2.0 * math.pi, **f32) / torch.tensor(float(width), **f32)
        phi = torch.tensor(float(yaw), **f32) + xs - torch.tensor(math.pi, **f32)
        theta = (torch.arange(height, **f32) + 0.5) * torch.tensor(math.pi, **f32) / torch.tensor(float(height), **f32) \
            - torch.tensor(math.pi / 2.0, **f32)
        ct = torch.cos(theta)[:, None]
        d = torch.stack([torch.sin(phi)[None, :] * ct, torch.sin(theta)[:, None].expand(height, width),
                         torch.cos(phi)[None, :] * ct], -1)
        start = torch.tensor(np.ascontiguousarray(cam, np.float32)[:3].copy(), device=dev).expand(height, width, 3)
        rays = torch.cat([start, d], -1).reshape(-1, 6).contiguous()
        seeds = (torch.arange(width * height, dtype=torch.int64, device=dev) & abi.RT_SHADE_SEED_MASK).to(torch.int32)
        return self.radiance_rays_device(rays, light, seeds=seeds).reshape(height, width, 4)

    def trace_stats(self):
        return self._stats("rt_debug_trace_stats", TRACE_STATS_KEYS)

    def wave_timeline(self):
        out = (C.c_uint64 * 8)()
        _check(lib().rt_debug_wave_timeline(self._h, out))
        n = max(int(out[0]), 1)
        first, last = int(out[1]), int(out[2])
        return {"waves": int(out[0]), "span_us": (last - first) / 100.0, "mean_start_us": (int(out[3]) / n - first) / 100.0,
                "mean_idle_tail_us": (last - int(out[4]) / n) / 100.0, "jobs": int(out[5]), "max_jobs_per_wave": int(out[6]), "listed_jobs": int(out[7])}

    def wave_seeds(self):
        fn = lib().rt_debug_wave_seeds
        fn.argtypes = [C.c_void_p, C.c_void_p, C.c_int64, C.POINTER(C.c_int32), C.POINTER(C.c_uint64)]
        dims, cnt = (C.c_int32 * 3)(), (C.c_uint64 * 4)()
        _check(fn(self._h, None, 0, dims, cnt))
        rec = np.zeros((int(dims[0]), int(dims[1])), SEED_DTYPE)
        if rec.size:
            _check(fn(self._h, rec.ctypes.data_as(C.c_void_p), rec.size, dims, cnt))
        return {"tile_rows": int(dims[0]), "tiles_per_row": int(dims[1]), "rows_per_tile": int(dims[2]),
                "tiles_primary": int(cnt[0]), "tiles_shadow": int(cnt[1]), "jobs_primary": int(cnt[2]), "jobs_shadow": int(cnt[3]),
                "records": rec}

    def wave_seeds_wide(self):
        fn = lib().rt_debug_wave_seeds_wide
        fn.argtypes = [C.c_void_p, C.c_void_p, C.c_int64, C.POINTER(C.c_int32), C.POINTER(C.c_uint64)]
        dims, cnt = (C.c_int32 * 3)(), (C.c_uint64 * 10)()
        _check(fn(self._h, None, 0, dims, cnt))
        rec = np.zeros((int(dims[0]), int(dims[1])), SEED_DTYPE)
        if rec.size:
            _check(fn(self._h, rec.ctypes.data_as(C.c_void_p), rec.size, dims, cnt))
        d = {"tile_rows": int(dims[0]), "tiles_per_row": int(dims[1]), "rows_per_tile": int(dims[2]), "records": rec}
        for q, k in enumerate(SEED_WIDE_KEYS):
            d["tiles_" + k], d["jobs_" + k] = int(cnt[2 * q]), int(cnt[2 * q + 1])
        return d

    def world_masks(self):
        g, w = C.c_int32(), C.c_int32()
        n = _check(lib().rt_debug_world_masks(self._h, None, 0, C.byref(g), C.byref(w)))
        out = np.zeros(n, np.uint64)
        _check(lib().rt_debug_world_masks(self._h, out.ctypes.data_as(C.POINTER(C.c_uint64)), n, C.byref(g), C.byref(w)))
        return out.reshape(g.value, g.value, g.value, w.value)

    def block_costs(self):
        n = _check(lib().rt_debug_block_costs(self._h, None, 0))
        out = np.zeros(n, np.uint32)
        _check(lib().rt_debug_block_costs(self._h, out.ctypes.data_as(C.POINTER(C.c_uint32)), n))
        return out.reshape((self.rows + 15) // 16, (self.width + 15) // 16)

    def last_kernel_ms(self):
        ms = C.c_float()
        _check(lib().rt_last_kernel_ms(self._h, C.byref(ms)))
        return float(ms.value)
```

Before: 4.414 million Mrays/s.

## Certify plain tiles in seed pass and shade them via a short direct path

The seed kernel now tries to prove, with conservative floating-point error bounds, that every primary ray in a tile hits one known diffuse triangle and that its shadow rays see nothing that can block them. It marks such tiles with a certificate. The main wave kernel then skips full traversal and bounce handling for certified jobs: it intersects the known triangle analytically and runs only light sampling. This adds seed-kernel work and a debug API that cross-checks certified tiles against the full path. Correctness depends on the error bounds being truly conservative.

```diff
diff --git a/include/uob_rt.h b/include/uob_rt.h
--- a/include/uob_rt.h
+++ b/include/uob_rt.h
@@ -215,6 +215,9 @@
 
 int rt_debug_wave_seeds_wide(rt_ctx* ctx, void* records, int64_t cap, int32_t dims[3], uint64_t counters[10]);
 
+int rt_debug_wave_plain(rt_ctx* ctx, const float rot[12], const float cam[3], const float light[3], float focal,
+                        int32_t* tile_h, int64_t cap, int32_t dims[3], uint64_t counters[8]);
+
 enum { RT_COPY_2D = 0,
        RT_COPY_PEER = 1,
        RT_COPY_LINEAR = 2    };
diff --git a/uob_raytracer_amd/csrc/rt_api.hip b/uob_raytracer_amd/csrc/rt_api.hip
--- a/uob_raytracer_amd/csrc/rt_api.hip
+++ b/uob_raytracer_amd/csrc/rt_api.hip
@@ -76,6 +76,7 @@
   if (const char* e = getenv("UOB_RT_SEED_KP")) { const int v = atoi(e); if (v >= 1 && v <= 64) t.seed_kp = v; }
   if (const char* e = getenv("UOB_RT_SEED_CASTERS")) { const int v = atoi(e); if (v >= 0 && v <= 64) t.seed_casters = v; }
   if (const char* e = getenv("UOB_RT_SEED_SPH")) t.seed_sph = atoi(e) != 0;
+  if (const char* e = getenv("UOB_RT_NO_PLAIN")) t.no_plain = atoi(e) != 0;
   if (const char* e = getenv("UOB_RT_FILTER_FORM")) t.filter_form = !strcmp(e, "direct") ? kFilterFormDirect : kFilterFormBuiltIn;
   return t;
 }
@@ -322,6 +323,23 @@
   if (tiled) use_tiled_scene(c, P);
 }
 
+static int use_seed_table(rt_ctx* c, FrameParams* P) {
+  const int R = c->tune.seed_rows;
+  const int tile_rows = (P->H + R - 1) / R;
+  const size_t tiles = (size_t)tile_rows * (size_t)P->nseg;
+  if (c->seed_cap < tiles) {
+    if (c->d_seed.alloc(tiles) != hipSuccess) return alloc_failed();
+    c->seed_cap = tiles;
+  }
+  P->seed = c->d_seed; P->seed_rows = R; P->seed_tile_rows = tile_rows; P->seed_rows_magic = div_magic_for(R);
+  P->seed_hy = 0.5f * (float)(R * P->aa_y - 1) * P->sy;
+  for (int k = 0; k < 3; ++k) P->seed_eu[k] = 1.0001f * (fabsf(P->rot[4 * k]) * P->job_hx + fabsf(P->rot[4 * k + 1]) * P->seed_hy);
+  P->seed_kp_cap = c->tune.seed_kp; P->seed_caster_cap = c->tune.seed_casters; P->seed_keep_sph = c->tune.seed_sph ? 1 : 0;
+  P->no_plain = c->tune.no_plain ? 1 : 0;
+  c->seed_tile_rows = tile_rows; c->seed_nseg = P->nseg; c->seed_rows = R;
+  return RT_OK;
+}
+
 static int launch_frame(rt_ctx* c, const float rot[12], const float cam[3], const float light[3], float focal,
                         uint32_t* d_argb, float4* d_rgb, hipStream_t stream, bool out_global = false) {
   if (!c || !rot || !cam || !light) { set_error("NULL argument"); return RT_E_INVALID; }
@@ -361,28 +379,19 @@
     if (c->tune.timeline) {
       const size_t waves = (size_t)P.wave_blocks * 4;
       if (!c->d_timeline) {
-        if (c->d_timeline.alloc(waves * 3) != hipSuccess) { set_error("hipMalloc failed (timeline)"); return RT_E_NOMEM; }
+        if (c->d_timeline.alloc(waves * 3 + 1) != hipSuccess) { set_error("hipMalloc failed (timeline)"); return RT_E_NOMEM; }
         c->timeline_waves = waves;
       }
       if (c->timeline_waves >= waves) {
-        HIP_TRY(hipMemsetAsync(c->d_timeline, 0, c->timeline_waves * 3 * sizeof(uint64_t), stream));
+        HIP_TRY(hipMemsetAsync(c->d_timeline, 0, (c->timeline_waves * 3 + 1) * sizeof(uint64_t), stream));
         P.counters = reinterpret_cast<unsigned long long*>(c->d_timeline.p);
         c->timeline_valid = true;
       }
     }
     if (!c->tune.no_seed && wave_takes_seed(P, !(c->cfg.flags & RT_FLAG_NO_CULL))) {
-      const int R = c->tune.seed_rows;
-      const int tile_rows = (P.H + R - 1) / R;
-      const size_t tiles = (size_t)tile_rows * (size_t)P.nseg;
-      if (c->seed_cap < tiles) {
-        if (c->d_seed.alloc(tiles) != hipSuccess) return alloc_failed();
-        c->seed_cap = tiles;
-      }
-      P.seed = c->d_seed; P.seed_rows = R; P.seed_tile_rows = tile_rows; P.seed_rows_magic = div_magic_for(R);
-      P.seed_hy = 0.5f * (float)(R * P.aa_y - 1) * P.sy;
-      for (int k = 0; k < 3; ++k) P.seed_eu[k] = 1.0001f * (fabsf(rot[4 * k]) * P.job_hx + fabsf(rot[4 * k + 1]) * P.seed_hy);
-      P.seed_kp_cap = c->tune.seed_kp; P.seed_caster_cap = c->tune.seed_casters; P.seed_keep_sph = c->tune.seed_sph ? 1 : 0;
-      c->seed_tile_rows = tile_rows; c->seed_nseg = P.nseg; c->seed_rows = R;
+      const int rc = use_seed_table(c, &P);
+      if (rc != RT_OK) return rc;
+      if (c->timeline_valid) P.plain_taken = reinterpret_cast<unsigned long long*>(c->d_timeline.p) + c->timeline_waves * 3;
     }
     launch_wave(P, !(c->cfg.flags & RT_FLAG_NO_CULL), false, stream);
   } else if (wave_paths && !(c->cfg.flags & RT_FLAG_NO_CULL) && mesh_kernel_supports(P)) {
@@ -738,6 +747,7 @@
   for (size_t t = 0; t < rec.size(); ++t) {
     SeedRec& r = rec[t];
     r.flags &= kSeedPrimary | kSeedShadow;
+    r.cert = 0u;
     if (!(r.flags & kSeedPrimary)) r.Kp = 0ull;
     if (!(r.flags & kSeedShadow)) { r.D0[0] = r.D0[1] = r.D0[2] = 0.0f; r.ed = 0.0f; r.K = 0ull; r.Kh = 0ull; r.h = -1; }
     const uint64_t n = rows[t / (size_t)c->seed_nseg];
@@ -767,7 +777,58 @@
     for (int q = 0; q < 5; ++q)
       if (is[q]) { counters[2 * q] += 1; counters[2 * q + 1] += n; }
   }
+  for (SeedRec& r : rec) r.cert = 0u;
   if (records) memcpy(records, rec.data(), (size_t)((int64_t)rec.size() < cap ? (int64_t)rec.size() : cap) * sizeof(SeedRec));
+  return RT_OK;
+}
+
+int rt_debug_wave_plain(rt_ctx* c, const float rot[12], const float cam[3], const float light[3], float focal,
+                        int32_t* tile_h, int64_t cap, int32_t dims[3], uint64_t counters[8]) {
+  if (!c || !rot || !cam || !light || !dims || !counters || cap < 0 || (cap > 0 && !tile_h)) { set_error("NULL argument"); return RT_E_INVALID; }
+  c = lead_ctx(c);
+  dims[0] = dims[1] = dims[2] = 0;
+  for (int q = 0; q < 8; ++q) counters[q] = 0;
+  if (c->owned_rows == 0) return RT_OK;
+  DeviceGuard guard;
+  HIP_TRY(hipSetDevice(c->device));
+  if (c->timed) HIP_TRY(hipEventSynchronize(c->ev1));
+  if (c->tune.timeline && c->timeline_valid && c->seed_tile_rows != 0) {
+    uint64_t taken = 0;
+    HIP_TRY(hipMemcpy(&taken, c->d_timeline.p + c->timeline_waves * 3, sizeof taken, hipMemcpyDeviceToHost));
+    counters[6] = taken; counters[7] = 1;
+  }
+  FrameParams P;
+  fill_params(c, rot, cam, light, focal, &P);
+  const bool cull = !(c->cfg.flags & RT_FLAG_NO_CULL);
+  if ((c->cfg.flags & RT_FLAG_GENERIC_KERNEL) || !wave_kernel_supports(P) || !wave_takes_seed(P, cull)) return RT_OK;
+  const int rc0 = use_seed_table(c, &P);
+  if (rc0 != RT_OK) return rc0;
+  DevMem<unsigned long long> d_check;
+  if (d_check.alloc(4) != hipSuccess) return alloc_failed();
+  P.counters = c->d_counters;
+  P.plain_check = d_check;
+  HIP_TRY(wait_aov(c, c->stream));
+  HIP_TRY(wait_scene(c, c->stream));
+  HIP_TRY(hipMemsetAsync(c->d_counters, 0, sizeof(rt_work), c->stream));
+  HIP_TRY(hipMemsetAsync(d_check, 0, 4 * sizeof(unsigned long long), c->stream));
+  launch_wave_seed(P, c->stream);
+  launch_wave(P, cull, true, c->stream);
+  HIP_TRY(hipGetLastError());
+  unsigned long long chk[4];
+  HIP_TRY(hipMemcpyAsync(chk, d_check, sizeof chk, hipMemcpyDeviceToHost, c->stream));
+  HIP_TRY(hipStreamSynchronize(c->stream));
+  std::vector<SeedRec> rec;
+  std::vector<uint64_t> rows;
+  const int rc = read_seed_table(c, &rec, &rows);
+  if (rc != RT_OK) return rc;
+  dims[0] = c->seed_tile_rows; dims[1] = c->seed_nseg; dims[2] = c->seed_rows;
+  for (size_t t = 0; t < rec.size(); ++t) {
+    const SeedRec& r = rec[t];
+    const bool plain = (r.cert & kCertPlain) != 0u;
+    if (plain) { counters[0] += 1; counters[1] += rows[t / (size_t)c->seed_nseg]; }
+    if ((int64_t)t < cap) tile_h[t] = plain ? r.h : -1 - (int32_t)((r.cert >> kCertFailShift) & 3u);
+  }
+  for (int q = 0; q < 4; ++q) counters[2 + q] = chk[q];
   return RT_OK;
 }
 
diff --git a/uob_raytracer_amd/csrc/rt_device.h b/uob_raytracer_amd/csrc/rt_device.h
--- a/uob_raytracer_amd/csrc/rt_device.h
+++ b/uob_raytracer_amd/csrc/rt_device.h
@@ -22,8 +22,11 @@
   unsigned long long K, Kh, Kp;
   int32_t h;
   uint32_t flags;
-  uint32_t pad[4];
+  uint32_t cert;
+  uint32_t pad[3];
 };
+constexpr uint32_t kCertTake = 1u, kCertPlain = 2u;
+constexpr int kCertFailShift = 8;
 constexpr uint32_t kSeedPrimary = 1u, kSeedShadow = 2u;
 constexpr uint32_t kSeedPrimaryWide = 4u, kSeedPrimarySph = 8u;
 constexpr int kSeedShadowShift = 4;
@@ -102,6 +105,9 @@
   float seed_hy;
   float seed_eu[3];
   int32_t seed_kp_cap, seed_caster_cap, seed_keep_sph;
+  int32_t no_plain;
+  unsigned long long* plain_check;
+  unsigned long long* plain_taken;
 };
 
 
diff --git a/uob_raytracer_amd/csrc/rt_host.h b/uob_raytracer_amd/csrc/rt_host.h
--- a/uob_raytracer_amd/csrc/rt_host.h
+++ b/uob_raytracer_amd/csrc/rt_host.h
@@ -37,6 +37,7 @@
                        float* d_out10, hipStream_t stream);
 void launch_wave(const FrameParams& P, bool cull, bool count, hipStream_t stream);
 void launch_wave_prof(const FrameParams& P, hipStream_t stream);
+void launch_wave_seed(const FrameParams& P, hipStream_t stream);
 bool wave_kernel_supports(const FrameParams& P);
 bool wave_takes_seed(const FrameParams& P, bool cull);
 int wave_blocks_per_cu(bool leave_room);
@@ -117,6 +118,7 @@
   int seed_kp = 64;
   int seed_casters = 32;
   bool seed_sph = true;
+  bool no_plain = false;
 };
 
 inline std::atomic<int64_t> g_live[4];
diff --git a/uob_raytracer_amd/csrc/rt_kernel_wave.hip b/uob_raytracer_amd/csrc/rt_kernel_wave.hip
--- a/uob_raytracer_amd/csrc/rt_kernel_wave.hip
+++ b/uob_raytracer_amd/csrc/rt_kernel_wave.hip
@@ -308,6 +308,7 @@
   RT_STAMP(prof, 0)
   Work wk, xw;
   if (COUNT) for (int q = 0; q < 8; ++q) xw.v[q] = 0;
+  unsigned long long pw[4] = {0ull, 0ull, 0ull, 0ull};
   int head = (int)((blockIdx.x * kWavesPerBlock + wave) % kJobHeads);
   const bool lpt = !COUNT && !PROF && PC(heavy_new) != nullptr;
   unsigned int n_heavy = 0u;
@@ -387,7 +388,8 @@
   unsigned long long Kp_job = n == 64 ? ~0ull : ((1ull << n) - 1ull);
   bool sph_job = P.nsph > 0;
   constexpr bool SEED = CULL && !COUNT && !PROF && MASKS && STRIDE == 32 && AA_X == 4 && AA_Y == 2 && SS == 64 && !MULTI && !BIGAA;
-  bool seeded = false;
+  bool seeded = false, plain_job = false;
+  int plain_h = 0;
   if (SEED && PC(seed) != nullptr) {
     const int trow = (int)div_magic((uint32_t)y, PC(seed_rows_magic));
     const int ti = __builtin_amdgcn_readfirstlane(trow * PC(nseg) + (job - jrow * PC(nseg)));
@@ -402,6 +404,7 @@
     static_assert((kSeedShadowWide >> kSeedShadowShift) == kJkValid && (kSeedShadowSph >> kSeedShadowShift) == kJkSph &&
                   (kSeedShadowBlocked >> kSeedShadowShift) == kJkBlocked, "jk_flags is a shift and a mask of the record's flags");
     jk_flags = (int)((sf >> kSeedShadowShift) & 7u);
+    if ((rec->cert & kCertTake) != 0u) { plain_job = true; plain_h = rec->h; }
   }
   if (CULL && !(SEED && seeded)) {
     const int lnJ = opaque(lane);
@@ -421,6 +424,41 @@
                                            1.0001f * bsqrt(dot3(eu, eu)), false)) != 0ull;
   }
   RT_STAMP(prof, 0)
+  int chk_h = -1;
+  if (COUNT && PC(plain_check) != nullptr && PC(seed) != nullptr) {
+    const int trow = (int)div_magic((uint32_t)y, PC(seed_rows_magic));
+    const int ti = __builtin_amdgcn_readfirstlane(trow * PC(nseg) + (job - jrow * PC(nseg)));
+    if ((PC(seed)[ti].cert & kCertPlain) != 0u) chk_h = PC(seed)[ti].h;
+  }
+  if (SEED && plain_job) {
+    const int hq = __builtin_amdgcn_readfirstlane(plain_h);
+    const float4 hc4 = S.c[hq], hcol = S.col[hq];
+    const f3 hpc = xyz(S.pc[hq]), hqc = xyz(S.qc[hq]), hv0 = xyz(S.v0[hq]), he1 = xyz(S.e1[hq]), he2 = xyz(S.e2[hq]);
+    Ray ray;
+    ray.N = xyz(S.nrm[hq]);
+    for (int k = 0; k < jt; ++k) {
+      const int lnA = opaque(lane);
+      const int pA = lnA / (AA_X * AA_Y ? AA_X * AA_Y : 1), a = lnA - pA * aa;
+      const int ay = a / (AA_X ? AA_X : 1);
+      const f3 d = primary_ray(P, x0 + k * PT + pA, y, a - ay * aa_x, ay, aa_x, aa_y, sy).dir;
+      const f3 nd = -d;
+      const float rr = rcp_exact(detc(nd, xyz(hc4)));
+      const float u = detc(nd, hpc) * rr, v = detc(nd, hqc) * rr;
+      ray.P = (hv0 + u * he1) + v * he2;
+      const LightSetup ls = light_setup(light, ray);
+      float total = 0.0f;
+      if (ballot(!(ls.term == 0.0f)) != 0ull) total = light_sum_full<(SS <= 64 ? SS : 0)>(NS, ls.term);
+      const float l = 0.5f + div_count(total, NS, inv_S);
+      const f3 contrib = mk(hcol.x * l, hcol.y * l, hcol.z * l);
+      const int lnD = opaque(lane);
+      const f3 acc = aa_sum(contrib, aa, (lnD / (AA_X * AA_Y ? AA_X * AA_Y : 1)) * aa);
+      const int rel = lnD - k * PT;
+      const int srcl = (rel >= 0 && rel < PT) ? rel * aa : 0;
+      const f3 pv = mk(shfl(acc.x, srcl), shfl(acc.y, srcl), shfl(acc.z, srcl));
+      if (rel >= 0 && rel < PT) outc = pv;
+    }
+    if (timeline && lane == 0 && PC(plain_taken) != nullptr) atomicAdd(PC(plain_taken), 1ull);
+  } else
   for (int k = 0; k < jt; ++k) {
     const int lnA = opaque(lane);
     const int kp = BIGAA ? k / chunks : k;
@@ -662,6 +700,12 @@
       xw.v[6] += (unsigned)__popcll(work & ballot(lit && unshadowed == NS));
       xw.v[7] += (unsigned)__popcll(work & ballot(lit && unshadowed == 0));
     }
+    if (COUNT && chk_h >= 0) {
+      pw[0] += (unsigned)__popcll(ballot(valid));
+      pw[1] += (unsigned)__popcll(ballot(valid && (!lit || secondary || ray.tri != chk_h)));
+      pw[2] += (unsigned)__popcll(ballot(valid && slit && unshadowed != NS));
+      pw[3] += (unsigned)__popcll(ballot(valid && lit && !(radius_sq > 1e-18f && radius_sq < 1e30f)));
+    }
     const f3 contrib = shade<(SS <= 64 ? SS : 0)>(lit, secondary, unshadowed, NS, term, inv_S, ray.col, sum_needed);
     if (BIGAA) {
       if (chunk == 0) aa_run = mk(0.f, 0.f, 0.f);
@@ -718,6 +762,7 @@
   }
   if (COUNT) {
     if (lane == 0) for (int q = 0; q < 8; ++q) if (xw.v[q]) atomicAdd(&PC(counters)[q], xw.v[q]);
+    if (lane == 0 && PC(plain_check) != nullptr) for (int q = 0; q < 4; ++q) if (pw[q]) atomicAdd(&PC(plain_check)[q], pw[q]);
   }
 }
 
@@ -772,7 +817,7 @@
     SeedRec rec;
     rec.D0[0] = rec.D0[1] = rec.D0[2] = 0.0f; rec.ed = 0.0f;
     rec.K = 0ull; rec.Kh = 0ull; rec.Kp = 0ull; rec.h = -1; rec.flags = 0u;
-    rec.pad[0] = rec.pad[1] = rec.pad[2] = rec.pad[3] = 0u;
+    rec.cert = 0u; rec.pad[0] = rec.pad[1] = rec.pad[2] = 0u;
     bool mine = false;
     {
       const int yr = y0 + lane;
@@ -838,6 +883,33 @@
             rec.flags |= kSeedShadowWide | (l1.sph ? kSeedShadowSph : 0u) | (l1.blocked ? kSeedShadowBlocked : 0u) |
                          (strict && nothing ? kSeedShadow : 0u);
           }
+          if (strict && nothing && l1.ok) {
+            const int hl = __builtin_amdgcn_readfirstlane(h);
+            const float4 hc4 = S.c[hl];
+            const AllHit ah = primary_all_hit(duc, eu, dumax, xyz(hc4), hc4.w, xyz(S.pc[hl]), xyz(S.qc[hl]));
+            const f3 hv0 = xyz(S.v0[hl]), he1 = xyz(S.e1[hl]), he2 = xyz(S.e2[hl]);
+            const float B = norm1(mk(P.cam[0], P.cam[1], P.cam[2]) - hv0), E = norm1(he1) + norm1(he2), c1 = norm1(xyz(hc4));
+            const float caminf = max_abs3(P.cam[0], P.cam[1], P.cam[2]);
+            const float T = 1.7323f * ah.tau * dumax;
+            const float err_a = 1.01f * ah.tau * (4e-6f * dumax) * (1.0f + 0.5774f * ah.G * c1);
+            const float err_b = 4e-6f * ah.G * ((B + E) * E + c1) * E + 1e-6f * (norm_inf(hv0) + E);
+            const float err_c = 4e-6f * ah.G * (B + T) * (c1 + E * E) + 1e-6f * (caminf + T);
+            const float err_l = 1e-6f * (P.light_inf + caminf + T + ed);
+            const float maxdev = wave_max_pos(lane < 4 && corner_ok ? dev : 0.0f);
+            const float ed_c = uniform(maxdev + (2.0f * err_a + err_b + err_c + err_l));
+            bool ed_ok = ed_c <= uniform(ed * 0.9999f);
+            if (!ed_ok && ed_c < 1e30f) {
+              const Level1 lc = level1_bundle(P, S, SC, lane, ns, tri_lanes, light, P.hbox, s0, D0, ed_c, dlen0, h);
+              ed_ok = lc.ok && lc.Kh == 0ull && !lc.sph && !lc.blocked;
+            }
+            const float edw = fmaxf(ed, ed_c);
+            const float dmin = dlen0 - 1.7321f * edw, dmax = dlen0 + 1.7321f * edw;
+            const bool sane_ok = dmin > 2e-9f && dmax < 5e14f;
+            const bool diffuse = S.col[hl].w > 0.0f;
+            const bool plain = ah.ok && diffuse && ed_ok && sane_ok;
+            rec.cert = plain ? (kCertPlain | (P.no_plain ? 0u : kCertTake))
+                             : (uint32_t)(!(ah.ok && diffuse) ? 1 : (!ed_ok ? 2 : 3)) << kCertFailShift;
+          }
         }
         }
       }
@@ -874,16 +946,18 @@
   hipLaunchKernelGGL((rt_draw_wave<true, false, true>), wave_grid(P), dim3(64 * kWavesPerBlock), wave_kernel_lds(P, true), stream, P);
 }
 
+void launch_wave_seed(const FrameParams& P, hipStream_t stream) {
+  const int tiles = P.seed_tile_rows * P.nseg;
+  const int want = (tiles + kWavesPerBlock - 1) / kWavesPerBlock;
+  const int room = P.wave_blocks > 0 ? P.wave_blocks : 256 * kMinWaves;
+  hipLaunchKernelGGL(rt_wave_seed, dim3(want < room ? (want > 0 ? want : 1) : room), dim3(64 * kWavesPerBlock), wave_kernel_lds(P, true) , stream, P);
+}
+
 void launch_wave(const FrameParams& P, bool cull, bool count, hipStream_t stream) {
   const dim3 block(64 * kWavesPerBlock);
   const dim3 grid = wave_grid(P);
   const size_t lds_bytes = wave_kernel_lds(P, cull);
-  if (P.seed != nullptr && !count) {
-    const int tiles = P.seed_tile_rows * P.nseg;
-    const int want = (tiles + kWavesPerBlock - 1) / kWavesPerBlock;
-    const int room = P.wave_blocks > 0 ? P.wave_blocks : 256 * kMinWaves;
-    hipLaunchKernelGGL(rt_wave_seed, dim3(want < room ? (want > 0 ? want : 1) : room), block, wave_kernel_lds(P, true) , stream, P);
-  }
+  if (P.seed != nullptr && !count) launch_wave_seed(P, stream);
   const size_t heads_bytes = 2 * kJobHeads * kJobHeadStride * sizeof(unsigned int), state_bytes = kJobHeadStride * sizeof(unsigned int);
   if (P.heavy_new != nullptr && !count) {
     const bool before = P.heavy_new_state < P.job_counter;
diff --git a/uob_raytracer_amd/csrc/rt_wave_common.h b/uob_raytracer_amd/csrc/rt_wave_common.h
--- a/uob_raytracer_amd/csrc/rt_wave_common.h
+++ b/uob_raytracer_amd/csrc/rt_wave_common.h
@@ -461,6 +461,29 @@
   return (!can_pos && !can_neg) || cW || cU || cE;
 }
 
+struct AllHit { bool ok; float G, tau; };
+__device__ __forceinline__ AllHit primary_all_hit(f3 duc, f3 eu, float dumax, f3 c, float nA0cam, f3 pc, f3 qc) {
+  const f3 md = -duc;
+  const float Ac = bdetc(md, c), N1 = bdetc(md, pc), N2 = bdetc(md, qc);
+  const float sl = 4e-6f * dumax;
+  const float EA = eu.x * fabsf(c.x) + eu.y * fabsf(c.y) + eu.z * fabsf(c.z) + sl * norm1(c);
+  const float E1 = eu.x * fabsf(pc.x) + eu.y * fabsf(pc.y) + eu.z * fabsf(pc.z) + sl * norm1(pc);
+  const float E2 = eu.x * fabsf(qc.x) + eu.y * fabsf(qc.y) + eu.z * fabsf(qc.z) + sl * norm1(qc);
+  const f3 w = (pc + qc) - c;
+  const float cn = norm1(c) + norm1(pc) + norm1(qc);
+  const float sg = copysignf(1.0f, Ac);
+  const float W = sg * bdetc(md, w);
+  const float EW = eu.x * fabsf(w.x) + eu.y * fabsf(w.y) + eu.z * fabsf(w.z) + 2.0f * sl * cn;
+  const float lo = fabsf(Ac) - EA, hi = fabsf(Ac) + EA;
+  AllHit r;
+  r.G = 1.7323f * dumax / lo;
+  r.tau = 1.0001f * fabsf(nA0cam) / lo;
+  r.ok = dumax < 1e30f && lo > 4e-30f * dumax && lo > 1e-30f && hi < 1e30f &&
+         sg * nA0cam > 1e-18f && r.tau * (1.7323f * dumax) < 1e30f &&
+         sg * N1 - E1 > 0.0f && sg * N2 - E2 > 0.0f && W + EW < -4e-6f * hi;
+  return r;
+}
+
 static_assert(RT_MAX_SPHERES <= 64, "sphere_bundle_maybe: one lane per sphere");
 __device__ __forceinline__ bool sphere_bundle_maybe(const FrameParams& P, int lane, f3 o, float eo, f3 dir, float dlen, float jm,
                                                     bool casters_only) {
diff --git a/uob_raytracer_amd/runtime.py b/uob_raytracer_amd/runtime.py
--- a/uob_raytracer_amd/runtime.py
+++ b/uob_raytracer_amd/runtime.py
@@ -17,7 +17,7 @@
     "rt_abi_version", "rt_last_error", "rt_config_default", "rt_config_owned_rows", "rt_init", "rt_render",
     "rt_render_device", "rt_count_work", "rt_count_executed", "rt_last_kernel_ms", "rt_destroy", "rt_scene_cornell_box",
     "rt_scene_load_obj", "rt_scene_load_obj_ex", "rt_triangle_compute_normal", "rt_scene_pack", "rt_rotation_matrix",
-    "rt_selftest_rcp", "rt_selftest_normalize", "rt_selftest_shade", "rt_selftest_all_within", "rt_debug_trace_rays", "rt_debug_block_costs", "rt_debug_world_masks", "rt_debug_wave_timeline", "rt_debug_wave_seeds", "rt_debug_wave_seeds_wide", "rt_register_output", "rt_unregister_output",
+    "rt_selftest_rcp", "rt_selftest_normalize", "rt_selftest_shade", "rt_selftest_all_within", "rt_debug_trace_rays", "rt_debug_block_costs", "rt_debug_world_masks", "rt_debug_wave_timeline", "rt_debug_wave_seeds", "rt_debug_wave_seeds_wide", "rt_debug_wave_plain", "rt_register_output", "rt_unregister_output",
     "rt_debug_band_copy_plan", "rt_update_scene", "rt_update_scene_device", "rt_debug_tile_data",
     "rt_trace_rays", "rt_trace_rays_device", "rt_debug_trace_stats",
     "rt_render_aov", "rt_render_aov_device", "rt_debug_aov_stats",
@@ -62,6 +62,9 @@
 SEED_PRIMARY, SEED_SHADOW = 1, 2
 SEED_PRIMARY_WIDE, SEED_PRIMARY_SPH, SEED_SHADOW_WIDE, SEED_SHADOW_SPH, SEED_SHADOW_BLOCKED = 4, 8, 16, 32, 64
 SEED_WIDE_KEYS = ("primary", "shadow", "casters", "sphere", "blocked")
+PLAIN_KEYS = ("tiles_plain", "jobs_plain", "lanes_checked", "lanes_off_h", "lanes_shadowed", "lanes_insane", "jobs_short_loop",
+              "jobs_short_loop_counted")
+PLAIN_NOT, PLAIN_FAILS_ALL_HIT, PLAIN_FAILS_ED, PLAIN_FAILS_SANE = -1, -2, -3, -4
 
 
 def lib():
@@ -1080,6 +1083,22 @@
             d["tiles_" + k], d["jobs_" + k] = int(cnt[2 * q]), int(cnt[2 * q + 1])
         return d
 
+    def wave_plain(self, rot, cam, light, focal):
+        rot, cam, light = self._args(rot, cam, light)
+        fn = lib().rt_debug_wave_plain
+        fn.argtypes = [C.c_void_p, C.POINTER(C.c_float), C.POINTER(C.c_float), C.POINTER(C.c_float), C.c_float,
+                       C.POINTER(C.c_int32), C.c_int64, C.POINTER(C.c_int32), C.POINTER(C.c_uint64)]
+        dims, cnt = (C.c_int32 * 3)(), (C.c_uint64 * 8)()
+        _check(fn(self._h, _fp(rot), _fp(cam), _fp(light), C.c_float(focal), None, 0, dims, cnt))
+        h = np.full((int(dims[0]), int(dims[1])), -1, np.int32)
+        if h.size:
+            _check(fn(self._h, _fp(rot), _fp(cam), _fp(light), C.c_float(focal), h.ctypes.data_as(C.POINTER(C.c_int32)), h.size,
+                      dims, cnt))
+        d = {"tile_rows": int(dims[0]), "tiles_per_row": int(dims[1]), "rows_per_tile": int(dims[2]), "h": h, "plain": h >= 0}
+        for q, k in enumerate(PLAIN_KEYS):
+            d[k] = int(cnt[q])
+        return d
+
     def world_masks(self):
         g, w = C.c_int32(), C.c_int32()
         n = _check(lib().rt_debug_world_masks(self._h, None, 0, C.byref(g), C.byref(w)))
```

Result: no change. 4.453 million Mrays/s, median of 6 (+0.9%).
